# wenet-e2e/wesep

Measured on AMD Instinct MI355X. Metric: utterances/sec (4 s, 16 kHz, 2-spk) fwd+bwd, pBSRNN, higher is better.
Workload: dtype bf16x3+fp16x2+fp16x1 split products (+fp8 lo terms), fp32 accumulate; 1 GPU; pBSRNN FiLM multi-fuse, 6 repeats, feature_dim 128, fixed 256-d embeddings; fwd + SI-SDR + bwd + per-tensor clip + Adam-L2; bf16x3 (x-projections, projections, d(hcat), BN / mask GEMMs) + fp16x2 (recurrent products of all four recurrence kernels, d(xn)) + fp16x1 (LSTM weight gradients); 2-byte saved gates / d(gates); fp32 accumulate; BPTT kernels: W_hh as fp16 hi + block-scaled FP8 lo; the lo term; rows_per_gpu=32, global_rows=32, samples_per_row=64000, parallelism=dp1

## Files before the change

include/wesep_hip.h:

```cpp
#ifndef WESEP_HIP_H_
#define WESEP_HIP_H_

#ifdef __cplusplus
extern "C" {
#endif

#define WS_ABI_VERSION 20
#define WS_OK 0
#define WS_ERR_INVALID (-1)
#define WS_ERR_LAUNCH (-2)

int ws_abi_version(void);
const char* ws_last_error(void);

#define WS_PROF_LSTM_FWD 0
#define WS_PROF_LSTM_BWD 1
#define WS_PROF_GEMM_NT 2
#define WS_PROF_GEMM_TN 3
#define WS_PROF_NKINDS 4
int ws_prof_enable(int on);
int ws_prof_collect(int kind, double* total_ms, long long* launches);
int ws_debug_dirty_lds(float value, int nblocks, int spins, float* sink, void* stream);
int ws_debug_occupy(int nblocks, int usec, const unsigned* stop, float* sink, void* stream);

// ... 76 lines not shown

int ws_reduce_slabs(const float* slab, int nsplit, long long stride, long long count,
                    float* out, int w, long long ldo, void* stream);

int ws_transpose(const float* src, int rows, int cols, long long lds, float* dst, void* stream);

typedef struct ws_groups_geom {
  const int* band_w;
  const int* band_off;
  long long gs1, gs2, rs;
  int ngroups, gdiv, L, W;
  int nbands, pad_;
} ws_groups_geom;
int ws_group_stats(const float* x, const ws_groups_geom* geo, float eps, float* stats, void* stream);
int ws_group_stats_len(const float* x, const ws_groups_geom* geo, const int* glen, int glen_div, float eps, float* stats,
                       void* stream);

int ws_gn_bwd_reduce(const float* x, const float* dxn, const float* stats, const float* gamma,
                     const float* const* gamma_tab, const ws_groups_geom* geo, float* ab,
                     void* stream);
int ws_gn_bwd_apply(const float* x, const float* dxn, const float* stats, const float* ab,
                    const float* gamma, const float* const* gamma_tab, const float* res,
                    const ws_groups_geom* geo, float* dx, void* stream);
int ws_gn_param_grad(const float* x, const float* dxn, const float* stats,
                     const ws_groups_geom* geo, int nsplit, float* slab, void* stream);

int ws_gn_bwd_fused(const float* x, const float* dxn, const float* stats, const float* gamma,
                    const float* res, const ws_groups_geom* geo, int nwg, float* dx, float* pslab,
                    float* pout, unsigned* counter, void* stream);
int ws_gn_bwd_fused2(const float* x, const float* dxn, const float* dxn2, const float* stats, const float* gamma,
                     const float* res, const ws_groups_geom* geo, int nwg, float* dx, float* pslab,
                     float* pout, unsigned* counter, void* stream);
int ws_gn_bwd_apply_pg(const float* x, const float* dxn, const float* stats, const float* ab,
                       const float* gamma, const float* res, const ws_groups_geom* geo, float* dx,
                       float* pslab, float* pout, unsigned* counter, void* stream);

typedef struct ws_lstm_args {
  float* gates;
  float* cbuf;
  float* hcat;
  const float* dhcat;
  const float* wpack;
  long long sq_s1, sq_s2, step_rows;
  int nseq, sq_div, L, mode;
  const unsigned* run_if;
  const float* gates_in;
  float* dgates;
  int gfmt;
  int rfmt;
  const unsigned* amax;
  float* dxn;
  long long dxn_dir_stride;
  const float* wxpack;
} ws_lstm_args;
#define WS_GATES_F32 0
#define WS_GATES_H2 1
#define WS_GATES_H2S 2
#define WS_GATES_H2F 3
#define WS_DGATES_EXP 8
#define WS_LSTM_F32_MT1 1
#define WS_LSTM_F32_MT2 2
#define WS_LSTM_BF16X3 3
#define WS_LSTM_BF16X3_BLK 4
#define WS_LSTM_BF16X3_BLK16 5
#define WS_LSTM_H 256
#define WS_LSTM_PACK_FLOATS (2 * 4 * WS_LSTM_H * WS_LSTM_H)
int ws_lstm_pack(const float* whh_f, const float* whh_r, float* pack_fwd, float* pack_bwd,
                 int mode, void* stream);
int ws_lstm_pack_bwd_f8(const float* whh_f, const float* whh_r, float* pack_bwd, void* stream);
#define WS_LSTM_DX_PACK_FLOATS (16 * (48 * 1024 + 64) / 4)
int ws_lstm_pack_dx_f8(const float* wcat, float* pack, void* stream);
int ws_lstm_fwd(const ws_lstm_args* a, void* stream);
int ws_lstm_bwd(const ws_lstm_args* a, void* stream);
typedef struct ws_lstm_cluster_args {
  float* gates;
  float* cbuf;
  float* hcat;
  const float* dhcat;
  const float* whh_f;
  const float* whh_r;
  void* xchg;
  unsigned* flags;
  unsigned* status;
  int nseq, L;
  int dbg, gfmt;
  const float* gates_in;
} ws_lstm_cluster_args;
int ws_lstm_fwd_cluster(const ws_lstm_cluster_args* a, void* stream);
typedef struct ws_lstm_cluster2_args {
  float* gates;
  float* cbuf;
  float* hcat;
  const float* xn;
  const float* wcat;
  const float* bcat;
  const float* whh_f;
  const float* whh_r;
  void* xchg;
  unsigned* tword;
  unsigned* status;
  int nseq, L;
  int dbg, rfmt;
  float* dbg_buf;
} ws_lstm_cluster2_args;
int ws_lstm_fwd_cluster2(const ws_lstm_cluster2_args* a, void* stream);
int ws_lstm_bwd_cluster(const ws_lstm_cluster_args* a, void* stream);
typedef struct ws_lstm_pair_args {
  float* gates;
  const float* cbuf;
  const float* dhcat;
  const float* wpack;
  void* xchg;
  unsigned* flags;
  unsigned* status;
  float* dbg_buf;
  int nseq, L;
  int dbg, gfmt;
  float* dgates;
  const unsigned* amax;
  int rfmt, pad_;
} ws_lstm_pair_args;
int ws_lstm_pack_pair(const float* whh_f, const float* whh_r, float* pack, void* stream);
int ws_lstm_pack_pair_f16(const float* whh_f, const float* whh_r, float* pack, void* stream);
int ws_lstm_pack_pair_f8(const float* whh_f, const float* whh_r, float* pack, void* stream);
int ws_lstm_pack_pair_f8mx(const float* whh_f, const float* whh_r, float* pack, void* stream);
int ws_lstm_bwd_pair(const ws_lstm_pair_args* a, void* stream);
int ws_lstm_cat_ih(const float* wih_f, const float* wih_r, const float* bih_f, const float* bhh_f,
                   const float* bih_r, const float* bhh_r, int n_in, float* wcat, float* bcat,
                   void* stream);

typedef struct ws_seqmap {
  long long sq_s1, sq_s2, step_rows;
  int nseq, sq_div, L;
  int nvalid;
} ws_seqmap;

int ws_pack_w(const float* W, int N, int K, long long ldw, int trans, int order, float* out,
              void* stream);
int ws_pack_w_f16(const float* W, int N, int K, long long ldw, int trans, int order, float* out,
                  void* stream);
int ws_pack_w_f16f8(const float* W, int N, int K, long long ldw, int trans, float* out, void* stream);

typedef struct ws_gemm_p2b_args {
  const float* A;
  const float* Wpack;
  const float* bias;
  float* C;
  float* A_bl;
  const float* stats;
  const float* gamma;
  const float* beta;
  ws_seqmap sm;
  long long lda, st_m1, st_m2, st_base;
  int st_div1, st_div2, N, K;
  const unsigned* run_if;
  unsigned* amax;
  void* A_bl16;
} ws_gemm_p2b_args;
int ws_gemm_p2b(const ws_gemm_p2b_args* a, void* stream);
int ws_gemm_p2b_len(const ws_gemm_p2b_args* a, const int* steps, int steps_div, void* stream);

typedef struct ws_gemm_b2p_args {
  const float* A;
  const float* Wpack;
  const float* bias;
  const float* R;
  float* C;
  ws_seqmap sm;
  long long ldc;
  int N, K;
  int a_fmt, pad_;
  const unsigned* amax;
  void* a16_out;
} ws_gemm_b2p_args;
int ws_gemm_b2p(const ws_gemm_b2p_args* a, void* stream);

typedef struct ws_gemm_tnb_args {
  const float* G;
  const float* A0;
  const float* A1;
  float* slab;
  float* bslab;
  float* aslab;
  long long slab_stride, bslab_stride, aslab_stride;
  int g_width, g_off, g_cols;
  int a0_width, a0_off, a0_cols, a0_shift;
  int a1_width, a1_off, a1_cols, a1_shift;
  int nblk, L, nsplit, blocks_per_split;
  int g_fmt;
  const unsigned* amax;
  int a_fmt, pad_;
} ws_gemm_tnb_args;
int ws_gemm_tnb(const ws_gemm_tnb_args* a, void* stream);

typedef struct ws_bands {
  const int* band_of_bin;
  const int* band_f0;
  const int* band_bw;
  int nband, nbins;
} ws_bands;
int ws_stft_bandsplit(const float* wav, int R, int T, const ws_bands* b, float* xbs, void* stream);
int ws_stft_bandsplit_len(const float* wav, int R, int T, const int* lengths, const ws_bands* b, float* xbs, void* stream);
int ws_mask_istft_frames(const float* xbs, const float* mask3, int R, int Tf, const ws_bands* b,
                         float* frames, void* stream);
int ws_istft_ola(const float* frames, int R, int Tf, int T, float* wav, void* stream);
int ws_istft_ola_len(const float* frames, int R, int Tf, int T, const int* lengths, float* wav, void* stream);
int ws_mask_istft_bwd(const float* dwav, const float* xbs, const float* mask3, int R, int Tf,
                      int T, const ws_bands* b, float* dmask3, void* stream);

int ws_affine_fwd(const float* z, const float* a, const float* b, float a0, long long rows,
// ... 229 lines not shown
```

wesep_amd/_lib.py:

```python
import ctypes as C
import os

import numpy as np
import torch

_HERE = os.path.dirname(os.path.abspath(__file__))
LIB_PATH = os.environ.get("WESEP_HIP_LIB") or os.path.join(_HERE, "libwesep_hip.so")

WS_OK = 0
PROF_LSTM_FWD, PROF_LSTM_BWD, PROF_GEMM_NT, PROF_GEMM_TN = 0, 1, 2, 3
LSTM_H = 256
ABI_VERSION = 20
GATES_F32, GATES_H2, GATES_H2S, GATES_H2F = 0, 1, 2, 3
DGATES_EXP = 8


def dgates_scale(amax_bits: int) -> float:
    e = (int(amax_bits) >> 23) & 0xFF
    return 1.0 if e in (0, 255) else 2.0 ** (min(max(DGATES_EXP + 254 - e, 1), 253) - 127)


LSTM_F32_MT1, LSTM_F32_MT2, LSTM_BF16X3, LSTM_BF16X3_BLK, LSTM_BF16X3_BLK16 = 1, 2, 3, 4, 5
LSTM_PACK_FLOATS = 2 * 4 * LSTM_H * LSTM_H

# ... 13 lines not shown

class Conv3x3PackArgs(C.Structure):
    _fields_ = [("src", Conv3x3PackSrc * 5), ("out", _p), ("Cin", _i), ("Cout", _i), ("nsrc", _i), ("flip", _i)]


class Conv3x3Args(C.Structure):
    _fields_ = [(n, _p) for n in ("X", "W", "bias", "R", "Y")] + [(n, _ll) for n in ("ldx", "ldw", "ldy")] + \
               [(n, _i) for n in ("B", "H", "Wd", "Cin", "Cout", "pad_")]


class Conv3x3WgradArgs(C.Structure):
    _fields_ = [(n, _p) for n in ("G", "X", "slab", "bslab")] + [(n, _ll) for n in ("ldg", "ldx", "slab_stride", "bslab_stride")] + \
               [(n, _i) for n in ("B", "H", "Wd", "Wx", "sw", "Cin", "Nn", "nsplit", "tiles_per_split", "pad_")]


class HeadsArgs(C.Structure):
    _fields_ = [(n, _p) for n in ("x", "dy", "slope", "gamma", "beta", "y", "stats", "dx", "slab")] + \
               [(n, _ll) for n in ("ldx", "lddx")] + [(n, _i) for n in ("B", "T", "Tp", "Q", "nh", "ch", "nwg")] + \
               [("eps", C.c_float)]


class GemmNTArgs(C.Structure):
    _fields_ = [(n, _p) for n in ("A", "W", "bias", "C", "R", "T", "stats", "gamma", "beta", "groups")] + \
               [(n, _ll) for n in ("a_s1", "a_s2", "c_s1", "c_s2", "st_m1", "st_m2", "st_base")] + \
               [(n, _i) for n in ("a_div", "c_div", "st_div1", "st_div2", "M", "N", "K", "ldw",
                                  "act", "ngroups", "max_n", "vec")] + [("conv", ConvView)]


class GemmTNArgs(C.Structure):
    _fields_ = [(n, _p) for n in ("G", "A", "slab", "bslab", "stats", "gamma", "beta", "groups")] + \
               [(n, _ll) for n in ("g_s1", "g_s2", "a_s1", "a_s2", "st_m1", "st_m2", "st_base",
                                   "slab_stride", "bslab_stride", "out_off", "bout_off")] + \
               [(n, _i) for n in ("g_div", "a_div", "st_div1", "st_div2", "M", "Nn", "Kk",
                                  "rows_per_split", "nsplit", "shift_rows", "seq_div", "seq_len",
                                  "ngroups", "max_n", "max_k", "vec")] + [("conv", ConvView)]


class ConvWgradArgs(C.Structure):
    _fields_ = [(n, _p) for n in ("G", "X", "slab", "bslab")] + \
               [(n, _ll) for n in ("ldg", "slab_stride", "bslab_stride")] + \
               [(n, _i) for n in ("M", "Nn", "nsplit", "tiles_per_split")] + [("conv", ConvView)]


class GroupsGeom(C.Structure):
    _fields_ = [("band_w", _p), ("band_off", _p), ("gs1", _ll), ("gs2", _ll), ("rs", _ll),
                ("ngroups", _i), ("gdiv", _i), ("L", _i), ("W", _i), ("nbands", _i), ("pad_", _i)]


class LstmArgs(C.Structure):
    _fields_ = [(n, _p) for n in ("gates", "cbuf", "hcat", "dhcat", "wpack")] + \
               [(n, _ll) for n in ("sq_s1", "sq_s2", "step_rows")] + \
               [(n, _i) for n in ("nseq", "sq_div", "L", "mode")] + [("run_if", _p)] + \
               [("gates_in", _p), ("dgates", _p), ("gfmt", _i), ("rfmt", _i), ("amax", _p)] + \
               [("dxn", _p), ("dxn_dir_stride", _ll), ("wxpack", _p)]


class SeqMapC(C.Structure):
    _fields_ = [("sq_s1", _ll), ("sq_s2", _ll), ("step_rows", _ll), ("nseq", _i), ("sq_div", _i), ("L", _i), ("nvalid", _i)]


class GemmP2BArgs(C.Structure):
    _fields_ = [(n, _p) for n in ("A", "Wpack", "bias", "C", "A_bl", "stats", "gamma", "beta")] + \
               [("sm", SeqMapC)] + [(n, _ll) for n in ("lda", "st_m1", "st_m2", "st_base")] + \
               [(n, _i) for n in ("st_div1", "st_div2", "N", "K")] + [("run_if", _p), ("amax", _p), ("A_bl16", _p)]


class GemmB2PArgs(C.Structure):
    _fields_ = [(n, _p) for n in ("A", "Wpack", "bias", "R", "C")] + [("sm", SeqMapC), ("ldc", _ll), ("N", _i), ("K", _i),
                                                                         ("a_fmt", _i), ("pad_", _i), ("amax", _p), ("a16_out", _p)]


class GemmTNBArgs(C.Structure):
    _fields_ = [(n, _p) for n in ("G", "A0", "A1", "slab", "bslab", "aslab")] + \
               [(n, _ll) for n in ("slab_stride", "bslab_stride", "aslab_stride")] + \
               [(n, _i) for n in ("g_width", "g_off", "g_cols", "a0_width", "a0_off", "a0_cols", "a0_shift",
                                  "a1_width", "a1_off", "a1_cols", "a1_shift", "nblk", "L", "nsplit",
                                  "blocks_per_split", "g_fmt")] + [("amax", _p), ("a_fmt", _i), ("pad_", _i)]


class LstmClusterArgs(C.Structure):
    _fields_ = [(n, _p) for n in ("gates", "cbuf", "hcat", "dhcat", "whh_f", "whh_r", "xchg", "flags", "status")] + \
               [("nseq", _i), ("L", _i), ("dbg", _i), ("gfmt", _i), ("gates_in", _p)]


class LstmCluster2Args(C.Structure):
    _fields_ = [(n, _p) for n in ("gates", "cbuf", "hcat", "xn", "wcat", "bcat", "whh_f", "whh_r", "xchg", "tword", "status")] + \
               [("nseq", _i), ("L", _i), ("dbg", _i), ("rfmt", _i), ("dbg_buf", _p)]


class LstmPairArgs(C.Structure):
    _fields_ = [(n, _p) for n in ("gates", "cbuf", "dhcat", "wpack", "xchg", "flags", "status", "dbg_buf")] + \
               [("nseq", _i), ("L", _i), ("dbg", _i), ("gfmt", _i), ("dgates", _p), ("amax", _p), ("rfmt", _i), ("pad_", _i)]


class Bands(C.Structure):
    _fields_ = [("band_of_bin", _p), ("band_f0", _p), ("band_bw", _p), ("nband", _i), ("nbins", _i)]


GROUP_NT_DTYPE = np.dtype([("W", "<u8"), ("bias", "<u8"), ("gamma", "<u8"), ("beta", "<u8"),
                           ("a_off", "<i8"), ("c_off", "<i8"), ("st_base", "<i8"),
                           ("K", "<i4"), ("N", "<i4"), ("ldw", "<i4"), ("pad_", "<i4")])
GROUP_TN_DTYPE = np.dtype([("gamma", "<u8"), ("beta", "<u8"), ("g_off", "<i8"), ("a_off", "<i8"),
                           ("st_base", "<i8"), ("out_off", "<i8"), ("bout_off", "<i8"),
                           ("Nn", "<i4"), ("Kk", "<i4"), ("pad0_", "<i4"), ("pad1_", "<i4")])
TENSOR_REF_DTYPE = np.dtype([("param", "<u8"), ("grad", "<u8"), ("exp_avg", "<u8"),
                             ("exp_avg_sq", "<u8"), ("numel", "<i8")])
assert GROUP_NT_DTYPE.itemsize == 72 and GROUP_TN_DTYPE.itemsize == 72 and TENSOR_REF_DTYPE.itemsize == 40

class LstmFusedArgs(C.Structure):
    _fields_ = [("gates", _p), ("cbuf", _p), ("hcat", _p), ("xn", _p), ("wpack", _p), ("bias", _p),
                ("nseq", _i), ("L", _i), ("gfmt", _i), ("hfmt", _i)]


LSTM_FUSED_PACK_FLOATS = 2 * 8 * 24 * 4 * 2 * 64 * 4
LSTM_DX_PACK_FLOATS = 16 * (48 * 1024 + 64) // 4

_SIGS = {
    "ws_abi_version": (_i, []),
    "ws_last_error": (C.c_char_p, []),
    "ws_prof_enable": (_i, [_i]),
    "ws_prof_collect": (_i, [_i, C.POINTER(C.c_double), C.POINTER(_ll)]),
    "ws_debug_dirty_lds": (_i, [_f, _i, _i, _p, _p]),
    "ws_debug_occupy": (_i, [_i, _i, _p, _p, _p]),
    "ws_pack_w_f16": (_i, [_p, _i, _i, _ll, _i, _i, _p, _p]),
    "ws_pack_w_f16f8": (_i, [_p, _i, _i, _ll, _i, _p, _p]),
    "ws_gemm_nt": (_i, [C.POINTER(GemmNTArgs), _p]),
    "ws_gemm_tn": (_i, [C.POINTER(GemmTNArgs), _p]),
    "ws_reduce_slabs": (_i, [_p, _i, _ll, _ll, _p, _i, _ll, _p]),
    "ws_transpose": (_i, [_p, _i, _i, _ll, _p, _p]),
    "ws_group_stats": (_i, [_p, C.POINTER(GroupsGeom), _f, _p, _p]),
    "ws_group_stats_len": (_i, [_p, C.POINTER(GroupsGeom), _p, _i, _f, _p, _p]),
    "ws_gn_bwd_reduce": (_i, [_p, _p, _p, _p, _p, C.POINTER(GroupsGeom), _p, _p]),
    "ws_gn_bwd_apply": (_i, [_p, _p, _p, _p, _p, _p, _p, C.POINTER(GroupsGeom), _p, _p]),
    "ws_gn_param_grad": (_i, [_p, _p, _p, C.POINTER(GroupsGeom), _i, _p, _p]),
    "ws_gn_bwd_fused": (_i, [_p, _p, _p, _p, _p, C.POINTER(GroupsGeom), _i, _p, _p, _p, _p, _p]),
    "ws_gn_bwd_fused2": (_i, [_p, _p, _p, _p, _p, _p, C.POINTER(GroupsGeom), _i, _p, _p, _p, _p, _p]),
    "ws_gn_bwd_apply_pg": (_i, [_p, _p, _p, _p, _p, _p, C.POINTER(GroupsGeom), _p, _p, _p, _p, _p]),
    "ws_lstm_pack": (_i, [_p, _p, _p, _p, _i, _p]),
    "ws_lstm_fwd": (_i, [C.POINTER(LstmArgs), _p]),
    "ws_lstm_bwd": (_i, [C.POINTER(LstmArgs), _p]),
    "ws_lstm_fwd_cluster": (_i, [C.POINTER(LstmClusterArgs), _p]),
    "ws_lstm_bwd_cluster": (_i, [C.POINTER(LstmClusterArgs), _p]),
    "ws_lstm_fwd_cluster2": (_i, [C.POINTER(LstmCluster2Args), _p]),
    "ws_lstm_pack_pair": (_i, [_p, _p, _p, _p]),
    "ws_lstm_pack_pair_f16": (_i, [_p, _p, _p, _p]),
# ... 158 lines not shown
```

wesep_amd/blstm_core.py:

```python
import math
import os
from typing import NamedTuple

import numpy as np
import torch

from . import _lib as L
from . import dev

H = L.LSTM_H
G4 = 4 * H
N = 128


def _empty(dev_, *shape):
    return torch.empty(*shape, device=dev_, dtype=torch.float32)


def _reduce_new(slab, nsplit, stride, shape):
    out = _empty(slab.device, *shape)
    dev.reduce_slabs(slab, nsplit, stride, int(np.prod(shape)), out)
    return out


def _h2_probe() -> int:
    return int(os.environ.get("WESEP_H2_PROBE", "0"))


_PROBE_SAT = [0, 0.0]


def _probe_round(t, kind, packed=False):
    if kind == "f16":
        t.copy_(t.half().float())
    elif kind == "u16":
        v = t.view(-1, 2, 4, 64 * 128)
        v[:, :, 2].mul_(0.5).add_(0.5)
        v.copy_(torch.floor(v * 65535.0 + 0.5) / 65535.0)
        v[:, :, 2].mul_(2.0).sub_(1.0)
    elif packed and torch.cuda.is_available():
        t.view(torch.int32).bitwise_and_(-65536)
    else:
        t.copy_(t.bfloat16().float())


def tnb_a16() -> bool:
    return os.environ.get("WESEP_TNB_A16", "1") != "0"


def pair_rfmt(gfmt) -> int:
    rf = int(os.environ.get("WESEP_PAIR_RF", "3"))
    if rf not in (0, 1, 2, 3):
        raise ValueError(f"WESEP_PAIR_RF={rf}: 0, 1, 2 or 3")
    return rf if gfmt == L.GATES_H2F else 0


def dxn_fmt(g_fmt) -> int:
    return 3 if g_fmt == 2 and os.environ.get("WESEP_DXN_F8", "1") != "0" else g_fmt


def band_rfmt(gfmt, lmode) -> int:
    rf = int(os.environ.get("WESEP_BAND_RF", "3"))
    if rf not in (0, 2, 3):
        raise ValueError(f"WESEP_BAND_RF={rf}: 0, 2 or 3")
    if rf == 3 and os.environ.get("WESEP_BAND_DX", "0") == "1":
        rf = 2
    return rf if gfmt == L.GATES_H2F and lmode == L.LSTM_BF16X3_BLK else 0


def band_dx(brf, seq, geo) -> bool:
    return (brf == 2 and os.environ.get("WESEP_BAND_DX", "0") == "1" and not seq.nvalid and dev.gn_bwd_fused_ok(geo))


_SIDE_STREAMS = {}


def _side_stream(device):
    key = (device.type, device.index)
    if key not in _SIDE_STREAMS:
        pr = os.environ.get("WESEP_SIDE_PRIORITY")
        _SIDE_STREAMS[key] = torch.cuda.Stream(device=device, priority=int(pr)) if pr else torch.cuda.Stream(device=device)
    return _SIDE_STREAMS[key]
# ... 199 lines not shown
        self.cache.note(kind)
        return self.cache.get(self.sig, key, lambda: self._build(kind))

    def _build(self, kind):
        W, lmode, pair_rf = self, self.lmode, self.pair_rf
        wih_f, whh_f, bih_f, bhh_f, wih_r, whh_r, bih_r, bhh_r, proj_w = self.weights
        d = wih_f.device
        N = wih_f.shape[1]
        if kind == "cat":
            wcat, bcat = _empty(d, 2 * G4, N), _empty(d, 2 * G4)
            dev.lstm_cat_ih(wih_f.contiguous(), wih_r.contiguous(), bih_f, bhh_f, bih_r, bhh_r, N, wcat, bcat)
            return wcat, bcat
        if kind == "whh":
            return whh_f.contiguous(), whh_r.contiguous()
        if kind == "hh":
            pack_f, pack_b = _empty(d, L.LSTM_PACK_FLOATS), _empty(d, L.LSTM_PACK_FLOATS)
            dev.lstm_pack(*W("whh"), pack_f, pack_b, lmode)
            return pack_f, pack_b
        if kind == "hh8":
            pack = _empty(d, L.LSTM_PACK_FLOATS)
            dev.lstm_pack_bwd_f8(*W("whh"), pack)
            return pack
        if kind == "wx8":
            pack = _empty(d, L.LSTM_DX_PACK_FLOATS)
            dev.lstm_pack_dx_f8(W("cat")[0], pack)
            return pack
        if kind in ("hhp", "hhp16"):
            pack = _empty(d, L.LSTM_PACK_FLOATS)
            dev.lstm_pack_pair(*W("whh"), pack, f16=pair_rf if kind == "hhp16" else 0)
            return pack
        if kind in ("fused", "fused16", "fused8"):
            fpack = _empty(d, L.LSTM_FUSED_PACK_FLOATS)
            dev.lstm_pack_fused(wih_f.contiguous(), wih_r.contiguous(), *W("whh"), fpack,
                                hfmt={"fused": 0, "fused16": 1, "fused8": 5}[kind])
            return fpack
        if kind == "wih":
            out = _empty(d, 2 * G4 * N)
            dev.pack_w(W("cat")[0], 2 * G4, N, N, out, order=0)
            return out
        if kind in ("wihT", "wihT16", "wihT8"):
            out = _empty(d, N * 2 * G4)
            dev.pack_w(W("cat")[0], N, 2 * G4, N, out, trans=True, order=1, f16={"wihT": 0, "wihT16": 1, "wihT8": 2}[kind])
            return out
        if kind == "pw":
            return proj_w.contiguous()
        if kind == "proj":
            out = _empty(d, N * 2 * H)
            dev.pack_w(W("pw"), N, 2 * H, 2 * H, out, order=1)
            return out
        if kind == "projT":
            out = _empty(d, 2 * H * N)
            dev.pack_w(W("pw"), 2 * H, N, 2 * H, out, trans=True, order=0)
            return out
        raise KeyError(kind)


class BlstmPlan(NamedTuple):
    nb: int
    lmode: int
    cluster: bool
    fwd: str
    bptt: str
    grad: bool
    gfmt: int
    g_fmt: int
    a16: bool
    pair_rfmt: int
    band_rfmt: int
    band_dx: bool
    a_fmt: int


_WIHT_KIND = {0: "wihT", 1: "wihT", 2: "wihT16", 3: "wihT8"}


def make_plan(seq, device, grad, gn_geo=None, ragged=False) -> BlstmPlan:
    lmode = dev.lstm_blk_mode(seq.nseq)
    cluster = dev.lstm_cluster_ok(seq, device)
    bptt = _bptt_kind(seq, device, cluster)
    gfmt = L.GATES_F32 if bptt == "cluster" else dev.gates_fmt()
    h2 = gfmt != L.GATES_F32
    if ragged:
        fwd = "cluster" if cluster else "stream"
    elif dev.lstm_fuse_ok(seq.nseq, cluster):
        fwd = "fused"
    elif cluster:
        fwd = "cluster2" if h2 and dev.lstm_cluster2_on() else "cluster"
    else:
        fwd = "stream"
    g_fmt = {L.GATES_H2: 1, L.GATES_H2F: 2}.get(gfmt, 0)
    brf = band_rfmt(gfmt, lmode) if grad and bptt == "stream" else 0
    return BlstmPlan(
        nb=dev.bl_num_blocks(seq), lmode=lmode, cluster=cluster, fwd=fwd, bptt=bptt, grad=grad, gfmt=gfmt, g_fmt=g_fmt,
        a16=gfmt == L.GATES_H2F and grad and tnb_a16(), pair_rfmt=pair_rfmt(gfmt) if grad and bptt == "pair" else 0,
        band_rfmt=brf, band_dx=bool(brf) and gn_geo is not None and band_dx(brf, seq, gn_geo), a_fmt=dxn_fmt(g_fmt))


def consume_once(ctx, who):
    if ctx.consumed:
        raise L.WesepHipError(f"{who}: second backward through the same graph (retain_graph / multi-loss loops): "
                              "the blocked path consumes its saved gates in place; run the forward again")
    ctx.consumed = True


def blstm_forward(plan, W, x, seq, res, bias, norm=None, steps=None):
    d = x.device
    norm = norm or {}
    if steps is not None and (plan.fwd in ("fused", "cluster2") or plan.grad):
        raise L.WesepHipError(f"blstm_forward: per-sequence step counts with forward branch '{plan.fwd}', grad={plan.grad}: "
                              "only the branches over precomputed gates know them, and only the forward")
    lens = dict(steps=steps[0], steps_div=steps[1]) if steps is not None else {}
    nb, gfmt, lmode = plan.nb, plan.gfmt, plan.lmode
    h2 = gfmt != L.GATES_F32
    wcat, bcat = W("cat")
    whf, whr = W("whh")
    xn = _empty(d, nb, 32 * N)
    cbuf, hcat = _empty(d, nb, 32 * 2 * H), _empty(d, nb, 32 * 2 * H)
    gates = _empty(d, dev.blh_floats(nb, 2 * G4)) if h2 else _empty(d, nb, 32 * 2 * G4)
    xn16 = _empty(d, dev.blh_floats(nb, N)) if plan.a16 else None
    hcat16 = _empty(d, dev.blh_floats(nb, 2 * H)) if plan.a16 else None
    if plan.fwd == "fused":
        dev.gemm_p2b(A=x, lda=N, sm=seq, Wpack=None, N=0, C_out=None, A_bl=xn, A_bl16=xn16, **norm)
        hf = dev.lstm_fused_hfmt(gfmt)
        dev.lstm_fwd_fused(gates, cbuf, hcat, xn, W("fused8" if hf & 4 else "fused16" if hf else "fused"), bcat, seq, gfmt=gfmt,
                           hfmt=hf)
    elif plan.fwd == "cluster2":
        dev.gemm_p2b(A=x, lda=N, sm=seq, Wpack=None, N=0, C_out=None, A_bl=xn, A_bl16=xn16, **norm)
        tw = dev.lstm_fwd_cluster2(gates, cbuf, hcat, xn, wcat, bcat, whf, whr, seq, dbg=_cluster_dbg())
        pre = dev.fallback_scratch(d, nb * 32 * 2 * G4)
        dev.gemm_p2b(A=x, lda=N, sm=seq, Wpack=W("wih"), N=2 * G4, C_out=pre, bias=bcat, run_if=tw, **norm)
        dev.lstm_fwd(gates, cbuf, hcat, W("hh")[0], seq, lmode, run_if=tw, gfmt=gfmt, gates_in=pre)
        del pre
    else:
        pre = _empty(d, nb, 32 * 2 * G4) if h2 else gates
        xproj = dict(A=x, lda=N, sm=seq, Wpack=W("wih"), N=2 * G4, C_out=pre, bias=bcat, A_bl=xn, A_bl16=xn16, **norm, **lens)
        rec = dict(gfmt=gfmt, gates_in=pre) if h2 else {}
        dev.gemm_p2b(**xproj)
        if _h2_probe() & 768 and not torch.cuda.is_available():
            pre.copy_(pre.half().float() if _h2_probe() & 256 else pre.bfloat16().float())
        if plan.fwd == "cluster":
            tw = dev.lstm_fwd_cluster(gates, cbuf, hcat, whf, whr, seq, dbg=_cluster_dbg(), **rec)
            if not h2:
                dev.gemm_p2b(run_if=tw, **xproj)
            dev.lstm_fwd(gates, cbuf, hcat, W("hh")[0], seq, lmode, run_if=tw, **rec)
        else:
            dev.lstm_fwd(gates, cbuf, hcat, W("hh")[0], seq, lmode, **rec)
        del pre
    out = torch.empty_like(res)
    dev.gemm_b2p(A=hcat, K=2 * H, sm=seq, Wpack=W("proj"), C_out=out, ldc=N, bias=bias, R=res, a16_out=hcat16)
    if _h2_probe() and not h2:
        if _h2_probe() & 1:
            _probe_round(gates, "f16")
        if _h2_probe() & 8:
            _probe_round(gates, "u16")
        if _h2_probe() & 4:
            _probe_round(cbuf, "f16")
    if plan.grad:
        W("projT")
        if not plan.band_dx:
            W(_WIHT_KIND[plan.a_fmt])
        if plan.bptt == "pair":
            W("hhp16" if plan.pair_rfmt else "hhp")
        if (plan.bptt == "stream" and not plan.band_rfmt) or (plan.bptt == "pair" and h2):
            W("hh")
        if plan.bptt == "stream" and plan.band_rfmt:
            W("hh8")
            if plan.band_dx:
                W("wx8")
    return out, (gates, cbuf, hcat, xn16 if plan.a16 else xn, hcat16)


def blstm_bptt(plan, W, gates, cbuf, hcat, dout, seq, release):
    d = dout.device
    nb, gfmt = plan.nb, plan.gfmt
    dh, dout_bl = _empty(d, nb, 32 * 2 * H), _empty(d, nb, 32 * N)
    dxn2 = None
    amax = amax_word(d) if gfmt == L.GATES_H2F else None
    dev.gemm_p2b(A=dout, lda=N, sm=seq, Wpack=W("projT"), N=2 * H, C_out=dh, A_bl=dout_bl, amax=amax)
    if _h2_probe() & 16:
        _probe_round(dh, "bf16")
    ready = mark_wgrads_ready(d) if release else None
    if plan.bptt == "cluster":
        dg = gates
        dev.lstm_bwd_cluster(gates, cbuf, dh, *W("whh"), seq)
    elif gfmt == L.GATES_F32:
        dg = gates
        if plan.bptt == "pair":
            dev.lstm_bwd_pair(gates, cbuf, dh, W("hhp"), seq, dbg=_pair_dbg())
        else:
            dev.lstm_bwd(gates, cbuf, hcat, dh, W("hh")[1], seq, plan.lmode)
    elif plan.bptt == "pair":
        dg = _empty(d, nb, 32 * 2 * G4) if gfmt == L.GATES_H2S else _empty(d, dev.blh_floats(nb, 2 * G4))
        rf = plan.pair_rfmt
        tw = dev.lstm_bwd_pair(gates, cbuf, dh, W("hhp16" if rf else "hhp"), seq, gfmt=gfmt, dgates=dg, repairable=True,
                               dbg=_pair_dbg(), amax=amax, rfmt=rf, dbg_buf=_pair_stamp_buf(d, seq.L))
        dev.lstm_bwd(gates, cbuf, hcat, dh, W("hh")[1], seq, plan.lmode, gfmt=gfmt, dgates=dg, run_if=tw, amax=amax)
    else:
        dg = _empty(d, nb, 32 * 2 * G4) if gfmt == L.GATES_H2S else gates
        brf = plan.band_rfmt
        if plan.band_dx:
            dxn2 = _empty(d, 2, dout.numel() // N, N)
        dev.lstm_bwd(gates, cbuf, hcat, dh, W("hh8") if brf else W("hh")[1], seq, plan.lmode, gfmt=gfmt,
                     dgates=dg if gfmt == L.GATES_H2S else None, amax=amax, rfmt=brf, dxn=dxn2,
                     wxpack=W("wx8") if dxn2 is not None else None)
    if _h2_probe() & 2 and gfmt == L.GATES_F32:
        _probe_round(gates, "bf16", packed=True)
    if _h2_probe() & 32 and gfmt == L.GATES_F32 and not torch.cuda.is_available():
        amax = float(dh.abs().max())
        S = 2.0 ** (10 - math.floor(math.log2(amax))) if amax > 0 and math.isfinite(amax) else 1.0
        sc = gates * S
        _PROBE_SAT[0] += int((sc.abs() > 65504.0).sum())
        _PROBE_SAT[1] = max(_PROBE_SAT[1], float(sc.abs().max()) / 65504.0)
        gates.copy_(sc.clamp(-65504.0, 65504.0).half().float() / S)
    if ready is not None:
        flush_deferred_wgrads(d, ready)
    return dg, dout_bl, amax, dxn2


def weight_grads(gates, xn, hcat, dout_bl, seq, nb, g_fmt=0, amax=None, hcat16=None):
    d = gates.device
    a_fmt = 1 if hcat16 is not None else 0
    if _h2_probe() & 192 and not torch.cuda.is_available() and not a_fmt:
        rnd = (lambda t: t.half().float()) if _h2_probe() & 64 else (lambda t: t.bfloat16().float())
        xn, hcat = rnd(xn), rnd(hcat)
    if os.environ.get("WESEP_PROBE_SKIP_WGRAD") == "1":
        z_ = lambda *s_: torch.zeros(*s_, device=d)
        return [z_(G4, N), z_(G4, H), z_(G4), z_(G4), z_(G4, N), z_(G4, H), z_(G4), z_(G4), z_(N, 2 * H), z_(N)]
    if _h2_probe() & 1024 and not torch.cuda.is_available() and amax is not None:
        S = L.dgates_scale(int(amax.reshape(-1)[0]))
        hcat = hcat.half().float()
        dout_bl = (dout_bl * S).half().float() / S
    ns, bps = dev.tnb_splits(nb, (2 * H) // 128)
    slab, aslab = _empty(d, ns, 2 * H * N), _empty(d, ns, N)
    dev.gemm_tnb(G=hcat, g_width=2 * H, g_off=0, g_cols=2 * H, A0=dout_bl, a0_width=N, a0_off=0, a0_cols=N,
                 nblk=nb, L_=seq.L, slab=slab, nsplit=ns, blocks_per_split=bps, aslab=aslab)
    dproj_w = _reduce_new(slab, ns, 2 * H * N, (2 * H, N)).t().contiguous()
    dproj_b = _reduce_new(aslab, ns, N, (N,))
    ns, bps = dev.tnb_splits(nb, G4 // 128)
    slab, bslab = _empty(d, ns, G4 * (N + H)), _empty(d, ns, G4)
    dwih, dwhh, db = [], [], []
    for di in (0, 1):
        dev.gemm_tnb(G=gates, g_width=2 * G4, g_off=di * G4, g_cols=G4, A0=xn, a0_width=N, a0_off=0,
                     a0_cols=N, A1=hcat16 if a_fmt else hcat, a1_width=2 * H, a1_off=di * H, a1_cols=H,
                     a1_shift=(-1 if di == 0 else 1), nblk=nb, L_=seq.L, slab=slab, nsplit=ns,
                     blocks_per_split=bps, bslab=bslab, g_fmt=g_fmt, amax=amax, a_fmt=a_fmt)
        dw = _reduce_new(slab, ns, G4 * (N + H), (G4, N + H))
        dwih.append(dw[:, :N].contiguous())
        dwhh.append(dw[:, N:].contiguous())
        db.append(_reduce_new(bslab, ns, G4, (G4,)))
    return [dwih[0], dwhh[0], db[0], db[0].clone(), dwih[1], dwhh[1], db[1], db[1].clone(),
            dproj_w, dproj_b]


def blstm_weight_grads(plan, dg, xn, hcat, dout_bl, amax, hcat16, seq, box, order=tuple(range(10))):
    if box is None:
        wg = weight_grads(dg, xn, hcat, dout_bl, seq, plan.nb, plan.g_fmt, amax, hcat16)
        return [wg[i] for i in order]
# ... 19 lines not shown
```

wesep_amd/csrc/gemm_blk.hip:

```cpp
#include <stdlib.h>

#include <type_traits>

#include "common.h"

typedef __bf16 bf16x8 __attribute__((ext_vector_type(8)));
typedef unsigned int u32x4 __attribute__((ext_vector_type(4)));
typedef unsigned int u32x2 __attribute__((ext_vector_type(2)));
typedef float f32x2 __attribute__((ext_vector_type(2)));
typedef _Float16 f16x8 __attribute__((ext_vector_type(8)));
typedef _Float16 f16x2 __attribute__((ext_vector_type(2)));
typedef int i32x4 __attribute__((ext_vector_type(4)));
typedef int v8i __attribute__((ext_vector_type(8)));
typedef __fp16 h16x2 __attribute__((ext_vector_type(2)));

__device__ __forceinline__ f32x16 mfma32(bf16x8 a, bf16x8 b, f32x16 c) {
  return __builtin_amdgcn_mfma_f32_32x32x16_bf16(a, b, c, 0, 0, 0);
}

__device__ __forceinline__ void split8(const float* v, bf16x8& hi, bf16x8& lo) {
#pragma unroll
  for (int j = 0; j < 8; ++j) {
    hi[j] = (__bf16)v[j];
    lo[j] = (__bf16)(v[j] - (float)hi[j]);
// ... 108 lines not shown
__global__ __launch_bounds__(256) void pack_w16f8_kernel(const float* __restrict__ W, int K, long long ldw, int trans,
                                                         unsigned char* __restrict__ out) {
  const int st = blockIdx.x, nt = threadIdx.x >> 6, lane = threadIdx.x & 63, n = 32 * nt + (lane & 31);
  unsigned char* sb = out + (long long)st * 24576;
  float res[32];
  float mx = 0.f;
#pragma unroll
  for (int i = 0; i < 4; ++i) {
    f16x8 hi;
#pragma unroll
    for (int j = 0; j < 8; ++j) {
      const int k = 64 * st + 16 * i + 8 * (lane >> 5) + j;
      const float v = WS_PACK16_SCALE * (trans ? W[(long long)k * ldw + n] : W[(long long)n * ldw + k]);
      hi[j] = (_Float16)v;
      res[8 * i + j] = v - (float)hi[j];
      mx = fmaxf(mx, fabsf(res[8 * i + j]));
    }
    reinterpret_cast<f16x8*>(sb)[(i * 4 + nt) * 64 + lane] = hi;
  }
#pragma unroll
  for (int o = 32; o >= 1; o >>= 1) mx = fmaxf(mx, __shfl_xor(mx, o));
  int E = mx > 0.f ? ((__float_as_int(mx) >> 23) & 255) - 127 - 7 : 0;
  E = max(E, -126);
  const float inv = __int_as_float((127 - E) << 23);
  unsigned int* o8 = reinterpret_cast<unsigned int*>(sb + 16384 + nt * 2048 + lane * 16);
#pragma unroll
  for (int j = 0; j < 32; j += 4) {
    int c = 0;
    c = __builtin_amdgcn_cvt_pk_fp8_f32(res[j] * inv, res[j + 1] * inv, c, false);
    c = __builtin_amdgcn_cvt_pk_fp8_f32(res[j + 2] * inv, res[j + 3] * inv, c, true);
    o8[(j >> 4) * 256 + ((j & 15) >> 2)] = (unsigned int)c;
  }
  if (lane == 0) (out + (long long)(K / 64) * 24576)[st * 4 + nt] = (unsigned char)(127 + E);
}

extern "C" int ws_pack_w_f16f8(const float* W, int N, int K, long long ldw, int trans, float* out, void* stream) {
  WS_REQUIRE(W && out && N == 128 && K > 0 && K % 64 == 0, "ws_pack_w_f16f8: N = 128, K %% 64 (N=%d K=%d)", N, K);
  hipLaunchKernelGGL(pack_w16f8_kernel, dim3(K / 64), dim3(256), 0, (hipStream_t)stream, W, K, ldw, trans,
                     reinterpret_cast<unsigned char*>(out));
  return ws_check_launch("ws_pack_w_f16f8");
}

extern "C" int ws_pack_w(const float* W, int N, int K, long long ldw, int trans, int order, float* out,
                         void* stream) {
  WS_REQUIRE(W && out && N > 0 && K > 0 && N % 32 == 0 && K % 16 == 0, "ws_pack_w: N %% 32, K %% 16 (N=%d K=%d)",
             N, K);
  WS_REQUIRE(order == 0 || order == 1, "ws_pack_w: order");
  hipLaunchKernelGGL(pack_w_kernel, dim3((N * K / 8 + 255) / 256), dim3(256), 0, (hipStream_t)stream, W, N, K, ldw,
                     trans, order, reinterpret_cast<__bf16*>(out));
  return ws_check_launch("ws_pack_w");
}

#define P2B_K 128
template <bool LEN>
__global__ __launch_bounds__(512, 4) void gemm_p2b_kernel(const ws_gemm_p2b_args p, const int* __restrict__ steps,
                                                          int steps_div) {
  __shared__ __attribute__((aligned(16))) u32x4 wl[2][2048];
  if (p.run_if && *p.run_if == 0u) return;
  const int tid = threadIdx.x, lane = tid & 63, i = lane & 31, half = lane >> 5;
  const int w = __builtin_amdgcn_readfirstlane(tid >> 6);
  const int nblk = ((p.sm.nseq + 31) / 32) * p.sm.L;
  const int b = blockIdx.x * 8 + w;
  const bool active = b < nblk;
  const int bb = active ? b : nblk - 1;
  bool valid;
  const long long pos = seq_pos(p.sm, bb, i, valid);
  if (LEN) {
    const int tile = bb / p.sm.L, step = bb - tile * p.sm.L;
    const int nv = p.sm.nvalid > 0 ? p.sm.nvalid : p.sm.nseq;
    valid = valid && step < steps[min(tile * 32 + i, nv - 1) / steps_div];
  }

  bf16x8 xh[8], xl[8];
  {
    const float* arow = p.A + pos * p.lda;
    float mean = 0.f, rstd = 1.f;
    if (p.stats) {
      const long long s = (pos / p.st_div1) * p.st_m1 + (pos % p.st_div2) * p.st_m2 + p.st_base;
      mean = p.stats[2 * s];
      rstd = p.stats[2 * s + 1];
    }
    float* eb = p.A_bl ? p.A_bl + (long long)bb * (32 * P2B_K) + i * 4 : nullptr;
    unsigned short* eb16 = p.A_bl16 ? reinterpret_cast<unsigned short*>(p.A_bl16) + (long long)bb * (32 * P2B_K) + i * 4 : nullptr;
#pragma unroll
    for (int ks = 0; ks < 8; ++ks) {
      const int k0 = 16 * ks + 8 * half;
      f32x4 v0 = *reinterpret_cast<const f32x4*>(arow + k0);
      f32x4 v1 = *reinterpret_cast<const f32x4*>(arow + k0 + 4);
      if (p.stats) {
        const f32x4 g0 = *reinterpret_cast<const f32x4*>(p.gamma + k0), g1 = *reinterpret_cast<const f32x4*>(p.gamma + k0 + 4);
        const f32x4 b0 = *reinterpret_cast<const f32x4*>(p.beta + k0), b1 = *reinterpret_cast<const f32x4*>(p.beta + k0 + 4);
        v0 = (v0 - mean) * rstd * g0 + b0;
        v1 = (v1 - mean) * rstd * g1 + b1;
      }
      if (!valid) {
        v0 = f32x4{0.f, 0.f, 0.f, 0.f};
        v1 = v0;
      }
      const float v[8] = {v0[0], v0[1], v0[2], v0[3], v1[0], v1[1], v1[2], v1[3]};
      split8(v, xh[ks], xl[ks]);
      if (eb && active) {
        u32x4 c0, c1;
        pack8(xh[ks], xl[ks], c0, c1);
        *reinterpret_cast<u32x4*>(eb + (k0 / 4) * 128) = c0;
        *reinterpret_cast<u32x4*>(eb + (k0 / 4 + 1) * 128) = c1;
      }
      if (eb16 && active) {
        const f16x2 h0 = {(_Float16)v[0], (_Float16)v[1]}, h1 = {(_Float16)v[2], (_Float16)v[3]};
        const f16x2 h2 = {(_Float16)v[4], (_Float16)v[5]}, h3 = {(_Float16)v[6], (_Float16)v[7]};
        *reinterpret_cast<u32x2*>(eb16 + (k0 / 4) * 128) = u32x2{__builtin_bit_cast(unsigned, h0), __builtin_bit_cast(unsigned, h1)};
        *reinterpret_cast<u32x2*>(eb16 + (k0 / 4 + 1) * 128) = u32x2{__builtin_bit_cast(unsigned, h2), __builtin_bit_cast(unsigned, h3)};
      }
    }
  }

  const int nstage = p.N / 64;
  if (nstage == 0) return;
  const u32x4* wsrc = reinterpret_cast<const u32x4*>(p.Wpack);
  u32x4 wreg[4];
#pragma unroll
  for (int q = 0; q < 4; ++q) wreg[q] = wsrc[tid + 512 * q];
#pragma unroll
  for (int q = 0; q < 4; ++q) wl[0][tid + 512 * q] = wreg[q];
  __syncthreads();
  float* cblk = p.C + (long long)bb * 32 * p.N + i * 4;
  float cmax = 0.f;
  for (int st = 0; st < nstage; ++st) {
    const int cur = st & 1;
    if (st + 1 < nstage) {
#pragma unroll
      for (int q = 0; q < 4; ++q) wreg[q] = wsrc[(long long)(st + 1) * 2048 + tid + 512 * q];
    }
#pragma unroll
    for (int t2 = 0; t2 < 2; ++t2) {
      const u32x4* wt = &wl[cur][t2 * 1024 + lane];
      f32x16 acc;
#pragma unroll
      for (int ks = 0; ks < 8; ++ks) {
        const bf16x8 ah = __builtin_bit_cast(bf16x8, wt[(ks * 2) * 64]);
        const bf16x8 al = __builtin_bit_cast(bf16x8, wt[(ks * 2 + 1) * 64]);
        if (ks == 0) {
          const f32x16 zero = {0.f, 0.f, 0.f, 0.f, 0.f, 0.f, 0.f, 0.f, 0.f, 0.f, 0.f, 0.f, 0.f, 0.f, 0.f, 0.f};
          acc = mfma32(ah, xh[ks], zero);
        } else {
          acc = mfma32(ah, xh[ks], acc);
        }
        acc = mfma32(al, xh[ks], acc);
        acc = mfma32(ah, xl[ks], acc);
      }
      if (active) {
        const int n0 = st * 64 + t2 * 32;
#pragma unroll
        for (int j = 0; j < 4; ++j) {
          const int n = n0 + 8 * j + 4 * half;
          f32x4 v = {acc[4 * j], acc[4 * j + 1], acc[4 * j + 2], acc[4 * j + 3]};
          if (p.bias) v += *reinterpret_cast<const f32x4*>(p.bias + n);
          if (!valid) v = f32x4{0.f, 0.f, 0.f, 0.f};
          *reinterpret_cast<f32x4*>(cblk + (n / 4) * 128) = v;
          cmax = fmaxf(fmaxf(cmax, fmaxf(fabsf(v[0]), fabsf(v[1]))), fmaxf(fabsf(v[2]), fabsf(v[3])));
        }
      }
    }
    if (st + 1 < nstage) {
#pragma unroll
      for (int q = 0; q < 4; ++q) wl[cur ^ 1][tid + 512 * q] = wreg[q];
    }
    __syncthreads();
  }
  if (p.amax) {
#pragma unroll
    for (int o = 32; o > 0; o >>= 1) cmax = fmaxf(cmax, __shfl_xor(cmax, o, 64));
    if (lane == 0) atomicMax(p.amax, __float_as_uint(cmax));
  }
}

static int gemm_p2b_launch(const char* who, const ws_gemm_p2b_args* a, const int* steps, int steps_div, void* stream) {
  WS_REQUIRE(a && a->A && ((a->Wpack && a->C) || (a->N == 0 && (a->A_bl || a->A_bl16))), "%s: null pointer", who);
  WS_REQUIRE(a->K == P2B_K, "%s: K must be %d (got %d)", who, P2B_K, a->K);
  WS_REQUIRE(a->N >= 0 && a->N % 64 == 0, "%s: N %% 64 (N=%d)", who, a->N);
  WS_REQUIRE(a->lda >= a->K && a->lda % 4 == 0, "%s: lda", who);
  WS_REQUIRE(a->sm.nseq > 0 && a->sm.L > 0 && a->sm.sq_div > 0, "%s: bad sequence map", who);
  WS_REQUIRE(!a->stats || (a->gamma && a->beta && a->st_div1 > 0 && a->st_div2 > 0), "%s: norm args", who);
  const int nblk = ((a->sm.nseq + 31) / 32) * a->sm.L;
  hipStream_t s = (hipStream_t)stream;
  const bool timed = a->run_if == nullptr;
  if (timed) ws_prof_begin(WS_PROF_GEMM_NT, s);
  if (steps)
    hipLaunchKernelGGL((gemm_p2b_kernel<true>), dim3((nblk + 7) / 8), dim3(512), 0, s, *a, steps, steps_div);
  else
    hipLaunchKernelGGL((gemm_p2b_kernel<false>), dim3((nblk + 7) / 8), dim3(512), 0, s, *a, steps, steps_div);
  if (timed) ws_prof_end(WS_PROF_GEMM_NT, s);
  return ws_check_launch(who);
}

extern "C" int ws_gemm_p2b(const ws_gemm_p2b_args* a, void* stream) {
  return gemm_p2b_launch("ws_gemm_p2b", a, nullptr, 1, stream);
}

extern "C" int ws_gemm_p2b_len(const ws_gemm_p2b_args* a, const int* steps, int steps_div, void* stream) {
  WS_REQUIRE(steps && steps_div > 0, "ws_gemm_p2b_len: steps table / steps_div");
  return gemm_p2b_launch("ws_gemm_p2b_len", a, steps, steps_div, stream);
}

template <int A16>
__global__ __launch_bounds__(512, 4) void gemm_b2p_kernel(const ws_gemm_b2p_args p) {
  __shared__ __attribute__((aligned(16))) u32x4 wl[2][2048];
  __shared__ long long posl[8][32];
  const int tid = threadIdx.x, lane = tid & 63, i = lane & 31, half = lane >> 5;
  const int w = __builtin_amdgcn_readfirstlane(tid >> 6);
  const int nblk = ((p.sm.nseq + 31) / 32) * p.sm.L;
  const int b = blockIdx.x * 8 + w;
  const bool active = b < nblk;
  const int bb = active ? b : nblk - 1;
  {
    bool valid;
    const long long pos = seq_pos(p.sm, bb, i, valid);
    if (half == 0) posl[w][i] = valid ? pos : -1;
  }
  const int K = p.K, nstage = K / 64;
  typedef typename std::conditional<A16 != 0, u32x2, f32x4>::type acell;
  typedef typename std::conditional<A16 != 0, unsigned short, float>::type aelem;
  constexpr int SU = A16 == 3 ? 1536 : 2048, NQ = SU / 512;
  const int* wsc = reinterpret_cast<const int*>(reinterpret_cast<const unsigned char*>(p.Wpack) + (long long)nstage * 24576);
  int sc_n = A16 == 3 ? wsc[0] : 0;
  const float inv_s = A16 >= 2 ? ws_dgates_scale_inv(*p.amax) * (1.f / WS_PACK16_SCALE) : 1.f;
  const aelem* ab = reinterpret_cast<const aelem*>(p.A) + (long long)bb * 32 * K + i * 4 + 2 * half * 128;
  const __amdgpu_buffer_rsrc_t wsr = __builtin_amdgcn_make_buffer_rsrc(const_cast<float*>(p.Wpack), 0, (unsigned)nstage * SU * 16u,
                                                                        0x00020000);
  auto wstage = [&](int st, int buf) {
#pragma unroll
    for (int q = 0; q < NQ; ++q)
      __builtin_amdgcn_raw_ptr_buffer_load_lds(wsr, (__attribute__((address_space(3))) void*)&wl[buf][(w * NQ + q) * 64], 16, lane * 16,
                                               (st * SU + (w * NQ + q) * 64) * 16, 0, 0);
  };
  constexpr int HS = A16 == 0 ? 2 : 1, KH = 4 / HS;
  acell an[2 * KH];
  auto load_a = [&](int st, int hs) {
    const aelem* a2 = ab + ((long long)st * 16 + hs * KH * 4) * 128;
#pragma unroll
    for (int ks = 0; ks < KH; ++ks) {
      an[2 * ks] = *reinterpret_cast<const acell*>(a2 + (4 * ks) * 128);
      an[2 * ks + 1] = *reinterpret_cast<const acell*>(a2 + (4 * ks + 1) * 128);
    }
// ... 704 lines not shown
```

wesep_amd/csrc/lstm.hip:

```cpp
#include "common.h"

#define LH WS_LSTM_H
#define LG (4 * LH)
#define HL_LD 68
#define DG_LD 260

__device__ __forceinline__ f32x4 mfma16(float a, float b, f32x4 c) {
  return __builtin_amdgcn_mfma_f32_16x16x4f32(a, b, c, 0, 0, 0);
}

__device__ __forceinline__ float fast_sigmoid(float x) {
  return __builtin_amdgcn_rcpf(1.f + __expf(-x));
}
__device__ __forceinline__ float fast_tanh(float x) {
  const float ax = fabsf(x);
  const float e = __expf(-2.f * ax);
  const float t = (1.f - e) * __builtin_amdgcn_rcpf(1.f + e);
  return copysignf(t, x);
}

__global__ void lstm_pack_kernel(const float* __restrict__ whh_f, const float* __restrict__ whh_r,
                                 float* __restrict__ pf, float* __restrict__ pb) {
  const int total = 2 * LG * LH;
  for (int idx = blockIdx.x * blockDim.x + threadIdx.x; idx < total; idx += gridDim.x * blockDim.x) {
// ... 302 lines not shown
#pragma unroll
      for (int s = 0; s < 2; ++s)
#pragma unroll
        for (int r = 0; r < 4; ++r) dh[mt][s][r] = 0.f;
    const float* arow = dgl + (lq * 16 + l15) * DG_LD;
    f32x4 bcur[2], bnxt[2];
    bcur[0] = b00;
    bcur[1] = b01;
#pragma unroll 4
    for (int ks4 = 0; ks4 < 64; ++ks4) {
      if (ks4 + 1 < 64) {
        bnxt[0] = wp[((ks4 + 1) * 2 + 0) * 64];
        bnxt[1] = wp[((ks4 + 1) * 2 + 1) * 64];
      }
      f32x4 a[MT];
#pragma unroll
      for (int mt = 0; mt < MT; ++mt)
        a[mt] = *reinterpret_cast<const f32x4*>(arow + mt * (64 * DG_LD) + 4 * ks4);
#pragma unroll
      for (int q = 0; q < 4; ++q)
#pragma unroll
        for (int s = 0; s < 2; ++s)
#pragma unroll
          for (int mt = 0; mt < MT; ++mt) dh[mt][s] = mfma16(a[mt][q], bcur[s][q], dh[mt][s]);
      bcur[0] = bnxt[0];
      bcur[1] = bnxt[1];
    }
    __syncthreads();
  }
}

static int lstm_check(const ws_lstm_args* a, bool bwd, const char* who) {
  WS_REQUIRE(a && a->gates && a->cbuf && a->hcat && a->wpack, "%s: null pointer", who);
  WS_REQUIRE(!bwd || a->dhcat, "%s: null dhcat", who);
  WS_REQUIRE(a->nseq > 0 && a->L > 0 && a->sq_div > 0, "%s: bad nseq/L/sq_div", who);
  WS_REQUIRE((a->mode & 255) >= WS_LSTM_F32_MT1 && (a->mode & 255) <= WS_LSTM_BF16X3_BLK16, "%s: bad mode %d", who,
             a->mode);
  WS_REQUIRE(!a->run_if || (!bwd && (a->mode & 255) >= WS_LSTM_BF16X3) || (bwd && (a->mode & 255) >= WS_LSTM_BF16X3_BLK),
             "%s: run_if is honoured by the split-bf16 forward kernels and the blocked-layout BPTT kernels only", who);
  WS_REQUIRE(a->gfmt >= WS_GATES_F32 && a->gfmt <= WS_GATES_H2F, "%s: bad gfmt %d", who, a->gfmt);
  WS_REQUIRE(a->gfmt != WS_GATES_H2F || !bwd || a->amax, "%s: WS_GATES_H2F needs amax", who);
  WS_REQUIRE(a->gfmt == WS_GATES_F32 || (a->mode & 255) >= WS_LSTM_BF16X3_BLK,
             "%s: gfmt %d is a format of the blocked-layout modes", who, a->gfmt);
  WS_REQUIRE(a->gfmt == WS_GATES_F32 || bwd || a->gates_in, "%s: gfmt %d needs gates_in (the fp32 pre-activations)", who,
             a->gfmt);
  WS_REQUIRE(a->gfmt != WS_GATES_H2S || !bwd || a->dgates, "%s: WS_GATES_H2S needs dgates", who);
  WS_REQUIRE(a->gfmt == WS_GATES_F32 || ((a->mode >> 8) & 7) == 0, "%s: probe builds are WS_GATES_F32 only", who);
  WS_REQUIRE(a->rfmt == 0 || ((a->rfmt == 2 || a->rfmt == 3) && bwd && a->mode == WS_LSTM_BF16X3_BLK && a->gfmt == WS_GATES_H2F),
             "%s: rfmt %d (2 / 3 = fp16 recurrence on fp16 + FP8 weights, 3: the lo term on the FP8 MFMA: ws_lstm_bwd, "
             "WS_LSTM_BF16X3_BLK, WS_GATES_H2F only)", who, a->rfmt);
  WS_REQUIRE(!a->dxn || (bwd && a->rfmt == 2 && a->wxpack && a->dxn_dir_stride > 0 && a->dxn_dir_stride < (1ll << 29) && !a->run_if),
             "%s: dxn (d(xn) inside the BPTT, ABI v19) needs rfmt 2, wxpack (ws_lstm_pack_dx_f8), 0 < dxn_dir_stride < 2^29 floats "
             "(32-bit store offsets) and no run_if", who);
  return WS_OK;
}

extern "C" int ws_lstm_fwd(const ws_lstm_args* a, void* stream) {
  int rc = lstm_check(a, false, "ws_lstm_fwd");
  if (rc != WS_OK) return rc;
  hipStream_t s = (hipStream_t)stream;
  const int per = 16 * a->mode;
  dim3 grid((a->nseq + per - 1) / per, 2), block(512);
  const bool timed = a->run_if == nullptr;
  if (timed) ws_prof_begin(WS_PROF_LSTM_FWD, s);
  if ((a->mode & 255) == WS_LSTM_BF16X3_BLK16)
    ws_launch_lstm_fwd_s16(a, s);
  else if ((a->mode & 255) >= WS_LSTM_BF16X3)
    ws_launch_lstm_fwd_bf16(a, s);
  else if (a->mode == WS_LSTM_F32_MT1)
    hipLaunchKernelGGL((lstm_fwd_kernel<1>), grid, block, 0, s, *a);
  else
    hipLaunchKernelGGL((lstm_fwd_kernel<2>), grid, block, 0, s, *a);
  if (timed) ws_prof_end(WS_PROF_LSTM_FWD, s);
  return ws_check_launch("ws_lstm_fwd");
}

extern "C" int ws_lstm_bwd(const ws_lstm_args* a, void* stream) {
  int rc = lstm_check(a, true, "ws_lstm_bwd");
  if (rc != WS_OK) return rc;
  hipStream_t s = (hipStream_t)stream;
  const int per = 16 * a->mode;
  dim3 grid((a->nseq + per - 1) / per, 2), block(512);
  const bool timed = a->run_if == nullptr;
  if (timed) ws_prof_begin(WS_PROF_LSTM_BWD, s);
  if ((a->mode & 255) == WS_LSTM_BF16X3_BLK16)
    ws_launch_lstm_bwd_s16(a, s);
  else if ((a->mode & 255) >= WS_LSTM_BF16X3)
    ws_launch_lstm_bwd_bf16(a, s);
  else if (a->mode == WS_LSTM_F32_MT1)
    hipLaunchKernelGGL((lstm_bwd_kernel<1>), grid, block, 0, s, *a);
  else
    hipLaunchKernelGGL((lstm_bwd_kernel<2>), grid, block, 0, s, *a);
  if (timed) ws_prof_end(WS_PROF_LSTM_BWD, s);
  return ws_check_launch("ws_lstm_bwd");
}
```

wesep_amd/csrc/lstm_bf16.hip:

```cpp
#include <stdlib.h>

#include "lstm_bf16_common.h"

__global__ void lstm_pack_bf16_kernel(const float* __restrict__ whh_f, const float* __restrict__ whh_r,
                                      __bf16* __restrict__ pf, __bf16* __restrict__ pb) {
  const int total = 2 * LG * LH;
  for (int idx = blockIdx.x * blockDim.x + threadIdx.x; idx < total; idx += gridDim.x * blockDim.x) {
    {
      int r = idx;
      const int j = r & 7; r >>= 3;
      const int lane = r & 63; r >>= 6;
      const int g = r & 3; r >>= 2;
      const int ks = r & 15; r >>= 4;
      const int w = r & 7; r >>= 3;
      const int d = r;
      const float* W = d ? whh_r : whh_f;
      const int row = g * 256 + 32 * w + (lane & 31);
      const int k = 16 * ks + 8 * (lane >> 5) + j;
      const float v = W[row * LH + k];
      const __bf16 hi = (__bf16)v;
      const long long unit = ((((long long)(d * 8 + w) * 16 + ks) * 4 + g) * 2) * 64 + lane;
      pf[unit * 8 + j] = hi;
      pf[(unit + 64) * 8 + j] = (__bf16)(v - (float)hi);
    }
// ... 223 lines not shown
      for (int j = 0; j < 4; ++j)
#pragma unroll
        for (int r = 0; r < 4; ++r) acc[g][4 * j + r] += xg[g][j][r];
    if (!(DBG & 2)) {
#pragma unroll
      for (int j = 0; j < 4; ++j)
#pragma unroll
        for (int g = 0; g < 4; ++g) xg[g][j] = ld_gate(tn, g, j);
    }
    __builtin_amdgcn_sched_barrier(0);
#pragma unroll
    for (int j = 0; j < 4; ++j) {
      f32x4 pre[4];
#pragma unroll
      for (int g = 0; g < 4; ++g)
#pragma unroll
        for (int r = 0; r < 4; ++r) pre[g][r] = acc[g][4 * j + r];
      f32x4 vi, vf, vg, vo, vc, vh;
      const f32x4 cold = *reinterpret_cast<const f32x4*>(cme + 8 * j);
#pragma unroll
      for (int r = 0; r < 4; ++r) {
        const float ig = fsig(pre[0][r]);
        const float fg = fsig(pre[1][r]);
        const float gg = ftanh(pre[2][r]);
        const float og = fsig(pre[3][r]);
        const float cn = fg * cold[r] + ig * gg;
        vi[r] = ig;
        vf[r] = fg;
        vg[r] = gg;
        vo[r] = og;
        vc[r] = cn;
        vh[r] = og * ftanh(cn);
      }
      bf16x4 h_hi, h_lo;
      split4(vh, h_hi, h_lo);
      *reinterpret_cast<bf16x4*>(nhi + 8 * j) = h_hi;
      *reinterpret_cast<bf16x4*>(nlo + 8 * j) = h_lo;
      *reinterpret_cast<f32x4*>(cme + 8 * j) = vc;
      if (!(DBG & 1) || step == L - 1) {
        st_gate(vi, t, 0, j);
        st_gate(vf, t, 1, j);
        st_gate(vg, t, 2, j);
        st_gate(vo, t, 3, j);
        st_ch(vc, p.cbuf, t, j);
        if constexpr (BLK) st_ch(pack_hl4(h_hi, h_lo), p.hcat, t, j);
        else st_ch(vh, p.hcat, t, j);
      }
      __builtin_amdgcn_sched_barrier(0);
    }
    __syncthreads();
  }
}

template <bool BLK, int DBG, int GF = 0, int RF = 0, bool DX = false>
__global__ __launch_bounds__(512, 2) void lstm_bwd_bf16_kernel(const ws_lstm_args p) {
  static_assert(RF == 0 || (BLK && GF == WS_GATES_H2F), "the fp16 recurrence takes the scaled-fp16 d(gates) of WS_GATES_H2F");
  static_assert(!DX || RF == 2, "d(xn) in the BPTT rides on the fp16 d(gates) image of rfmt 2");
  __shared__ __attribute__((aligned(16))) __bf16 dgl[RF ? 1 : 2][SQ * DROW];
  __shared__ __attribute__((aligned(16))) f32x4 xred[DX ? 8 * 2 * 64 : 1];
  if (p.run_if && *p.run_if == 0u) return;
  const int d = blockIdx.y, bx = blockIdx.x;
  const int tid = threadIdx.x, lane = tid & 63, l31 = lane & 31, half = lane >> 5;
  const int w = __builtin_amdgcn_readfirstlane(tid >> 6);
  const int L = p.L;
  const int ss = min(bx * SQ + l31, p.nseq - 1);
  const long long rowbase =
      BLK ? 0 : (long long)(ss / p.sq_div) * p.sq_s1 + (long long)(ss % p.sq_div) * p.sq_s2;
  const int ubase = 32 * w + 4 * half;
  const int glane = ((d * 256 + 8 * w + half) * 32 + l31) * 16;
  const int clane = ((d * 64 + 8 * w + half) * 32 + l31) * 16;
  auto goff = [&](int t, int g, int j) -> long long {
    return ((rowbase + (long long)t * p.step_rows) * 2 + d) * LG + g * 256 + ubase + 8 * j;
  };
  auto coff = [&](int t, int j) -> long long {
    return (rowbase + (long long)t * p.step_rows) * (2 * LH) + d * LH + ubase + 8 * j;
  };
  float* gdst = GF == WS_GATES_H2S ? p.dgates : p.gates;
  auto grs = [&](int t) { return mkrsrc(gdst + (long long)(bx * L + t) * (SQ * 2 * LG), SQ * 2 * LG * 4); };
  auto hrs = [&](int t) { return mkrsrc(p.gates + (long long)(bx * L + t) * (SQ * LG), SQ * 2 * LG * 2); };
  constexpr bool G2 = GF == WS_GATES_H2 || GF == WS_GATES_H2F;
  float* hdst = (G2 && p.dgates) ? p.dgates : p.gates;
  auto ors = [&](int t) { return mkrsrc(hdst + (long long)(bx * L + t) * (SQ * LG), SQ * 2 * LG * 2); };
  const float dS = GF == WS_GATES_H2F ? ws_dgates_scale(*p.amax) : 1.f;
  auto crs = [&](const float* b, int t) { return mkrsrc(b + (long long)(bx * L + t) * (SQ * 2 * LH), SQ * 2 * LH * 4); };
  typedef typename gate_cell<GF>::type gcell;
  auto ld_gate = [&](int t, int g, int j) -> gcell {
    if constexpr (GF != 0) return bld8(hrs(t), glane >> 1, (g * 64 + 2 * j) * 256);
    else if constexpr (BLK) return bld(grs(t), glane, (g * 64 + 2 * j) * 512);
    else return *reinterpret_cast<const f32x4*>(p.gates + goff(t, g, j));
  };
  auto st_gate = [&](const f32x4& v, int t, int g, int j) {
    if constexpr (BLK) bst(v, grs(t), glane, (g * 64 + 2 * j) * 512);
    else *reinterpret_cast<f32x4*>(p.gates + goff(t, g, j)) = v;
  };
  auto ld_ch = [&](const float* b, int t, int j) -> f32x4 {
    if constexpr (BLK) return bld(crs(b, t), clane, 2 * j * 512);
    else return *reinterpret_cast<const f32x4*>(b + coff(t, j));
  };

  const int kpar = DX ? (w >> 2) : 0;
  const __amdgpu_buffer_rsrc_t wrs = __builtin_amdgcn_make_buffer_rsrc(
      const_cast<float*>(p.wpack) + (long long)(d * 8 + w) * (64 * 2 * 64 * 4), 0, 64 * 2 * 1024, 0x00020000);
  const int wlane = lane * 16;
  bf16x8 wr[2][RF ? 4 : 8];
  u32x2 wq[2][RF ? 4 : 1];
  float wS[RF ? 8 : 1];
  int wE[RF == 3 ? 8 : 1];
  auto wfill = [&](int s, int chunk, int zo) {
    if constexpr (RF != 0) {
#pragma unroll
      for (int q = 0; q < 4; ++q) {
        const int fq = q ^ kpar;
        wr[s][q] = wload(wrs, wlane, zo + chunk * 6144 + fq * 1024);
        wq[s][q] = __builtin_bit_cast(u32x2, __builtin_amdgcn_raw_buffer_load_b64(wrs, lane * 8, zo + chunk * 6144 + 4096 + fq * 512, 0));
      }
    } else {
#pragma unroll
      for (int f = 0; f < 8; ++f) wr[s][f] = wload(wrs, wlane + (f & 3) * 1024, zo + chunk * 8192 + (f >> 2) * 4096);
    }
  };
  typedef _Float16 f16x8 __attribute__((ext_vector_type(8)));
  typedef _Float16 f16x2 __attribute__((ext_vector_type(2)));
  const __amdgpu_buffer_rsrc_t xrs = __builtin_amdgcn_make_buffer_rsrc(
      const_cast<char*>(reinterpret_cast<const char*>(p.wxpack)) + (DX ? (long long)(d * 8 + w) * WS_DX_REGION : 0), 0,
      DX ? WS_DX_REGION : 0, 0x00020000);
  bf16x8 xr[2][DX ? 2 : 1];
  u32x2 xq[2][DX ? 2 : 1];
  float xS[DX ? 8 : 1];
  f32x16 dxa;
  auto xfill = [&](int s, int chunk, int zo) {
    if constexpr (DX) {
#pragma unroll
      for (int q = 0; q < 2; ++q) {
        xr[s][q] = wload(xrs, wlane + q * 1024, zo + chunk * 3072);
        xq[s][q] = __builtin_bit_cast(u32x2, __builtin_amdgcn_raw_buffer_load_b64(xrs, lane * 8 + q * 512, zo + chunk * 3072 + 2048, 0));
      }
    }
  };
  if constexpr (RF != 0) {
    const float* st = p.wpack + (long long)(d * 8 + w) * (64 * 2 * 64 * 4) + 96 * 256;
#pragma unroll
    for (int g8 = 0; g8 < 8; ++g8) wS[g8] = __builtin_bit_cast(float, __builtin_amdgcn_readfirstlane(__builtin_bit_cast(int, st[g8])));
    if constexpr (RF == 3) {
#pragma unroll
      for (int g8 = 0; g8 < 8; ++g8) wE[g8] = (__builtin_bit_cast(int, wS[g8]) >> 23) & 255;
    }
  }
  if constexpr (DX) {
    const float* st = reinterpret_cast<const float*>(reinterpret_cast<const char*>(p.wxpack) + (long long)(d * 8 + w) * WS_DX_REGION + 48 * 1024);
#pragma unroll
    for (int g8 = 0; g8 < 8; ++g8) xS[g8] = __builtin_bit_cast(float, __builtin_amdgcn_readfirstlane(__builtin_bit_cast(int, st[g8])));
  }
  unsigned xoff = 0u;
  if constexpr (DX) {
    const int sq = bx * SQ + l31;
    const long long row = (long long)(sq / p.sq_div) * p.sq_s1 + (long long)(sq % p.sq_div) * p.sq_s2;
    xoff = sq < p.nseq ? (unsigned)(row * 512 + (32 * (w & 3) + 16 * kpar + 4 * half) * 4) : 0x80000000u;
  }
  const __amdgpu_buffer_rsrc_t xors = __builtin_amdgcn_make_buffer_rsrc(
      DX ? p.dxn + (long long)d * p.dxn_dir_stride : nullptr, 0, DX ? (unsigned)(p.dxn_dir_stride * 4) : 0u, 0x00020000);
  gcell n_i[4], n_f[4], n_g[4], n_o[4];
  f32x4 n_dh[4], n_cp[4], c_cur[4], dc[4];
  f32x16 dhr;
  const f32x4 zero4v = {0.f, 0.f, 0.f, 0.f};
#pragma unroll
  for (int j = 0; j < 4; ++j) dc[j] = zero4v;
#pragma unroll
  for (int i = 0; i < 16; ++i) dhr[i] = 0.f;

  auto load_step = [&](int t, int j) {
    n_i[j] = ld_gate(t, 0, j);
    n_f[j] = ld_gate(t, 1, j);
    n_g[j] = ld_gate(t, 2, j);
    n_o[j] = ld_gate(t, 3, j);
    n_dh[j] = ld_ch(p.dhcat, t, j);
    const int tp = d == 0 ? max(t - 1, 0) : min(t + 1, L - 1);
    n_cp[j] = ld_ch(p.cbuf, tp, j);
  };
  {
    const int t0 = d == 0 ? L - 1 : 0;
#pragma unroll
    for (int j = 0; j < 4; ++j) {
      load_step(t0, j);
      c_cur[j] = ld_ch(p.cbuf, t0, j);
    }
  }
  __builtin_amdgcn_sched_barrier(0);
  wfill(0, 0, 0);
  xfill(0, 0, 0);
  wfill(1, 1, 0);
  xfill(1, 1, 0);
  __builtin_amdgcn_sched_barrier(0);

  for (int step = 0; step < L; ++step) {
    const int t = d == 0 ? L - 1 - step : step;
    const int sn = min(step + 1, L - 1);
    const int tn = d == 0 ? L - 1 - sn : sn;
    const bool has_prev = d == 0 ? (t > 0) : (t < L - 1);
    int zo = 0;
    asm volatile("" : "+s"(zo));
    __bf16* dhi = &dgl[0][l31 * DROW + ubase];
    __bf16* dlo = &dgl[RF ? 0 : 1][l31 * DROW + ubase];
#pragma unroll
    for (int j = 0; j < 4; ++j) {
      f32x4 pi, pf, pg, po;
      const f32x4 vi = gate_val<false>(n_i[j]), vf = gate_val<false>(n_f[j]), vg = gate_val<true>(n_g[j]),
                  vo = gate_val<false>(n_o[j]);
#pragma unroll
      for (int r = 0; r < 4; ++r) {
        const float ig = vi[r], fg = vf[r], gg = vg[r], og = vo[r];
        const float dhv = dh_in<GF>(n_dh[j][r], dhr[4 * j + r], dS);
        const float tc = ftanh(c_cur[j][r]);
        const float dov = dhv * tc;
        const float dcv = dc[j][r] + dhv * og * (1.f - tc * tc);
        dc[j][r] = dcv * fg;
        pi[r] = dcv * gg * ig * (1.f - ig);
        pf[r] = dcv * (has_prev ? n_cp[j][r] : 0.f) * fg * (1.f - fg);
        pg[r] = dcv * ig * (1.f - gg * gg);
        po[r] = dov * og * (1.f - og);
      }
      c_cur[j] = n_cp[j];
      const bool st = !(DBG & 1) || step == L - 1;
      auto emit = [&](const f32x4& v, int g) {
        if constexpr (RF != 0) {
          const u32x2 code = enc_f16x4(v);
          *reinterpret_cast<u32x2*>(dhi + 256 * g + 8 * j) = code;
          if (st) bst8(code, ors(t), glane >> 1, (g * 64 + 2 * j) * 256);
          return;
        }
        bf16x4 hi, lo;
        split4(v, hi, lo);
        *reinterpret_cast<bf16x4*>(dhi + 256 * g + 8 * j) = hi;
        *reinterpret_cast<bf16x4*>(dlo + 256 * g + 8 * j) = lo;
        if (st) {
          if constexpr (G2) bst8(enc_dgates<GF>(v, hi), ors(t), glane >> 1, (g * 64 + 2 * j) * 256);
          else if constexpr (BLK) st_gate(pack_hl4(hi, lo), t, g, j);
          else st_gate(v, t, g, j);
        }
      };
      emit(pi, 0);
      emit(pf, 1);
      emit(pg, 2);
      emit(po, 3);
      if (!(DBG & 2)) load_step(tn, j);
      __builtin_amdgcn_sched_barrier(0);
    }
    __syncthreads();

    const __bf16* bhi = &dgl[0][l31 * DROW + 8 * half];
    const __bf16* blo = &dgl[RF ? 0 : 1][l31 * DROW + 8 * half];
    const __bf16* bhx[2] = {bhi + 16 * kpar, bhi - 16 * kpar};
    f32x16 acc0;
    f32x16 acc1;
    v8i b8;
#pragma unroll
    for (int ch = 0; ch < 16; ++ch) {
      const int s = ch & 1;
#pragma unroll
      for (int q = 0; q < 4; ++q) {
        const int ks = 4 * ch + q;
        const bf16x8 bh = *reinterpret_cast<const bf16x8*>((DX ? bhx[q & 1] : bhi) + 16 * ks);
        if constexpr (RF == 3) {
          typedef _Float16 f16x2 __attribute__((ext_vector_type(2)));
          typedef short s16x2 __attribute__((ext_vector_type(2)));
// ... 70 lines not shown
      const bool hi_rows = kpar != 0;
#pragma unroll
      for (int i = 0; i < 2; ++i) {
        f32x4 send;
#pragma unroll
        for (int r = 0; r < 4; ++r) {
          const float lo_v = dxa[4 * i + r], hi_v = dxa[8 + 4 * i + r];
          send[r] = hi_rows ? lo_v : hi_v;
          keep[i][r] = hi_rows ? hi_v : lo_v;
        }
        xred[(w * 2 + i) * 64 + lane] = send;
      }
    }
    __syncthreads();
    if constexpr (DX) {
      const float us = (1.f / 256.f) / dS;
      const unsigned trow = (unsigned)t * (unsigned)p.step_rows * 512u;
#pragma unroll
      for (int i = 0; i < 2; ++i) {
        const f32x4 o = xred[((w ^ 4) * 2 + i) * 64 + lane];
        __builtin_amdgcn_raw_buffer_store_b128(__builtin_bit_cast(u32x4, (keep[i] + o) * us), xors, xoff + trow + 32 * i, 0, 0);
      }
    }
  }
}

#define WS_DBG_DISPATCH(KERNEL)                                                          \
  if ((a->mode & 255) == WS_LSTM_BF16X3_BLK && a->gfmt == WS_GATES_H2) {                 \
    hipLaunchKernelGGL((KERNEL<true, 0, WS_GATES_H2>), grid, block, 0, s, *a);           \
  } else if ((a->mode & 255) == WS_LSTM_BF16X3_BLK && a->gfmt == WS_GATES_H2S) {         \
    hipLaunchKernelGGL((KERNEL<true, 0, WS_GATES_H2S>), grid, block, 0, s, *a);          \
  } else if ((a->mode & 255) == WS_LSTM_BF16X3_BLK && a->gfmt == WS_GATES_H2F) {         \
    hipLaunchKernelGGL((KERNEL<true, 0, WS_GATES_H2F>), grid, block, 0, s, *a);          \
  } else if ((a->mode & 255) == WS_LSTM_BF16X3_BLK) {                                    \
    switch ((a->mode >> 8) & 7) {                                                        \
      case 0: hipLaunchKernelGGL((KERNEL<true, 0>), grid, block, 0, s, *a); break;       \
      case 1: hipLaunchKernelGGL((KERNEL<true, 1>), grid, block, 0, s, *a); break;       \
      case 2: hipLaunchKernelGGL((KERNEL<true, 2>), grid, block, 0, s, *a); break;       \
      case 4: hipLaunchKernelGGL((KERNEL<true, 4>), grid, block, 0, s, *a); break;       \
      default: hipLaunchKernelGGL((KERNEL<true, 7>), grid, block, 0, s, *a); break;      \
    }                                                                                    \
  } else {                                                                               \
    hipLaunchKernelGGL((KERNEL<false, 0>), grid, block, 0, s, *a);                       \
  }

int ws_launch_lstm_fwd_bf16(const ws_lstm_args* a, hipStream_t s) {
  dim3 grid((a->nseq + SQ - 1) / SQ, 2), block(512);
  WS_DBG_DISPATCH(lstm_fwd_bf16_kernel)
  return 0;
}

int ws_launch_lstm_bwd_bf16(const ws_lstm_args* a, hipStream_t s) {
  dim3 grid((a->nseq + SQ - 1) / SQ, 2), block(512);
  if (a->rfmt == 2 && a->dxn) {
    hipLaunchKernelGGL((lstm_bwd_bf16_kernel<true, 0, WS_GATES_H2F, 2, true>), grid, block, 0, s, *a);
    return 0;
  }
  if (a->rfmt == 2) {
    hipLaunchKernelGGL((lstm_bwd_bf16_kernel<true, 0, WS_GATES_H2F, 2>), grid, block, 0, s, *a);
    return 0;
  }
  if (a->rfmt == 3) {
    hipLaunchKernelGGL((lstm_bwd_bf16_kernel<true, 0, WS_GATES_H2F, 3>), grid, block, 0, s, *a);
    return 0;
  }
  WS_DBG_DISPATCH(lstm_bwd_bf16_kernel)
  return 0;
}
```

wesep_amd/csrc/lstm_bf16_common.h:

```cpp
#pragma once
#include "common.h"

typedef __bf16 bf16x8 __attribute__((ext_vector_type(8)));
typedef __bf16 bf16x4 __attribute__((ext_vector_type(4)));

#define LH WS_LSTM_H
#define LG (4 * LH)
#define SQ 32
#define HROW 264
#define DROW 1032

typedef unsigned int u32x4 __attribute__((ext_vector_type(4)));

__device__ __forceinline__ bf16x8 wload(__amdgpu_buffer_rsrc_t rsrc, int voff, int soff) {
  return __builtin_bit_cast(bf16x8, __builtin_amdgcn_raw_buffer_load_b128(rsrc, voff, soff, 0));
}

__device__ __forceinline__ __amdgpu_buffer_rsrc_t mkrsrc(const float* base, unsigned bytes) {
  return __builtin_amdgcn_make_buffer_rsrc(const_cast<float*>(base), 0, bytes, 0x00020000);
}
#ifndef WS_STREAM_AUX
#define WS_STREAM_AUX 2
#endif
__device__ __forceinline__ f32x4 bld(__amdgpu_buffer_rsrc_t r, int voff, int soff) {
// ... 56 lines not shown
  l.y = __builtin_amdgcn_perm(u[3], u[2], WS_SEL_LO16);
  hi = __builtin_bit_cast(bf16x4, h);
  lo = __builtin_bit_cast(bf16x4, l);
}


typedef unsigned int u32x2 __attribute__((ext_vector_type(2)));
#define WS_U16_SIG 65535.f
#define WS_U16_TANH 32767.5f

__device__ __forceinline__ u32x2 bld8(__amdgpu_buffer_rsrc_t r, int voff, int soff) {
  return __builtin_bit_cast(u32x2, __builtin_amdgcn_raw_buffer_load_b64(r, voff, soff, WS_STREAM_AUX));
}
__device__ __forceinline__ void bst8(const u32x2& v, __amdgpu_buffer_rsrc_t r, int voff, int soff) {
  __builtin_amdgcn_raw_buffer_store_b64(v, r, voff + soff, 0, WS_STREAM_AUX);
}
template <bool TANH>
__device__ __forceinline__ u32x2 enc_u16x4(const f32x4& v) {
  const float s = TANH ? WS_U16_TANH : WS_U16_SIG, o = TANH ? WS_U16_TANH + 0.5f : 0.5f;
  unsigned u[4];
#pragma unroll
  for (int j = 0; j < 4; ++j) u[j] = (unsigned)__builtin_fmaf(v[j], s, o);
  return u32x2{u[0] | (u[1] << 16), u[2] | (u[3] << 16)};
}
template <bool TANH>
__device__ __forceinline__ f32x4 dec_u16x4(const u32x2& c) {
  const float s = TANH ? 1.f / WS_U16_TANH : 1.f / WS_U16_SIG, o = TANH ? -1.f : 0.f;
  f32x4 v;
  v[0] = __builtin_fmaf((float)(c[0] & 0xffffu), s, o);
  v[1] = __builtin_fmaf((float)(c[0] >> 16), s, o);
  v[2] = __builtin_fmaf((float)(c[1] & 0xffffu), s, o);
  v[3] = __builtin_fmaf((float)(c[1] >> 16), s, o);
  return v;
}
__device__ __forceinline__ u32x2 bf16x4_bits(const bf16x4& v) { return __builtin_bit_cast(u32x2, v); }
typedef _Float16 f16x4 __attribute__((ext_vector_type(4)));
__device__ __forceinline__ u32x2 enc_f16x4(const f32x4& vs) {
  f16x4 h;
#pragma unroll
  for (int j = 0; j < 4; ++j) h[j] = (_Float16)vs[j];
  return __builtin_bit_cast(u32x2, h);
}
template <int GF>
__device__ __forceinline__ u32x2 enc_dgates(const f32x4& v, const bf16x4& hi) {
  if constexpr (GF == WS_GATES_H2F) return enc_f16x4(v);
  else return bf16x4_bits(hi);
}
template <int GF>
__device__ __forceinline__ float dh_in(float dh, float rec, float S) {
  if constexpr (GF == WS_GATES_H2F) return __builtin_fmaf(dh, S, rec);
  else return dh + rec;
}

template <int GF> struct gate_cell { typedef f32x4 type; };
template <> struct gate_cell<WS_GATES_H2> { typedef u32x2 type; };
template <> struct gate_cell<WS_GATES_H2S> { typedef u32x2 type; };
template <> struct gate_cell<WS_GATES_H2F> { typedef u32x2 type; };
template <bool TANH> __device__ __forceinline__ f32x4 gate_val(const f32x4& c) { return c; }
template <bool TANH> __device__ __forceinline__ f32x4 gate_val(const u32x2& c) { return dec_u16x4<TANH>(c); }
```

wesep_amd/csrc/lstm_bf16_s16.hip:

```cpp
#include "lstm_bf16_common.h"

#define S16 16

__device__ __forceinline__ f32x4 mfma16(bf16x8 a, bf16x8 b, f32x4 c) {
  return __builtin_amdgcn_mfma_f32_16x16x32_bf16(a, b, c, 0, 0, 0);
}

__global__ void lstm_pack_s16_kernel(const float* __restrict__ whh_f, const float* __restrict__ whh_r,
                                     __bf16* __restrict__ pf, __bf16* __restrict__ pb) {
  const int total = 2 * LG * LH;
  for (int idx = blockIdx.x * blockDim.x + threadIdx.x; idx < total; idx += gridDim.x * blockDim.x) {
    {
      int r = idx;
      const int j = r & 7; r >>= 3;
      const int lane = r & 63; r >>= 6;
      const int tile = r & 7; r >>= 3;
      const int ks = r & 7; r >>= 3;
      const int w = r & 7; r >>= 3;
      const int d = r;
      const float* W = d ? whh_r : whh_f;
      const int row = (tile >> 1) * 256 + 32 * w + 16 * (tile & 1) + (lane & 15);
      const int k = 32 * ks + 8 * (lane >> 4) + j;
      const float v = W[row * LH + k];
      const __bf16 hi = (__bf16)v;
// ... 121 lines not shown

    const int sn = min(step + 1, L - 1);
    const int tn = d == 0 ? sn : L - 1 - sn;
#pragma unroll
    for (int g = 0; g < 4; ++g)
#pragma unroll
      for (int tu = 0; tu < 2; ++tu) acc[g][tu] += xg[g][tu];
#pragma unroll
    for (int tu = 0; tu < 2; ++tu)
#pragma unroll
      for (int g = 0; g < 4; ++g) xg[g][tu] = ld_gate(tn, g, tu);
    __builtin_amdgcn_sched_barrier(0);
    __bf16* nhi = &hl[cur ^ 1][0][n * HROW + ubase];
    __bf16* nlo = &hl[cur ^ 1][1][n * HROW + ubase];
#pragma unroll
    for (int tu = 0; tu < 2; ++tu) {
      f32x4 vi, vf, vg, vo, vc, vh;
      const f32x4 cold = *reinterpret_cast<const f32x4*>(cme + 16 * tu);
#pragma unroll
      for (int r = 0; r < 4; ++r) {
        const float ig = fsig(acc[0][tu][r]);
        const float fg = fsig(acc[1][tu][r]);
        const float gg = ftanh(acc[2][tu][r]);
        const float og = fsig(acc[3][tu][r]);
        const float cn = fg * cold[r] + ig * gg;
        vi[r] = ig;
        vf[r] = fg;
        vg[r] = gg;
        vo[r] = og;
        vc[r] = cn;
        vh[r] = og * ftanh(cn);
      }
      bf16x4 h_hi, h_lo;
      split4(vh, h_hi, h_lo);
      *reinterpret_cast<bf16x4*>(nhi + 16 * tu) = h_hi;
      *reinterpret_cast<bf16x4*>(nlo + 16 * tu) = h_lo;
      *reinterpret_cast<f32x4*>(cme + 16 * tu) = vc;
      st_gate(vi, t, 0, tu);
      st_gate(vf, t, 1, tu);
      st_gate(vg, t, 2, tu);
      st_gate(vo, t, 3, tu);
      st_ch(vc, p.cbuf, t, tu);
      st_ch(pack_hl4(h_hi, h_lo), p.hcat, t, tu);
      __builtin_amdgcn_sched_barrier(0);
    }
    __syncthreads();
  }
}


#ifndef S16_DBG
#define S16_DBG 0
#endif
template <int GF>
__global__ __launch_bounds__(512, 2) void lstm_bwd_s16_kernel(const ws_lstm_args p) {
  __shared__ __attribute__((aligned(16))) __bf16 dgl[2][S16 * DROW];
  if (p.run_if && *p.run_if == 0u) return;
  const int d = blockIdx.y;
  const int tile = blockIdx.x >> 1, hb = blockIdx.x & 1;
  const int tid = threadIdx.x, lane = tid & 63, n = lane & 15, mq = lane >> 4;
  const int w = __builtin_amdgcn_readfirstlane(tid >> 6);
  const int L = p.L;
  const int glane = ((d * 256 + 8 * w + mq) * 32 + 16 * hb + n) * 16;
  const int clane = ((d * 64 + 8 * w + mq) * 32 + 16 * hb + n) * 16;
  float* gdst = GF == WS_GATES_H2S ? p.dgates : p.gates;
  auto grs = [&](int t) { return mkrsrc(gdst + (long long)(tile * L + t) * (SQ * 2 * LG), SQ * 2 * LG * 4); };
  auto hrs = [&](int t) { return mkrsrc(p.gates + (long long)(tile * L + t) * (SQ * LG), SQ * 2 * LG * 2); };
  constexpr bool G2 = GF == WS_GATES_H2 || GF == WS_GATES_H2F;
  float* hdst = (G2 && p.dgates) ? p.dgates : p.gates;
  auto ors = [&](int t) { return mkrsrc(hdst + (long long)(tile * L + t) * (SQ * LG), SQ * 2 * LG * 2); };
  const float dS = GF == WS_GATES_H2F ? ws_dgates_scale(*p.amax) : 1.f;
  auto crs = [&](const float* b, int t) { return mkrsrc(b + (long long)(tile * L + t) * (SQ * 2 * LH), SQ * 2 * LH * 4); };
  typedef typename gate_cell<GF>::type gcell;
  auto ld_gate = [&](int t, int g, int tu) -> gcell {
    if constexpr (GF != 0) return bld8(hrs(t), glane >> 1, (g * 64 + 4 * tu) * 256);
    else return bld(grs(t), glane, (g * 64 + 4 * tu) * 512);
  };
  auto st_gate = [&](const f32x4& v, int t, int g, int tu) { bst(v, grs(t), glane, (g * 64 + 4 * tu) * 512); };
  auto ld_ch = [&](const float* b, int t, int tu) -> f32x4 { return bld(crs(b, t), clane, 4 * tu * 512); };
  const int ubase = 32 * w + 4 * mq;

  const __amdgpu_buffer_rsrc_t wrs = __builtin_amdgcn_make_buffer_rsrc(
      const_cast<float*>(p.wpack) + (long long)(d * 8 + w) * (32 * 4 * 64 * 4), 0, 32 * 4 * 1024, 0x00020000);
  const int wlane = lane * 16;
  bf16x8 wr[2][16];
#pragma unroll
  for (int s = 0; s < 2; ++s)
#pragma unroll
    for (int f = 0; f < 16; ++f) wr[s][f] = wload(wrs, wlane + (f & 3) * 1024, s * 16384 + (f >> 2) * 4096);

  gcell n_i[2], n_f[2], n_g[2], n_o[2];
  f32x4 n_dh[2], n_cp[2], c_cur[2], dc[2], dhr[2];
  const f32x4 zero4v = {0.f, 0.f, 0.f, 0.f};
#pragma unroll
  for (int tu = 0; tu < 2; ++tu) dc[tu] = dhr[tu] = zero4v;
  auto load_step = [&](int t, int tu) {
    n_i[tu] = ld_gate(t, 0, tu);
    n_f[tu] = ld_gate(t, 1, tu);
    n_g[tu] = ld_gate(t, 2, tu);
    n_o[tu] = ld_gate(t, 3, tu);
    n_dh[tu] = ld_ch(p.dhcat, t, tu);
    const int tp = d == 0 ? max(t - 1, 0) : min(t + 1, L - 1);
    n_cp[tu] = ld_ch(p.cbuf, tp, tu);
  };
  {
    const int t0 = d == 0 ? L - 1 : 0;
#pragma unroll
    for (int tu = 0; tu < 2; ++tu) {
      load_step(t0, tu);
      c_cur[tu] = ld_ch(p.cbuf, t0, tu);
    }
  }

  for (int step = 0; step < L; ++step) {
    const int t = d == 0 ? L - 1 - step : step;
    const int sn = min(step + 1, L - 1);
    const int tn = d == 0 ? L - 1 - sn : sn;
    const bool has_prev = d == 0 ? (t > 0) : (t < L - 1);
    int zo = 0;
    asm volatile("" : "+s"(zo));
    __bf16* dhi = &dgl[0][n * DROW + ubase];
    __bf16* dlo = &dgl[1][n * DROW + ubase];
#pragma unroll
    for (int tu = 0; tu < 2; ++tu) {
      f32x4 pi, pf, pg, po;
      const f32x4 vi = gate_val<false>(n_i[tu]), vf = gate_val<false>(n_f[tu]), vg = gate_val<true>(n_g[tu]),
                  vo = gate_val<false>(n_o[tu]);
#pragma unroll
      for (int r = 0; r < 4; ++r) {
        const float ig = vi[r], fg = vf[r], gg = vg[r], og = vo[r];
        const float dhv = dh_in<GF>(n_dh[tu][r], dhr[tu][r], dS);
        const float tc = ftanh(c_cur[tu][r]);
        const float dov = dhv * tc;
        const float dcv = dc[tu][r] + dhv * og * (1.f - tc * tc);
        dc[tu][r] = dcv * fg;
        pi[r] = dcv * gg * ig * (1.f - ig);
        pf[r] = dcv * (has_prev ? n_cp[tu][r] : 0.f) * fg * (1.f - fg);
        pg[r] = dcv * ig * (1.f - gg * gg);
        po[r] = dov * og * (1.f - og);
      }
      c_cur[tu] = n_cp[tu];
      auto emit = [&](const f32x4& v, int g) {
        bf16x4 hi, lo;
        split4(v, hi, lo);
        *reinterpret_cast<bf16x4*>(dhi + 256 * g + 16 * tu) = hi;
        *reinterpret_cast<bf16x4*>(dlo + 256 * g + 16 * tu) = lo;
        if constexpr (G2) bst8(enc_dgates<GF>(v, hi), ors(t), glane >> 1, (g * 64 + 4 * tu) * 256);
        else if (!(S16_DBG & 2)) st_gate(pack_hl4(hi, lo), t, g, tu);
      };
      emit(pi, 0);
      emit(pf, 1);
      emit(pg, 2);
      emit(po, 3);
      if (!(S16_DBG & 1)) load_step(tn, tu);
      __builtin_amdgcn_sched_barrier(0);
    }
    __syncthreads();

    const __bf16* bhi = &dgl[0][n * DROW + 8 * mq];
    const __bf16* blo = &dgl[1][n * DROW + 8 * mq];
    f32x4 acc[2];
#pragma unroll
    for (int ch = 0; ch < 8; ++ch) {
      const int s = ch & 1;
#pragma unroll
      for (int q = 0; q < 4; ++q) {
        const int ks = 4 * ch + q;
        const bf16x8 bh = *reinterpret_cast<const bf16x8*>(bhi + 32 * ks);
        const bf16x8 bl = *reinterpret_cast<const bf16x8*>(blo + 32 * ks);
#pragma unroll
        for (int tu = 0; tu < 2; ++tu) {
          const int f = (q * 2 + tu) * 2;
          if (ks == 0)
            acc[tu] = mfma16(wr[s][f], bh, zero4v);
          else
            acc[tu] = mfma16(wr[s][f], bh, acc[tu]);
        }
#pragma unroll
        for (int tu = 0; tu < 2; ++tu) acc[tu] = mfma16(wr[s][(q * 2 + tu) * 2 + 1], bh, acc[tu]);
#pragma unroll
        for (int tu = 0; tu < 2; ++tu) acc[tu] = mfma16(wr[s][(q * 2 + tu) * 2], bl, acc[tu]);
      }
      const int cn = (ch + 2) & 7;
      if (!(S16_DBG & 4)) {
#pragma unroll
      for (int f = 0; f < 16; ++f)
        wr[s][f] = wload(wrs, wlane + (f & 3) * 1024, zo + cn * 16384 + (f >> 2) * 4096);
      }
      __builtin_amdgcn_sched_barrier(0);
    }
    dhr[0] = acc[0];
    dhr[1] = acc[1];
    __syncthreads();
  }
}

int ws_launch_lstm_fwd_s16(const ws_lstm_args* a, hipStream_t s) {
  dim3 grid(2 * ((a->nseq + SQ - 1) / SQ), 2), block(512);
  if (a->gfmt) hipLaunchKernelGGL(lstm_fwd_s16_kernel<WS_GATES_H2>, grid, block, 0, s, *a);
  else hipLaunchKernelGGL(lstm_fwd_s16_kernel<0>, grid, block, 0, s, *a);
  return 0;
}

int ws_launch_lstm_bwd_s16(const ws_lstm_args* a, hipStream_t s) {
  dim3 grid(2 * ((a->nseq + SQ - 1) / SQ), 2), block(512);
  if (a->gfmt == WS_GATES_H2) hipLaunchKernelGGL(lstm_bwd_s16_kernel<WS_GATES_H2>, grid, block, 0, s, *a);
  else if (a->gfmt == WS_GATES_H2S) hipLaunchKernelGGL(lstm_bwd_s16_kernel<WS_GATES_H2S>, grid, block, 0, s, *a);
  else if (a->gfmt == WS_GATES_H2F) hipLaunchKernelGGL(lstm_bwd_s16_kernel<WS_GATES_H2F>, grid, block, 0, s, *a);
  else hipLaunchKernelGGL(lstm_bwd_s16_kernel<0>, grid, block, 0, s, *a);
  return 0;
}
```

wesep_amd/csrc/lstm_pair.hip:

```cpp
#include "lstm_bf16_common.h"

typedef __attribute__((address_space(1))) unsigned gu32;
#define SC1 16
#define PR_ROW 520
#define PR_SPIN_LIMIT (1u << 22)
#define PR_XSLOT 16384

__global__ void lstm_pack_pair_kernel(const float* __restrict__ whh_f, const float* __restrict__ whh_r,
                                      __bf16* __restrict__ out) {
  const int total = 2 * LG * LH;
  for (int idx = blockIdx.x * blockDim.x + threadIdx.x; idx < total; idx += gridDim.x * blockDim.x) {
    int r = idx;
    const int j = r & 7; r >>= 3;
    const int lane = r & 63; r >>= 6;
    const int ks = r & 31; r >>= 5;
    const int w = r & 7; r >>= 3;
    const int hs = r & 1; r >>= 1;
    const int d = r;
    const float* W = d ? whh_r : whh_f;
    const int mt = w < 4 ? 4 * (1 - hs) + w : 4 * hs + (w - 4);
    const int u = 32 * mt + (lane & 31);
    const int kl = 16 * ks + 8 * (lane >> 5) + j;
    const int row = (kl >> 7) * LH + 128 * hs + (kl & 127);
    const float v = W[row * LH + u];
// ... 113 lines not shown
}

extern "C" int ws_lstm_pack_pair_f8mx(const float* whh_f, const float* whh_r, float* pack, void* stream) {
  WS_REQUIRE(whh_f && whh_r && pack, "ws_lstm_pack_pair_f8mx: null pointer");
  hipLaunchKernelGGL(lstm_pack_pair_f8mx_kernel, dim3(32), dim3(512), 0, (hipStream_t)stream, whh_f, whh_r,
                     reinterpret_cast<char*>(pack));
  return ws_check_launch("ws_lstm_pack_pair_f8mx");
}

extern "C" int ws_lstm_pack_pair_f8(const float* whh_f, const float* whh_r, float* pack, void* stream) {
  WS_REQUIRE(whh_f && whh_r && pack, "ws_lstm_pack_pair_f8: null pointer");
  hipLaunchKernelGGL(lstm_pack_pair_f8_kernel, dim3(32), dim3(512), 0, (hipStream_t)stream, whh_f, whh_r,
                     reinterpret_cast<char*>(pack));
  return ws_check_launch("ws_lstm_pack_pair_f8");
}

extern "C" int ws_lstm_pack_pair_f16(const float* whh_f, const float* whh_r, float* pack, void* stream) {
  WS_REQUIRE(whh_f && whh_r && pack, "ws_lstm_pack_pair_f16: null pointer");
  hipLaunchKernelGGL(lstm_pack_pair_f16_kernel, dim3(512), dim3(256), 0, (hipStream_t)stream, whh_f, whh_r,
                     reinterpret_cast<_Float16*>(pack));
  return ws_check_launch("ws_lstm_pack_pair_f16");
}

extern "C" int ws_lstm_pack_pair(const float* whh_f, const float* whh_r, float* pack, void* stream) {
  WS_REQUIRE(whh_f && whh_r && pack, "ws_lstm_pack_pair: null pointer");
  hipLaunchKernelGGL(lstm_pack_pair_kernel, dim3(512), dim3(256), 0, (hipStream_t)stream, whh_f, whh_r,
                     reinterpret_cast<__bf16*>(pack));
  return ws_check_launch("ws_lstm_pack_pair");
}

__device__ __noinline__ void pair_timed_out(unsigned* tword, unsigned* status) {
  __hip_atomic_store((gu32*)tword, 1u, __ATOMIC_RELAXED, __HIP_MEMORY_SCOPE_AGENT);
  if (status) __hip_atomic_store((gu32*)status, 1u, __ATOMIC_RELAXED, __HIP_MEMORY_SCOPE_AGENT);
}

#define PAIR_RING 4
template <int RF> struct pair_ldsk { static constexpr int value = RF ? 12 : 8; };

typedef _Float16 f16x8 __attribute__((ext_vector_type(8)));
template <int RF>
__device__ __forceinline__ f32x16 pair_mfma(const bf16x8& a, const bf16x8& b, const f32x16& c) {
  if constexpr (RF != 0)
    return __builtin_amdgcn_mfma_f32_32x32x16_f16(__builtin_bit_cast(f16x8, a), __builtin_bit_cast(f16x8, b), c, 0, 0, 0);
  else
    return mfma32(a, b, c);
}

#define TS(k)                                                                                                      \
  if constexpr (V & 2048) {                                                                                        \
    if (pr == 0 && hs == 0 && wx == 0 && lane == 0 && p.dbg_buf)                                                   \
      reinterpret_cast<unsigned long long*>(p.dbg_buf)[(step * 2 + role) * 8 + (k)] = __builtin_readcyclecounter(); \
  }

template <int V, int GF = 0, int RF = 0>
__global__ __launch_bounds__(512, 2) void lstm_bwd_pair_kernel(const ws_lstm_pair_args p) {
  static_assert(RF == 0 || GF == WS_GATES_H2F, "the fp16 recurrence takes the scaled-fp16 d(gates) of WS_GATES_H2F");
  constexpr int PAIR_LDSK = pair_ldsk<RF>::value;
  __shared__ __attribute__((aligned(16))) __bf16 bimg[RF ? 1 : 2][SQ * PR_ROW];
  constexpr int LDSK8 = 27;
  constexpr int LDSB = 6;
  constexpr bool RES = RF >= 2;
  __shared__ __attribute__((aligned(16))) bf16x8 whl[RF == 3 ? 8 * LDSB * 128 : RF == 2 ? 4 * LDSK8 * 64 : 8 * PAIR_LDSK * 64];
  __shared__ __attribute__((aligned(16))) f32x4 rec[2][512];
  const int ntile = (p.nseq + SQ - 1) / SQ, npair = 2 * ntile;
  const int pr = ((int)blockIdx.x >> 4) * 8 + ((int)blockIdx.x & 7), hs = ((int)blockIdx.x >> 3) & 1;
  if (pr >= npair) return;
  long long wall_in = 0;
  if constexpr (V & 2048) wall_in = wall_clock64();
  const int d = pr & 1, tile = pr >> 1;
  const int tid = threadIdx.x, lane = tid & 63, n = lane & 31, half = lane >> 5;
  const int w = __builtin_amdgcn_readfirstlane(tid >> 6);
  const bool xrole = w < 4;
  const int wx = w & 3, role = w >> 2;
  const int L = p.L;

  const int q0 = 8 * wx + 4 * role + half;
  const int gvo = ((d * 256 + 32 * hs + q0) * 32 + n) * 16;
  const int cvo = ((d * 64 + 32 * hs + q0) * 32 + n) * 16;
  float* gdst = GF == WS_GATES_H2S ? p.dgates : p.gates;
  auto grs = [&](int t) { return mkrsrc(gdst + (long long)(tile * L + t) * (SQ * 2 * LG), SQ * 2 * LG * 4); };
  auto hrs = [&](int t) { return mkrsrc(p.gates + (long long)(tile * L + t) * (SQ * LG), SQ * 2 * LG * 2); };
  constexpr bool G2 = GF == WS_GATES_H2 || GF == WS_GATES_H2F;
  float* hdst = (G2 && p.dgates) ? p.dgates : p.gates;
  auto ors = [&](int t) { return mkrsrc(hdst + (long long)(tile * L + t) * (SQ * LG), SQ * 2 * LG * 2); };
  const float dS = GF == WS_GATES_H2F ? ws_dgates_scale(*p.amax) : 1.f;
  auto crs = [&](const float* b, int t) { return mkrsrc(b + (long long)(tile * L + t) * (SQ * 2 * LH), SQ * 2 * LH * 4); };
  typedef typename gate_cell<GF>::type gcell;
  auto ld_gate = [&](int t, int g, int e) -> gcell {
    if constexpr (GF != 0) return bld8(hrs(t), gvo >> 1, (g * 64 + 2 * e) * 256);
    else return bld(grs(t), gvo, (g * 64 + 2 * e) * 512);
  };
  const __amdgpu_buffer_rsrc_t xrs = __builtin_amdgcn_make_buffer_rsrc(
      reinterpret_cast<char*>(p.xchg) + (long long)pr * (4 * PR_XSLOT), 0, 4 * PR_XSLOT, 0x00020000);
  gu32* flags = (gu32*)(p.flags) + pr * 8;
  const int xc0 = ((8 * wx + half) * 32 + n) * 16;

  const char* wbase = reinterpret_cast<const char*>(p.wpack) + (long long)((d * 2 + hs) * 8 + w) * (2 * 32 * 1024);
  bf16x8 wh[32];
#pragma unroll
  for (int ks = 0; ks < 32; ++ks) wh[ks] = *reinterpret_cast<const bf16x8*>(wbase + ks * 1024 + lane * 16);
  bf16x8* wlds = &whl[w * PAIR_LDSK * 64 + lane];
  u32x2* wlds8 = reinterpret_cast<u32x2*>(whl) + w * LDSK8 * 64 + lane;
  u32x2 wq[RF == 2 ? 32 - LDSK8 : 1];
  v8i wq8[RF == 3 ? 8 - LDSB : 1];
  bf16x8* wlds3 = &whl[w * LDSB * 128 + lane];
  int sA = 127;
  float wS = 1.f;
  if constexpr (RF == 3) {
#pragma unroll
    for (int kb = 0; kb < 8; ++kb) {
      const i32x4 p0 = *reinterpret_cast<const i32x4*>(wbase + 32 * 1024 + kb * 2048 + lane * 16);
      const i32x4 p1 = *reinterpret_cast<const i32x4*>(wbase + 32 * 1024 + kb * 2048 + 1024 + lane * 16);
      if (kb < LDSB) {
        wlds3[(2 * kb) * 64] = __builtin_bit_cast(bf16x8, p0);
        wlds3[(2 * kb + 1) * 64] = __builtin_bit_cast(bf16x8, p1);
      } else {
        wq8[kb >= LDSB ? kb - LDSB : 0] = __builtin_shufflevector(p0, p1, 0, 1, 2, 3, 4, 5, 6, 7);
      }
    }
    sA = __builtin_amdgcn_readfirstlane(*reinterpret_cast<const int*>(wbase + 48 * 1024 + 4));
  } else if constexpr (RF == 2) {
#pragma unroll
    for (int ks = 0; ks < LDSK8; ++ks)
      wlds8[ks * 64] = *reinterpret_cast<const u32x2*>(wbase + 32 * 1024 + ks * 512 + lane * 8);
#pragma unroll
    for (int ks = 0; ks < 32 - LDSK8; ++ks)
      wq[ks] = *reinterpret_cast<const u32x2*>(wbase + 32 * 1024 + (LDSK8 + ks) * 512 + lane * 8);
    wS = __builtin_bit_cast(float, __builtin_amdgcn_readfirstlane(*reinterpret_cast<const int*>(wbase + 48 * 1024)));
  } else {
#pragma unroll
    for (int ks = 0; ks < PAIR_LDSK; ++ks)
      wlds[ks * 64] = *reinterpret_cast<const bf16x8*>(wbase + 32 * 1024 + ks * 1024 + lane * 16);
  }
  const __amdgpu_buffer_rsrc_t wrs =
      __builtin_amdgcn_make_buffer_rsrc(const_cast<char*>(wbase) + 32 * 1024, 0, 32 * 1024, 0x00020000);
  const int wlane = lane * 16;
  constexpr int NCH = 32 / PAIR_RING, CH0 = PAIR_LDSK / PAIR_RING;

  rec[0][tid] = rec[1][tid] = f32x4{0.f, 0.f, 0.f, 0.f};
  const f32x4* oth = &rec[role][(wx * 2) * 64 + lane];
  f32x4* mineo = &rec[role ^ 1][(wx * 2) * 64 + lane];

  gcell n_i[2], n_f[2], n_g[2], n_o[2];
  f32x4 n_dh[2], n_cp[2], c_cur[2], dc[2], mine[2];
  const f32x4 zero4v = {0.f, 0.f, 0.f, 0.f};
  auto load_step = [&](int t, int e) {
    n_i[e] = ld_gate(t, 0, e);
    n_f[e] = ld_gate(t, 1, e);
    n_g[e] = ld_gate(t, 2, e);
    n_o[e] = ld_gate(t, 3, e);
    n_dh[e] = bld(crs(p.dhcat, t), cvo, 2 * e * 512);
    const int tp = d == 0 ? max(t - 1, 0) : min(t + 1, L - 1);
    n_cp[e] = bld(crs(p.cbuf, tp), cvo, 2 * e * 512);
  };
  unsigned sink = 0u;
  auto touch = [&](__amdgpu_buffer_rsrc_t r, int voff, int soff) {
    asm volatile("buffer_load_dword %0, %1, %2, %3 offen" : "+v"(sink) : "v"(voff), "s"(r), "s"(soff));
  };
  auto touch_step = [&](int t) {
    const int tp = d == 0 ? max(t - 1, 0) : min(t + 1, L - 1);
#pragma unroll
    for (int e = 0; e < 2; ++e) {
#pragma unroll
      for (int g = 0; g < 4; ++g) touch(hrs(t), gvo >> 1, (g * 64 + 2 * e) * 256);
      touch(crs(p.dhcat, t), cvo, 2 * e * 512);
      touch(crs(p.cbuf, tp), cvo, 2 * e * 512);
    }
  };
  {
    const int t0 = d == 0 ? L - 1 : 0;
#pragma unroll
    for (int e = 0; e < 2; ++e) {
      load_step(t0, e);
      c_cur[e] = bld(crs(p.cbuf, t0), cvo, 2 * e * 512);
      dc[e] = mine[e] = zero4v;
    }
  }
  int dead = 0;
  __syncthreads();
  if constexpr (V & 2048) {
    if (threadIdx.x == 0 && p.dbg_buf) {
      long long* wt = reinterpret_cast<long long*>(p.dbg_buf) + (long long)L * 16 + (pr * 2 + hs) * 4;
      wt[0] = wall_in;
      wt[1] = wall_clock64();
    }
  }

  for (int step = 0; step < L; ++step) {
    const int t = d == 0 ? L - 1 - step : step;
    const int sn = min(step + 1, L - 1);
    const int tn = d == 0 ? L - 1 - sn : sn;
    const bool has_prev = d == 0 ? (t > 0) : (t < L - 1);
    const int par = step & 1;
    int zo = 0;
    asm volatile("" : "+s"(zo));
    f32x4 pk[2][4];
    TS(0);
#pragma unroll
    for (int e = 0; e < 2; ++e) {
      const int q = q0 + 2 * e;
      f32x4 dhr = mine[e] + oth[e * 64];
      if constexpr (RF != 0) dhr *= (1.f / 256.f);
      f32x4 pi, pf, pg, po;
      const f32x4 vi = gate_val<false>(n_i[e]), vf = gate_val<false>(n_f[e]), vg = gate_val<true>(n_g[e]),
                  vo = gate_val<false>(n_o[e]);
#pragma unroll
      for (int r = 0; r < 4; ++r) {
        const float ig = vi[r], fg = vf[r], gg = vg[r], og = vo[r];
        const float dhv = dh_in<GF>(n_dh[e][r], dhr[r], dS);
        const float tc = ftanh(c_cur[e][r]);
        const float dov = dhv * tc;
        const float dcv = dc[e][r] + dhv * og * (1.f - tc * tc);
        dc[e][r] = dcv * fg;
        pi[r] = dcv * gg * ig * (1.f - ig);
        pf[r] = dcv * (has_prev ? n_cp[e][r] : 0.f) * fg * (1.f - fg);
        pg[r] = dcv * ig * (1.f - gg * gg);
        po[r] = dov * og * (1.f - og);
      }
      c_cur[e] = n_cp[e];
      auto emit = [&](const f32x4& v, int g) {
        if constexpr (RF != 0) {
          const u32x2 code = enc_f16x4(v);
          *reinterpret_cast<u32x2*>(&bimg[0][n * PR_ROW + g * 128 + 4 * q]) = code;
          bst8(code, ors(t), gvo >> 1, (g * 64 + 2 * e) * 256);
          return;
        }
        bf16x4 hi, lo;
        split4(v, hi, lo);
        *reinterpret_cast<bf16x4*>(&bimg[0][n * PR_ROW + g * 128 + 4 * q]) = hi;
        *reinterpret_cast<bf16x4*>(&bimg[RF ? 0 : 1][n * PR_ROW + g * 128 + 4 * q]) = lo;
        if constexpr (G2) {
          bst8(enc_dgates<GF>(v, hi), ors(t), gvo >> 1, (g * 64 + 2 * e) * 256);
        } else {
          pk[e][g] = pack_hl4(hi, lo);
          bst(pk[e][g], grs(t), gvo, (g * 64 + 2 * e) * 512);
        }
      };
      emit(pi, 0);
      emit(pf, 1);
      emit(pg, 2);
      emit(po, 3);
    }
    if constexpr (RES) asm volatile("" : "+v"(sink));
    TS(1);
    __syncthreads();
    TS(2);

    if constexpr (RES) touch_step(tn);
    if (xrole) __builtin_amdgcn_s_setprio(1);
    bf16x8 wl[2][PAIR_RING];
    if constexpr (!RES) {
#pragma unroll
      for (int s = 0; s < 2; ++s)
#pragma unroll
        for (int f = 0; f < PAIR_RING; ++f)
          wl[s][f] = wload(wrs, wlane + f * 1024, zo + (CH0 + s) * (PAIR_RING * 1024));
    }
    const __bf16* bhi = &bimg[0][n * PR_ROW + 8 * half];
    const __bf16* blo = &bimg[RF ? 0 : 1][n * PR_ROW + 8 * half];
    f32x16 acc0, acc1;
#pragma unroll
    for (int r = 0; r < 16; ++r) acc0[r] = acc1[r] = 0.f;
// ... 139 lines not shown
          __builtin_amdgcn_s_sleep(1);
        }
      }
      TS(6);
      if (p.dbg & 64) __builtin_amdgcn_fence(__ATOMIC_ACQUIRE, "agent");
#pragma unroll
      for (int q4 = 0; q4 < 4; ++q4)
        pv[q4] = (p.dbg & 2) ? u32x4{0u, 0u, 0u, 0u}
                             : __builtin_amdgcn_raw_buffer_load_b128(xrs, xc0, (par * 2 + hs) * PR_XSLOT + q4 * 1024, SC1);
      }
      if (dead) {
#pragma unroll
        for (int q4 = 0; q4 < 4; ++q4) pv[q4] = u32x4{0x7fc00000u, 0x7fc00000u, 0x7fc00000u, 0x7fc00000u};
      }
      if (p.dbg_buf && !(V & 2048)) {
        float* db = p.dbg_buf + ((((long long)pr * L + step) * 2 + hs) * 2) * 4096;
#pragma unroll
        for (int q4 = 0; q4 < 4; ++q4) {
          *reinterpret_cast<f32x4*>(db + (xc0 >> 2) + q4 * 256) = sum[q4];
          *reinterpret_cast<u32x4*>(db + 4096 + (xc0 >> 2) + q4 * 256) = pv[q4];
        }
      }
      mine[0] = __builtin_bit_cast(f32x4, pv[0]);
      mine[1] = __builtin_bit_cast(f32x4, pv[1]);
      if constexpr (V & 2048) {
        asm volatile("s_waitcnt vmcnt(12)" ::: "memory");
        TS(7);
      }
      mineo[0] = __builtin_bit_cast(f32x4, pv[2]);
      mineo[64] = __builtin_bit_cast(f32x4, pv[3]);
    } else {
      mineo[0] = sum[0];
      mineo[64] = sum[1];
      mine[0] = sum[2];
      mine[1] = sum[3];
      TS(4);
      load_step(tn, 0);
      load_step(tn, 1);
    }
    __syncthreads();
  }
  if constexpr (V & 2048) {
    if (threadIdx.x == 0 && p.dbg_buf)
      reinterpret_cast<long long*>(p.dbg_buf)[(long long)L * 16 + (pr * 2 + hs) * 4 + 2] = wall_clock64();
  }
}

extern "C" int ws_lstm_bwd_pair(const ws_lstm_pair_args* a, void* stream) {
  WS_REQUIRE(a && a->gates && a->cbuf && a->dhcat && a->wpack && a->xchg && a->flags, "ws_lstm_bwd_pair: null pointer");
  WS_REQUIRE(a->nseq > 0 && a->L > 0, "ws_lstm_bwd_pair: nseq and L must be positive");
  WS_REQUIRE(a->gfmt >= WS_GATES_F32 && a->gfmt <= WS_GATES_H2F && (a->gfmt != WS_GATES_H2S || a->dgates) &&
                 (a->gfmt != WS_GATES_H2F || a->amax),
             "ws_lstm_bwd_pair: gfmt %d (WS_GATES_H2S needs dgates, WS_GATES_H2F needs amax)", a->gfmt);
  WS_REQUIRE(a->rfmt == 0 || (a->rfmt >= 1 && a->rfmt <= 3 && a->gfmt == WS_GATES_H2F),
             "ws_lstm_bwd_pair: rfmt %d (1 / 2 / 3 = fp16 recurrence, fp16 + fp16 / fp16 + fp8 weights / + the lo term on the FP8 "
             "MFMA: WS_GATES_H2F only)", a->rfmt);
  const int npair = 2 * ((a->nseq + SQ - 1) / SQ);
  static int cus = 0;
  if (!cus && hipDeviceGetAttribute(&cus, hipDeviceAttributeMultiprocessorCount, 0) != hipSuccess) cus = 0;
  WS_REQUIRE(2 * npair <= cus, "ws_lstm_bwd_pair: %d workgroups must be co-resident but the device has %d CUs", 2 * npair,
             cus);
  const int grid = 16 * ((npair + 7) / 8);
  hipStream_t s = (hipStream_t)stream;
  hipError_t e = hipMemsetAsync(a->flags, 0, ((size_t)npair * 8 + 8) * sizeof(unsigned), s);
  WS_REQUIRE(e == hipSuccess, "ws_lstm_bwd_pair: hipMemsetAsync failed");
  if (a->rfmt != 0) {
    e = hipMemsetAsync(a->xchg, 0x01, (size_t)npair * 4 * PR_XSLOT, s);
    WS_REQUIRE(e == hipSuccess, "ws_lstm_bwd_pair: hipMemsetAsync failed");
  }
  ws_prof_begin(WS_PROF_LSTM_BWD, s);
  if (a->rfmt == 3) {
    WS_REQUIRE(!(a->dbg & 2048), "ws_lstm_bwd_pair: cycle stamps (dbg 2048) exist for rfmt 0 .. 2");
    if (a->dbg & 8) hipLaunchKernelGGL((lstm_bwd_pair_kernel<8, WS_GATES_H2F, 3>), dim3(grid), dim3(512), 0, s, *a);
    else hipLaunchKernelGGL((lstm_bwd_pair_kernel<0, WS_GATES_H2F, 3>), dim3(grid), dim3(512), 0, s, *a);
    ws_prof_end(WS_PROF_LSTM_BWD, s);
    return ws_check_launch("ws_lstm_bwd_pair");
  }
  if (a->rfmt == 2) {
    if (a->dbg & 8) hipLaunchKernelGGL((lstm_bwd_pair_kernel<8, WS_GATES_H2F, 2>), dim3(grid), dim3(512), 0, s, *a);
    else if (a->dbg & 2048) hipLaunchKernelGGL((lstm_bwd_pair_kernel<2048, WS_GATES_H2F, 2>), dim3(grid), dim3(512), 0, s, *a);
    else hipLaunchKernelGGL((lstm_bwd_pair_kernel<0, WS_GATES_H2F, 2>), dim3(grid), dim3(512), 0, s, *a);
    ws_prof_end(WS_PROF_LSTM_BWD, s);
    return ws_check_launch("ws_lstm_bwd_pair");
  }
  if (a->rfmt == 1) {
    if (a->dbg & 8) hipLaunchKernelGGL((lstm_bwd_pair_kernel<8, WS_GATES_H2F, 1>), dim3(grid), dim3(512), 0, s, *a);
    else if (a->dbg & 2048) hipLaunchKernelGGL((lstm_bwd_pair_kernel<2048, WS_GATES_H2F, 1>), dim3(grid), dim3(512), 0, s, *a);
    else hipLaunchKernelGGL((lstm_bwd_pair_kernel<0, WS_GATES_H2F, 1>), dim3(grid), dim3(512), 0, s, *a);
    ws_prof_end(WS_PROF_LSTM_BWD, s);
    return ws_check_launch("ws_lstm_bwd_pair");
  }
  switch ((a->dbg & (8 | 2048)) + a->gfmt) {
    case 0: hipLaunchKernelGGL((lstm_bwd_pair_kernel<0, 0>), dim3(grid), dim3(512), 0, s, *a); break;
    case 1: hipLaunchKernelGGL((lstm_bwd_pair_kernel<0, WS_GATES_H2>), dim3(grid), dim3(512), 0, s, *a); break;
    case 2: hipLaunchKernelGGL((lstm_bwd_pair_kernel<0, WS_GATES_H2S>), dim3(grid), dim3(512), 0, s, *a); break;
    case 3: hipLaunchKernelGGL((lstm_bwd_pair_kernel<0, WS_GATES_H2F>), dim3(grid), dim3(512), 0, s, *a); break;
    case 8: hipLaunchKernelGGL((lstm_bwd_pair_kernel<8, 0>), dim3(grid), dim3(512), 0, s, *a); break;
    case 9: hipLaunchKernelGGL((lstm_bwd_pair_kernel<8, WS_GATES_H2>), dim3(grid), dim3(512), 0, s, *a); break;
    case 10: hipLaunchKernelGGL((lstm_bwd_pair_kernel<8, WS_GATES_H2S>), dim3(grid), dim3(512), 0, s, *a); break;
    case 11: hipLaunchKernelGGL((lstm_bwd_pair_kernel<8, WS_GATES_H2F>), dim3(grid), dim3(512), 0, s, *a); break;
    case 2048: hipLaunchKernelGGL((lstm_bwd_pair_kernel<2048, 0>), dim3(grid), dim3(512), 0, s, *a); break;
    case 2048 + 3: hipLaunchKernelGGL((lstm_bwd_pair_kernel<2048, WS_GATES_H2F>), dim3(grid), dim3(512), 0, s, *a); break;
    default: WS_REQUIRE(false, "ws_lstm_bwd_pair: dbg bits 8 and 2048 are exclusive; cycle stamps: WS_GATES_F32 / H2F only");
  }
  ws_prof_end(WS_PROF_LSTM_BWD, s);
  return ws_check_launch("ws_lstm_bwd_pair");
}
```

wesep_amd/dev.py:

```python
import ctypes as C
import os
from typing import NamedTuple, Optional

import numpy as np
import torch

from . import _lib as L

BIG = 1 << 30


def gemm_mode() -> str:
    return os.environ.get("WESEP_GEMM", "bf16x3")


def _mode_bit(mode):
    return 4 if (mode or gemm_mode()) == "bf16x3" else 0
GN_EPS = float(np.finfo(np.float32).eps)


class Rows(NamedTuple):
    div: int
    s1: int
    s2: int


def flat(ld: int) -> Rows:
    return Rows(BIG, 0, ld)


class StatMap(NamedTuple):
    div1: int
    m1: int
    div2: int
    m2: int
    base: int = 0


def _chk(t: Optional[torch.Tensor], name: str, dtype=torch.float32):
    if t is None:
        return
    if not t.is_cuda or t.dtype != dtype or not t.is_contiguous():
        raise L.WesepHipError(f"{name}: expected a contiguous {dtype} CUDA tensor, got "
                              f"{t.dtype} {t.device} contiguous={t.is_contiguous()}")


def _p(t: Optional[torch.Tensor], off: int = 0):
    if t is None:
        return None
    return C.c_void_p(t.data_ptr() + 4 * off)


ALG = None
# ... 244 lines not shown
    L.check(L.lib().ws_gn_param_grad(_p(x), _p(dxn), _p(stats), C.byref(g), nsplit, _p(slab),
                                     L.stream_ptr()), "ws_gn_param_grad")


class SeqMap(NamedTuple):
    nseq: int
    div: int
    s1: int
    s2: int
    step_rows: int
    L: int
    nvalid: int = 0


def lstm_mode(nseq: int) -> int:
    if os.environ.get("WESEP_LSTM", "bf16x3") == "bf16x3":
        return L.LSTM_BF16X3
    return L.LSTM_F32_MT2 if nseq >= 8192 else L.LSTM_F32_MT1


def lstm_blk_mode(nseq: int) -> int:
    env = os.environ.get("WESEP_LSTM_SEQS")
    if env:
        return L.LSTM_BF16X3_BLK16 if env == "16" else L.LSTM_BF16X3_BLK
    return L.LSTM_BF16X3_BLK16 if 2 * (-(-nseq // 32)) <= 128 else L.LSTM_BF16X3_BLK


def lstm_pack(whh_f, whh_r, pack_fwd, pack_bwd, mode=L.LSTM_BF16X3):
    for n, t in (("whh_f", whh_f), ("whh_r", whh_r), ("pack_fwd", pack_fwd), ("pack_bwd", pack_bwd)):
        _chk(t, n)
    L.check(L.lib().ws_lstm_pack(_p(whh_f), _p(whh_r), _p(pack_fwd), _p(pack_bwd), mode,
                                 L.stream_ptr()), "ws_lstm_pack")


def lstm_pack_bwd_f8(whh_f, whh_r, pack_bwd):
    for n, t in (("whh_f", whh_f), ("whh_r", whh_r), ("pack_bwd", pack_bwd)):
        _chk(t, n)
    L.check(L.lib().ws_lstm_pack_bwd_f8(_p(whh_f), _p(whh_r), _p(pack_bwd), L.stream_ptr()), "ws_lstm_pack_bwd_f8")


def lstm_pack_dx_f8(wcat, pack):
    for n, t in (("wcat", wcat), ("pack", pack)):
        _chk(t, n)
    L.check(L.lib().ws_lstm_pack_dx_f8(_p(wcat), _p(pack), L.stream_ptr()), "ws_lstm_pack_dx_f8")


def lstm_cat_ih(wih_f, wih_r, bih_f, bhh_f, bih_r, bhh_r, n_in, wcat, bcat):
    for t in (wih_f, wih_r, bih_f, bhh_f, bih_r, bhh_r, wcat, bcat):
        _chk(t, "lstm_cat_ih arg")
    L.check(L.lib().ws_lstm_cat_ih(_p(wih_f), _p(wih_r), _p(bih_f), _p(bhh_f), _p(bih_r), _p(bhh_r),
                                   n_in, _p(wcat), _p(bcat), L.stream_ptr()), "ws_lstm_cat_ih")


def _bptt_bytes(gfmt: int) -> int:
    return {L.GATES_F32: 40, L.GATES_H2: 24, L.GATES_H2S: 32, L.GATES_H2F: 24}[gfmt]


def gates_fmt() -> int:
    return {"h2": L.GATES_H2F, "h2b": L.GATES_H2, "h2s": L.GATES_H2S, "f32": L.GATES_F32}[os.environ.get("WESEP_GATES", "h2")]


def blh_floats(nblocks: int, C_: int) -> int:
    return nblocks * 32 * C_ // 2


def _lstm_args(gates, cbuf, hcat, wpack, sm: SeqMap, mode, dhcat=None, run_if=None, gfmt=0, gates_in=None, dgates=None,
               amax=None, rfmt=0, dxn=None, wxpack=None):
    for n, t in (("gates", gates), ("cbuf", cbuf), ("hcat", hcat), ("wpack", wpack), ("dhcat", dhcat),
                 ("gates_in", gates_in), ("dgates", dgates), ("dxn", dxn), ("wxpack", wxpack)):
        _chk(t, n)
    a = L.LstmArgs()
    a.gates, a.cbuf, a.hcat, a.dhcat, a.wpack = _p(gates), _p(cbuf), _p(hcat), _p(dhcat), _p(wpack)
    a.sq_s1, a.sq_s2, a.step_rows = sm.s1, sm.s2, sm.step_rows
    a.nseq, a.sq_div, a.L, a.mode = sm.nseq, sm.div, sm.L, mode
    a.run_if = C.c_void_p(run_if.data_ptr()) if run_if is not None else None
    a.gates_in, a.dgates, a.gfmt, a.rfmt = _p(gates_in), _p(dgates), gfmt, rfmt
    a.amax = C.c_void_p(amax.data_ptr()) if amax is not None else None
    if dxn is not None:
        if dxn.dim() != 3 or dxn.shape[0] != 2 or dxn.shape[2] != 128 or getattr(sm, "nvalid", 0):
            raise L.WesepHipError(f"lstm_bwd: dxn must be [2, P, 128] on a sequence map without padding sequences, got {tuple(dxn.shape)}")
        a.dxn, a.dxn_dir_stride, a.wxpack = _p(dxn), dxn.shape[1] * 128, _p(wxpack)
    return a


def lstm_fwd(gates, cbuf, hcat, wpack, sm: SeqMap, mode=L.LSTM_BF16X3, run_if=None, gfmt=0, gates_in=None):
    a = _lstm_args(gates, cbuf, hcat, wpack, sm, mode, run_if=run_if, gfmt=gfmt, gates_in=gates_in)
    if run_if is None:
        u = ALG_LSTM_UNITS or L.LSTM_H
        _alg("lstm_fwd", sm.nseq * sm.L * 2 * u * (16 + (2 if gfmt else 4) * 4 + 8), 2 * sm.nseq * sm.L * 2 * 4 * u * u)
    L.check(L.lib().ws_lstm_fwd(C.byref(a), L.stream_ptr()), "ws_lstm_fwd")


def lstm_bwd(gates, cbuf, hcat, dhcat, wpack, sm: SeqMap, mode=L.LSTM_BF16X3, gfmt=0, dgates=None, run_if=None, amax=None,
             rfmt=0, dxn=None, wxpack=None):
    a = _lstm_args(gates, cbuf, hcat, wpack, sm, mode, dhcat, gfmt=gfmt, dgates=dgates, run_if=run_if, amax=amax, rfmt=rfmt,
                   dxn=dxn, wxpack=wxpack)
    if run_if is None:
        _alg("lstm_bwd", _bptt_bytes(gfmt) * sm.nseq * sm.L * 2 * (ALG_LSTM_UNITS or L.LSTM_H),
             2 * sm.nseq * sm.L * 2 * 4 * (ALG_LSTM_UNITS or L.LSTM_H) ** 2)
    L.check(L.lib().ws_lstm_bwd(C.byref(a), L.stream_ptr()), "ws_lstm_bwd")


_CU_COUNT = {}


def cu_count(device) -> int:
    key = (device.type, device.index)
    if key not in _CU_COUNT:
        _CU_COUNT[key] = torch.cuda.get_device_properties(device).multi_processor_count
    return _CU_COUNT[key]


def lstm_cluster_ok(sm: SeqMap, device) -> bool:
    if os.environ.get("WESEP_LSTM_CLUSTER", "1") == "0":
        return False
    return sm.nseq % 64 == 0 and (sm.nseq // 32) * 8 <= cu_count(device) and sm.L >= 64


class _ClusterScratch:

    def __init__(self, device):
        self.device = device
        self.xchg = None
        self.flags = None
        self.status = torch.zeros(2, device=device, dtype=torch.int32)
        self.host = torch.zeros(2, dtype=torch.int32)
        if device.type == "cuda" and torch.cuda.is_available():
            self.host = self.host.pin_memory()
        self.event = None
        self.fallbacks = 0

    def get(self, xchg_floats: int, nflags: int):
        if self.xchg is None or self.xchg.numel() < xchg_floats:
            self.xchg = torch.empty(xchg_floats, device=self.device, dtype=torch.float32)
        if self.flags is None or self.flags.numel() < nflags:
            self.flags = torch.empty(nflags, device=self.device, dtype=torch.int32)
        return self.xchg, self.flags


_CLUSTER_SCRATCH = {}


def _cluster_scratch(device) -> _ClusterScratch:
    key = (device.type, device.index, L.stream_ptr().value)
    if key not in _CLUSTER_SCRATCH:
        _CLUSTER_SCRATCH[key] = _ClusterScratch(device)
    return _CLUSTER_SCRATCH[key]


# ... 106 lines not shown

def lstm_fwd_cluster2(gates, cbuf, hcat, xn, wcat, bcat, whh_f, whh_r, sm: SeqMap, status=None, dbg=0, dbg_buf=None, rfmt=None):
    for n, t in (("gates", gates), ("cbuf", cbuf), ("hcat", hcat), ("xn", xn), ("wcat", wcat), ("bcat", bcat),
                 ("whh_f", whh_f), ("whh_r", whh_r)):
        _chk(t, n)
    ncl = sm.nseq // 32
    sc = _cluster_scratch(gates.device)
    xchg, flags = sc.get(ncl * 2 * 8 * 4096 // 4, ncl * 8 + 8)
    a = L.LstmCluster2Args()
    a.gates, a.cbuf, a.hcat, a.xn, a.wcat, a.bcat = _p(gates), _p(cbuf), _p(hcat), _p(xn), _p(wcat), _p(bcat)
    a.whh_f, a.whh_r = _p(whh_f), _p(whh_r)
    tw = flags[ncl * 8:ncl * 8 + 1]
    a.xchg, a.tword = C.c_void_p(xchg.data_ptr()), C.c_void_p(tw.data_ptr())
    a.status = C.c_void_p((status if status is not None else sc.status).data_ptr())
    a.nseq, a.L, a.dbg = sm.nseq, sm.L, dbg
    a.rfmt = cluster2_rfmt() if rfmt is None else rfmt
    a.dbg_buf = C.c_void_p(dbg_buf.data_ptr()) if dbg_buf is not None else None
    u = ALG_LSTM_UNITS or L.LSTM_H
    _alg("lstm_fwd", sm.nseq * sm.L * (2 * u * 16 + 4 * 128), 2 * sm.nseq * sm.L * 2 * 4 * u * (u + 128))
    L.check(L.lib().ws_lstm_fwd_cluster2(C.byref(a), L.stream_ptr()), "ws_lstm_fwd_cluster2")
    return tw


def lstm_bwd_cluster(gates, cbuf, dhcat, whh_f, whh_r, sm: SeqMap, status=None, dbg=0):
    for n, t in (("gates", gates), ("cbuf", cbuf), ("dhcat", dhcat), ("whh_f", whh_f), ("whh_r", whh_r)):
        _chk(t, n)
    ncl = sm.nseq // 32
    sc = _cluster_scratch(gates.device)
    xchg, flags = sc.get(ncl * 2 * 64 * 8192 // 4, ncl * 8 + 8)
    a = L.LstmClusterArgs()
    a.gates, a.cbuf, a.dhcat, a.whh_f, a.whh_r = _p(gates), _p(cbuf), _p(dhcat), _p(whh_f), _p(whh_r)
    a.xchg, a.flags = C.c_void_p(xchg.data_ptr()), C.c_void_p(flags.data_ptr())
    a.status = C.c_void_p(status.data_ptr() if status is not None else sc.status.data_ptr() + 4)
    a.nseq, a.L, a.dbg = sm.nseq, sm.L, dbg
    L.check(L.lib().ws_lstm_bwd_cluster(C.byref(a), L.stream_ptr()), "ws_lstm_bwd_cluster")
    return flags[ncl * 8:ncl * 8 + 1]


def lstm_pair_ok(sm: SeqMap, device) -> bool:
    if os.environ.get("WESEP_LSTM_PAIR_BWD", "1") == "0":
        return False
    return 4 * (-(-sm.nseq // 32)) <= cu_count(device) // 2 and sm.L >= 64


def lstm_pack_pair(whh_f, whh_r, pack, f16=False):
    for n, t in (("whh_f", whh_f), ("whh_r", whh_r), ("pack", pack)):
        _chk(t, n)
    fn = (L.lib().ws_lstm_pack_pair, L.lib().ws_lstm_pack_pair_f16, L.lib().ws_lstm_pack_pair_f8,
          L.lib().ws_lstm_pack_pair_f8mx)[int(f16)]
    L.check(fn(_p(whh_f), _p(whh_r), _p(pack), L.stream_ptr()), "ws_lstm_pack_pair")


def lstm_bwd_pair(gates, cbuf, dhcat, wpack, sm: SeqMap, status=None, dbg=0, dbg_buf=None, gfmt=0, dgates=None,
                  repairable=False, amax=None, rfmt=0):
    for n, t in (("gates", gates), ("cbuf", cbuf), ("dhcat", dhcat), ("wpack", wpack), ("dgates", dgates)):
        _chk(t, n)
    npair = 2 * (-(-sm.nseq // 32))
    sc = _cluster_scratch(gates.device)
    xchg, flags = sc.get(npair * 65536 // 4, npair * 8 + 8)
    a = L.LstmPairArgs()
    a.gates, a.cbuf, a.dhcat, a.wpack = _p(gates), _p(cbuf), _p(dhcat), _p(wpack)
    a.xchg, a.flags = C.c_void_p(xchg.data_ptr()), C.c_void_p(flags.data_ptr())
    a.status = C.c_void_p(status.data_ptr() if status is not None else sc.status.data_ptr() + (0 if repairable else 4))
    a.nseq, a.L, a.dbg = sm.nseq, sm.L, dbg
    a.dbg_buf = C.c_void_p(dbg_buf.data_ptr()) if dbg_buf is not None else None
    a.gfmt, a.dgates = gfmt, _p(dgates)
    a.amax = C.c_void_p(amax.data_ptr()) if amax is not None else None
    a.rfmt = rfmt
    _alg("lstm_bwd", _bptt_bytes(gfmt) * sm.nseq * sm.L * 2 * (ALG_LSTM_UNITS or L.LSTM_H),
             2 * sm.nseq * sm.L * 2 * 4 * (ALG_LSTM_UNITS or L.LSTM_H) ** 2)
    L.check(L.lib().ws_lstm_bwd_pair(C.byref(a), L.stream_ptr()), "ws_lstm_bwd_pair")
    return flags[npair * 8:npair * 8 + 1]


class BandTables:

    def __init__(self, band_width, device):
        bw = np.asarray(band_width, dtype=np.int32)
        f0 = np.concatenate([[0], np.cumsum(bw)[:-1]]).astype(np.int32)
        self.nband = len(bw)
        self.nbins = int(bw.sum())
        self.bw_host, self.f0_host = bw, f0
        bob = np.repeat(np.arange(self.nband, dtype=np.int32), bw)
        to = lambda a: torch.from_numpy(np.ascontiguousarray(a)).to(device)
        self.band_of_bin, self.f0, self.bw = to(bob), to(f0), to(bw)
        self.bw2, self.off2 = to(2 * bw), to(2 * f0)

    def c(self):
        b = L.Bands()
        b.band_of_bin = C.c_void_p(self.band_of_bin.data_ptr())
        b.band_f0 = C.c_void_p(self.f0.data_ptr())
        b.band_bw = C.c_void_p(self.bw.data_ptr())
        b.nband, b.nbins = self.nband, self.nbins
        return b


def stft_bandsplit(wav, bands: BandTables, xbs, lengths=None):
    _chk(wav, "wav")
    _chk(xbs, "xbs")
    R, T = wav.shape
    b = bands.c()
    if lengths is not None:
        _chk_lens(lengths, R, "ws_stft_bandsplit_len")
        L.check(L.lib().ws_stft_bandsplit_len(_p(wav), R, T, _tab(lengths), C.byref(b), _p(xbs), L.stream_ptr()),
                "ws_stft_bandsplit_len")
        return
    L.check(L.lib().ws_stft_bandsplit(_p(wav), R, T, C.byref(b), _p(xbs), L.stream_ptr()),
            "ws_stft_bandsplit")


def mask_istft_frames(xbs, mask3, R, Tf, bands: BandTables, frames):
    for n, t in (("xbs", xbs), ("mask3", mask3), ("frames", frames)):
        _chk(t, n)
    b = bands.c()
    L.check(L.lib().ws_mask_istft_frames(_p(xbs), _p(mask3), R, Tf, C.byref(b), _p(frames),
                                         L.stream_ptr()), "ws_mask_istft_frames")


def istft_ola(frames, R, Tf, T, wav, lengths=None):
    _chk(frames, "frames")
    _chk(wav, "wav")
# ... 138 lines not shown
    out = torch.zeros(P, Cq * 4, device=xb.device, dtype=xb.dtype)
    out[pos[valid]] = rows[valid]
    return out


def blh_bf16_pack(xb: torch.Tensor) -> torch.Tensor:
    return xb.to(torch.bfloat16).contiguous().view(torch.float32)


def blh_f16_pack(xb: torch.Tensor) -> torch.Tensor:
    return xb.to(torch.float16).contiguous().view(torch.float32)


def blh_f16_unpack(buf: torch.Tensor, nblk: int, C_: int) -> torch.Tensor:
    return buf.reshape(-1)[: nblk * 32 * C_ // 2].view(torch.float16).view(nblk, C_ // 4, 32, 4).float()


def blh_bf16_unpack(buf: torch.Tensor, nblk: int, C_: int) -> torch.Tensor:
    return buf.reshape(-1)[: nblk * 32 * C_ // 2].view(torch.bfloat16).view(nblk, C_ // 4, 32, 4).float()


def blh_gates_unpack(buf: torch.Tensor, nblk: int) -> torch.Tensor:
    Cq = 2 * 4 * L.LSTM_H // 4
    code = (buf.reshape(-1)[: nblk * 32 * Cq * 2].view(torch.int16).to(torch.int32) & 0xFFFF).view(nblk, Cq, 32, 4).double()
    s_sig = float(torch.tensor(1.0 / 65535.0, dtype=torch.float32))
    s_tanh = float(torch.tensor(1.0 / 32767.5, dtype=torch.float32))
    is_g = ((torch.arange(Cq, device=buf.device) >> 6) & 3 == 2).view(1, Cq, 1, 1)
    return torch.where(is_g, code * s_tanh - 1.0, code * s_sig).float()


def _smc(sm: SeqMap):
    c = L.SeqMapC()
    c.sq_s1, c.sq_s2, c.step_rows, c.nseq, c.sq_div, c.L = sm.s1, sm.s2, sm.step_rows, sm.nseq, sm.div, sm.L
    c.nvalid = sm.nvalid
    return c


def pack_w(W, N: int, K: int, ldw: int, out, trans=False, order=0, w_off=0, f16=False):
    _chk(W, "W")
    _chk(out, "out")
    if out.numel() < N * K:
        raise L.WesepHipError("pack_w: output too small")
    if int(f16) == 2:
        if order != 1:
            raise L.WesepHipError("pack_w: the fp16 + FP8 pack exists in the b2p order only")
        L.check(L.lib().ws_pack_w_f16f8(_p(W, w_off), N, K, ldw, int(trans), _p(out), L.stream_ptr()), "ws_pack_w_f16f8")
        return
    fn = L.lib().ws_pack_w_f16 if f16 else L.lib().ws_pack_w
    L.check(fn(_p(W, w_off), N, K, ldw, int(trans), order, _p(out), L.stream_ptr()), "ws_pack_w_f16" if f16 else "ws_pack_w")


def gemm_p2b(*, A, lda: int, sm: SeqMap, Wpack, N: int, C_out, K=128, bias=None, A_bl=None, stats=None,
             gamma=None, beta=None, stat_map: Optional[StatMap] = None, run_if=None, amax=None, A_bl16=None, steps=None,
             steps_div=1):
    for n, t in (("A", A), ("Wpack", Wpack), ("bias", bias), ("C", C_out), ("A_bl", A_bl), ("stats", stats),
                 ("gamma", gamma), ("beta", beta), ("A_bl16", A_bl16)):
        _chk(t, n)
    a = L.GemmP2BArgs()
    a.A, a.Wpack, a.bias, a.C, a.A_bl = _p(A), _p(Wpack), _p(bias), _p(C_out), _p(A_bl)
    a.stats, a.gamma, a.beta = _p(stats), _p(gamma), _p(beta)
    a.sm = _smc(sm)
    st = stat_map or StatMap(1, 0, 1, 0, 0)
    a.st_div1, a.st_m1, a.st_div2, a.st_m2, a.st_base = st
    a.lda, a.N, a.K = lda, N, K
    a.run_if = C.c_void_p(run_if.data_ptr()) if run_if is not None else None
    a.amax = C.c_void_p(amax.data_ptr()) if amax is not None else None
    a.A_bl16 = _p(A_bl16)
    if ALG is not None and run_if is None:
        rows = (getattr(sm, "nvalid", 0) or sm.nseq) * sm.L
        _alg("gemm_nt", rows * (4 * K + 4 * N + (4 * K if A_bl is not None else 0) + (2 * K if A_bl16 is not None else 0)) + 4 * N * K,
             2 * rows * N * K)
    if steps is not None:
        _chk_lens(steps, -(-(getattr(sm, "nvalid", 0) or sm.nseq) // steps_div), "ws_gemm_p2b_len")
        L.check(L.lib().ws_gemm_p2b_len(C.byref(a), _tab(steps), steps_div, L.stream_ptr()), "ws_gemm_p2b_len")
        return
    L.check(L.lib().ws_gemm_p2b(C.byref(a), L.stream_ptr()), "ws_gemm_p2b")


def gemm_b2p(*, A, K: int, sm: SeqMap, Wpack, C_out, ldc: int, N=128, bias=None, R=None, a_fmt=0, amax=None, a16_out=None):
    for n, t in (("A", A), ("Wpack", Wpack), ("bias", bias), ("C", C_out), ("R", R), ("a16_out", a16_out)):
        _chk(t, n)
    if a16_out is not None and a_fmt != 0:
        raise L.WesepHipError("gemm_b2p: a16_out goes with a_fmt = 0 (split-pair A)")
    a = L.GemmB2PArgs()
    a.A, a.Wpack, a.bias, a.R, a.C = _p(A), _p(Wpack), _p(bias), _p(R), _p(C_out)
    a.sm = _smc(sm)
    a.ldc, a.N, a.K, a.a_fmt = ldc, N, K, a_fmt
    a.amax = C.c_void_p(amax.data_ptr()) if amax is not None else None
    a.a16_out = _p(a16_out)
    if ALG is not None:
        rows = (getattr(sm, "nvalid", 0) or sm.nseq) * sm.L
        _alg("gemm_nt", rows * ((2 if a_fmt else 4) * K + 4 * N * (1 + (R is not None)) + (2 * K if a16_out is not None else 0))
             + 4 * N * K, 2 * rows * N * K)
    L.check(L.lib().ws_gemm_b2p(C.byref(a), L.stream_ptr()), "ws_gemm_b2p")


def tnb_splits(nblk: int, gtiles: int):
    cap = int(os.environ.get("WESEP_TNB_MAXSPLIT", "64"))
    nsplit = max(1, min(cap, int(os.environ.get("WESEP_TNB_WGS", "256")) // gtiles, nblk))
    if nsplit >= 8:
        nsplit -= nsplit % 8
    bps = -(-nblk // nsplit)
    return nsplit, bps


def gemm_tnb(*, G, g_width: int, g_off: int, g_cols: int, A0, a0_width: int, a0_off: int, a0_cols: int,
             nblk: int, L_: int, slab, nsplit: int, blocks_per_split: int, a0_shift=0, A1=None, a1_width=0,
             a1_off=0, a1_cols=0, a1_shift=0, bslab=None, aslab=None, g_fmt=0, amax=None, a_fmt=0):
    for n, t in (("G", G), ("A0", A0), ("A1", A1), ("slab", slab), ("bslab", bslab), ("aslab", aslab)):
        _chk(t, n)
    a = L.GemmTNBArgs()
    a.G, a.A0, a.A1, a.slab, a.bslab, a.aslab = _p(G), _p(A0), _p(A1), _p(slab), _p(bslab), _p(aslab)
    a.slab_stride = g_cols * (a0_cols + a1_cols)
    a.bslab_stride = g_cols
    a.aslab_stride = a0_cols + a1_cols
    a.g_width, a.g_off, a.g_cols = g_width, g_off, g_cols
    a.a0_width, a.a0_off, a.a0_cols, a.a0_shift = a0_width, a0_off, a0_cols, a0_shift
    a.a1_width, a.a1_off, a.a1_cols, a.a1_shift = a1_width, a1_off, a1_cols, a1_shift
    a.nblk, a.L, a.nsplit, a.blocks_per_split, a.g_fmt, a.a_fmt = nblk, L_, nsplit, blocks_per_split, g_fmt, a_fmt
    a.amax = C.c_void_p(amax.data_ptr()) if amax is not None else None
    if ALG is not None:
        rows, acols = nblk * 32, a0_cols + a1_cols
        _alg("gemm_tn", rows * ((2 if g_fmt else 4) * g_cols + (2 if a_fmt else 4) * acols) + 4 * nsplit * g_cols * acols,
# ... 724 lines not shown
```

Baseline: 345.6 utterances/s.

## Store d(hcat) as block-scaled fp16 from projection GEMM into BPTT kernels

The projection-transpose GEMM can now emit d(hcat) directly as fp16 scaled per 32-row block, with the scale derived from the row amax of dout and the L1 norm of the projection weight. The BPTT kernels (stream and pair) read this fp16 image plus a per-block scale instead of an fp32 buffer. The aim is to halve the d(hcat) write and read traffic in the backward recurrence. In exchange it adds an amax reduction to the GEMM, extra template variants, and a bounded-precision risk in the gradients. It is enabled by default through an environment flag.

Result: no change. 349.1 utterances/s (median of 6 runs) (+1.0%).

```diff
diff --git a/include/wesep_hip.h b/include/wesep_hip.h
--- a/include/wesep_hip.h
+++ b/include/wesep_hip.h
@@ -152,6 +152,7 @@
   float* dxn;
   long long dxn_dir_stride;
   const float* wxpack;
+  const float* dh_scale;
 } ws_lstm_args;
 #define WS_GATES_F32 0
 #define WS_GATES_H2 1
@@ -219,6 +220,7 @@
   float* dgates;
   const unsigned* amax;
   int rfmt, pad_;
+  const float* dh_scale;
 } ws_lstm_pair_args;
 int ws_lstm_pack_pair(const float* whh_f, const float* whh_r, float* pack, void* stream);
 int ws_lstm_pack_pair_f16(const float* whh_f, const float* whh_r, float* pack, void* stream);
@@ -256,6 +258,9 @@
   const unsigned* run_if;
   unsigned* amax;
   void* A_bl16;
+  void* C16;
+  float* c_scale;
+  const float* w_l1;
 } ws_gemm_p2b_args;
 int ws_gemm_p2b(const ws_gemm_p2b_args* a, void* stream);
 int ws_gemm_p2b_len(const ws_gemm_p2b_args* a, const int* steps, int steps_div, void* stream);
diff --git a/wesep_amd/_lib.py b/wesep_amd/_lib.py
--- a/wesep_amd/_lib.py
+++ b/wesep_amd/_lib.py
@@ -89,7 +89,8 @@
                [(n, _ll) for n in ("sq_s1", "sq_s2", "step_rows")] + \
                [(n, _i) for n in ("nseq", "sq_div", "L", "mode")] + [("run_if", _p)] + \
                [("gates_in", _p), ("dgates", _p), ("gfmt", _i), ("rfmt", _i), ("amax", _p)] + \
-               [("dxn", _p), ("dxn_dir_stride", _ll), ("wxpack", _p)]
+               [("dxn", _p), ("dxn_dir_stride", _ll), ("wxpack", _p)] + \
+               [("dh_scale", _p)]
 
 
 class SeqMapC(C.Structure):
@@ -99,7 +100,8 @@
 class GemmP2BArgs(C.Structure):
     _fields_ = [(n, _p) for n in ("A", "Wpack", "bias", "C", "A_bl", "stats", "gamma", "beta")] + \
                [("sm", SeqMapC)] + [(n, _ll) for n in ("lda", "st_m1", "st_m2", "st_base")] + \
-               [(n, _i) for n in ("st_div1", "st_div2", "N", "K")] + [("run_if", _p), ("amax", _p), ("A_bl16", _p)]
+               [(n, _i) for n in ("st_div1", "st_div2", "N", "K")] + [("run_if", _p), ("amax", _p), ("A_bl16", _p)] + \
+               [("C16", _p), ("c_scale", _p), ("w_l1", _p)]
 
 
 class GemmB2PArgs(C.Structure):
@@ -127,7 +129,8 @@
 
 class LstmPairArgs(C.Structure):
     _fields_ = [(n, _p) for n in ("gates", "cbuf", "dhcat", "wpack", "xchg", "flags", "status", "dbg_buf")] + \
-               [("nseq", _i), ("L", _i), ("dbg", _i), ("gfmt", _i), ("dgates", _p), ("amax", _p), ("rfmt", _i), ("pad_", _i)]
+               [("nseq", _i), ("L", _i), ("dbg", _i), ("gfmt", _i), ("dgates", _p), ("amax", _p), ("rfmt", _i), ("pad_", _i),
+                ("dh_scale", _p)]
 
 
 class Bands(C.Structure):
diff --git a/wesep_amd/blstm_core.py b/wesep_amd/blstm_core.py
--- a/wesep_amd/blstm_core.py
+++ b/wesep_amd/blstm_core.py
@@ -28,6 +28,19 @@
 
 
 _PROBE_SAT = [0, 0.0]
+
+
+def dh16_block_scale(a_max, w_l1):
+    be = ((a_max.float() * w_l1).view(torch.int32) >> 23) & 0xFF
+    ok = (be >= 15) & (be != 255)
+    return torch.where(ok, (268 - be) << 23, torch.full_like(be, 127 << 23)).view(torch.float32)
+
+
+def _probe_round_dh16(dh, dout, sm, w_l1):
+    pos, valid = dev.bl_positions(sm, dout.device)
+    a = dout.reshape(-1, dout.shape[-1])[pos.reshape(-1)].abs().amax(dim=1) * valid.reshape(-1).to(dout.dtype)
+    s = dh16_block_scale(a.view(-1, 32).amax(dim=1), float(w_l1)).view(-1, 1)
+    dh.copy_((dh * s).half().float() / s)
 
 
 def _probe_round(t, kind, packed=False):
@@ -333,6 +346,8 @@
             out = _empty(d, 2 * H * N)
             dev.pack_w(W("pw"), 2 * H, N, 2 * H, out, trans=True, order=0)
             return out
+        if kind == "projT_l1":
+            return W("pw").abs().sum(dim=0).amax().reshape(1)
         raise KeyError(kind)
 
 
@@ -350,12 +365,13 @@
     band_rfmt: int
     band_dx: bool
     a_fmt: int
+    dh16: bool = False
 
 
 _WIHT_KIND = {0: "wihT", 1: "wihT", 2: "wihT16", 3: "wihT8"}
 
 
-def make_plan(seq, device, grad, gn_geo=None, ragged=False) -> BlstmPlan:
+def make_plan(seq, device, grad, gn_geo=None, ragged=False, dh16=True) -> BlstmPlan:
     lmode = dev.lstm_blk_mode(seq.nseq)
     cluster = dev.lstm_cluster_ok(seq, device)
     bptt = _bptt_kind(seq, device, cluster)
@@ -371,10 +387,13 @@
         fwd = "stream"
     g_fmt = {L.GATES_H2: 1, L.GATES_H2F: 2}.get(gfmt, 0)
     brf = band_rfmt(gfmt, lmode) if grad and bptt == "stream" else 0
+    bdx = bool(brf) and gn_geo is not None and band_dx(brf, seq, gn_geo)
+    d16 = (dh16 and grad and gfmt == L.GATES_H2F and bptt in ("pair", "stream") and not bdx and dev.dh16_on()
+           and not _pair_stamp_on() and dev.dh16_accepted())
     return BlstmPlan(
         nb=dev.bl_num_blocks(seq), lmode=lmode, cluster=cluster, fwd=fwd, bptt=bptt, grad=grad, gfmt=gfmt, g_fmt=g_fmt,
         a16=gfmt == L.GATES_H2F and grad and tnb_a16(), pair_rfmt=pair_rfmt(gfmt) if grad and bptt == "pair" else 0,
-        band_rfmt=brf, band_dx=bool(brf) and gn_geo is not None and band_dx(brf, seq, gn_geo), a_fmt=dxn_fmt(g_fmt))
+        band_rfmt=brf, band_dx=bdx, a_fmt=dxn_fmt(g_fmt), dh16=d16)
 
 
 def consume_once(ctx, who):
@@ -438,6 +457,8 @@
             _probe_round(cbuf, "f16")
     if plan.grad:
         W("projT")
+        if plan.dh16:
+            W("projT_l1")
         if not plan.band_dx:
             W(_WIHT_KIND[plan.a_fmt])
         if plan.bptt == "pair":
@@ -454,12 +475,18 @@
 def blstm_bptt(plan, W, gates, cbuf, hcat, dout, seq, release):
     d = dout.device
     nb, gfmt = plan.nb, plan.gfmt
-    dh, dout_bl = _empty(d, nb, 32 * 2 * H), _empty(d, nb, 32 * N)
+    dout_bl = _empty(d, nb, 32 * N)
     dxn2 = None
     amax = amax_word(d) if gfmt == L.GATES_H2F else None
-    dev.gemm_p2b(A=dout, lda=N, sm=seq, Wpack=W("projT"), N=2 * H, C_out=dh, A_bl=dout_bl, amax=amax)
-    if _h2_probe() & 16:
-        _probe_round(dh, "bf16")
+    if plan.dh16:
+        dh, dhs = _empty(d, dev.blh_floats(nb, 2 * H)), dict(dh_scale=_empty(d, nb))
+        dev.gemm_p2b(A=dout, lda=N, sm=seq, Wpack=W("projT"), N=2 * H, C_out=None, A_bl=dout_bl, amax=amax, C16=dh,
+                     c_scale=dhs["dh_scale"], w_l1=W("projT_l1"))
+    else:
+        dh, dhs = _empty(d, nb, 32 * 2 * H), {}
+        dev.gemm_p2b(A=dout, lda=N, sm=seq, Wpack=W("projT"), N=2 * H, C_out=dh, A_bl=dout_bl, amax=amax)
+        if _h2_probe() & 16:
+            _probe_round_dh16(dh, dout, seq, W("projT_l1"))
     ready = mark_wgrads_ready(d) if release else None
     if plan.bptt == "cluster":
         dg = gates
@@ -474,8 +501,8 @@
         dg = _empty(d, nb, 32 * 2 * G4) if gfmt == L.GATES_H2S else _empty(d, dev.blh_floats(nb, 2 * G4))
         rf = plan.pair_rfmt
         tw = dev.lstm_bwd_pair(gates, cbuf, dh, W("hhp16" if rf else "hhp"), seq, gfmt=gfmt, dgates=dg, repairable=True,
-                               dbg=_pair_dbg(), amax=amax, rfmt=rf, dbg_buf=_pair_stamp_buf(d, seq.L))
-        dev.lstm_bwd(gates, cbuf, hcat, dh, W("hh")[1], seq, plan.lmode, gfmt=gfmt, dgates=dg, run_if=tw, amax=amax)
+                               dbg=_pair_dbg(), amax=amax, rfmt=rf, dbg_buf=_pair_stamp_buf(d, seq.L), **dhs)
+        dev.lstm_bwd(gates, cbuf, hcat, dh, W("hh")[1], seq, plan.lmode, gfmt=gfmt, dgates=dg, run_if=tw, amax=amax, **dhs)
     else:
         dg = _empty(d, nb, 32 * 2 * G4) if gfmt == L.GATES_H2S else gates
         brf = plan.band_rfmt
@@ -483,7 +510,7 @@
             dxn2 = _empty(d, 2, dout.numel() // N, N)
         dev.lstm_bwd(gates, cbuf, hcat, dh, W("hh8") if brf else W("hh")[1], seq, plan.lmode, gfmt=gfmt,
                      dgates=dg if gfmt == L.GATES_H2S else None, amax=amax, rfmt=brf, dxn=dxn2,
-                     wxpack=W("wx8") if dxn2 is not None else None)
+                     wxpack=W("wx8") if dxn2 is not None else None, **dhs)
     if _h2_probe() & 2 and gfmt == L.GATES_F32:
         _probe_round(gates, "bf16", packed=True)
     if _h2_probe() & 32 and gfmt == L.GATES_F32 and not torch.cuda.is_available():
diff --git a/wesep_amd/csrc/gemm_blk.hip b/wesep_amd/csrc/gemm_blk.hip
--- a/wesep_amd/csrc/gemm_blk.hip
+++ b/wesep_amd/csrc/gemm_blk.hip
@@ -184,7 +184,14 @@
 }
 
 #define P2B_K 128
-template <bool LEN>
+__device__ __forceinline__ float p2b_block_scale(float bound, float& inv) {
+  const int be = (int)((__float_as_uint(bound) >> 23) & 0xffu);
+  inv = 1.f;
+  if (be < 15 || be == 255) return 1.f;
+  inv = __uint_as_float((unsigned)(be - 14) << 23);
+  return __uint_as_float((unsigned)(268 - be) << 23);
+}
+template <bool LEN, int H16>
 __global__ __launch_bounds__(512, 4) void gemm_p2b_kernel(const ws_gemm_p2b_args p, const int* __restrict__ steps,
                                                           int steps_div) {
   __shared__ __attribute__((aligned(16))) u32x4 wl[2][2048];
@@ -204,6 +211,7 @@
   }
 
   bf16x8 xh[8], xl[8];
+  float amx = 0.f;
   {
     const float* arow = p.A + pos * p.lda;
     float mean = 0.f, rstd = 1.f;
@@ -231,6 +239,11 @@
       }
       const float v[8] = {v0[0], v0[1], v0[2], v0[3], v1[0], v1[1], v1[2], v1[3]};
       split8(v, xh[ks], xl[ks]);
+      if constexpr (H16) {
+        amx = fmaxf(fmaxf(amx, fmaxf(fmaxf(fabsf(v[0]), fabsf(v[1])), fmaxf(fabsf(v[2]), fabsf(v[3])))),
+                    fmaxf(fmaxf(fabsf(v[4]), fabsf(v[5])), fmaxf(fabsf(v[6]), fabsf(v[7]))));
+        asm volatile("" : "+v"(amx));
+      }
       if (eb && active) {
         u32x4 c0, c1;
         pack8(xh[ks], xl[ks], c0, c1);
@@ -255,8 +268,18 @@
 #pragma unroll
   for (int q = 0; q < 4; ++q) wl[0][tid + 512 * q] = wreg[q];
   __syncthreads();
-  float* cblk = p.C + (long long)bb * 32 * p.N + i * 4;
-  float cmax = 0.f;
+  float* cblk = p.C ? p.C + (long long)bb * 32 * p.N + i * 4 : nullptr;
+  unsigned cmax = 0u;
+  float sb = 1.f;
+  unsigned short* c16blk = nullptr;
+  if constexpr (H16) {
+#pragma unroll
+    for (int o = 32; o > 0; o >>= 1) amx = fmaxf(amx, __shfl_xor(amx, o, 64));
+    float inv;
+    sb = p2b_block_scale(amx * *p.w_l1, inv);
+    if (active && lane == 0) p.c_scale[bb] = inv;
+    c16blk = reinterpret_cast<unsigned short*>(p.C16) + (long long)bb * 32 * p.N + i * 4;
+  }
   for (int st = 0; st < nstage; ++st) {
     const int cur = st & 1;
     if (st + 1 < nstage) {
@@ -288,8 +311,13 @@
           f32x4 v = {acc[4 * j], acc[4 * j + 1], acc[4 * j + 2], acc[4 * j + 3]};
           if (p.bias) v += *reinterpret_cast<const f32x4*>(p.bias + n);
           if (!valid) v = f32x4{0.f, 0.f, 0.f, 0.f};
-          *reinterpret_cast<f32x4*>(cblk + (n / 4) * 128) = v;
-          cmax = fmaxf(fmaxf(cmax, fmaxf(fabsf(v[0]), fabsf(v[1]))), fmaxf(fabsf(v[2]), fabsf(v[3])));
+          if constexpr (H16 != 1) *reinterpret_cast<f32x4*>(cblk + (n / 4) * 128) = v;
+          if constexpr (H16) {
+            const f16x2 h0 = {(_Float16)(v[0] * sb), (_Float16)(v[1] * sb)}, h1 = {(_Float16)(v[2] * sb), (_Float16)(v[3] * sb)};
+            *reinterpret_cast<u32x2*>(c16blk + (n / 4) * 128) = u32x2{__builtin_bit_cast(unsigned, h0), __builtin_bit_cast(unsigned, h1)};
+          }
+#pragma unroll
+          for (int r = 0; r < 4; ++r) cmax = max(cmax, min(__float_as_uint(fabsf(v[r])), 0x7f800000u));
         }
       }
     }
@@ -301,13 +329,15 @@
   }
   if (p.amax) {
 #pragma unroll
-    for (int o = 32; o > 0; o >>= 1) cmax = fmaxf(cmax, __shfl_xor(cmax, o, 64));
-    if (lane == 0) atomicMax(p.amax, __float_as_uint(cmax));
+    for (int o = 32; o > 0; o >>= 1) cmax = max(cmax, (unsigned)__shfl_xor((int)cmax, o, 64));
+    if (lane == 0) atomicMax(p.amax, cmax);
   }
 }
 
 static int gemm_p2b_launch(const char* who, const ws_gemm_p2b_args* a, const int* steps, int steps_div, void* stream) {
-  WS_REQUIRE(a && a->A && ((a->Wpack && a->C) || (a->N == 0 && (a->A_bl || a->A_bl16))), "%s: null pointer", who);
+  WS_REQUIRE(a && a->A && ((a->Wpack && (a->C || a->C16)) || (a->N == 0 && (a->A_bl || a->A_bl16))), "%s: null pointer", who);
+  WS_REQUIRE(!a->C16 || (a->N > 0 && a->c_scale && a->w_l1 && !a->bias),
+             "%s: C16 (block-scaled fp16 output) needs N > 0, c_scale, w_l1 and no bias", who);
   WS_REQUIRE(a->K == P2B_K, "%s: K must be %d (got %d)", who, P2B_K, a->K);
   WS_REQUIRE(a->N >= 0 && a->N % 64 == 0, "%s: N %% 64 (N=%d)", who, a->N);
   WS_REQUIRE(a->lda >= a->K && a->lda % 4 == 0, "%s: lda", who);
@@ -317,10 +347,20 @@
   hipStream_t s = (hipStream_t)stream;
   const bool timed = a->run_if == nullptr;
   if (timed) ws_prof_begin(WS_PROF_GEMM_NT, s);
-  if (steps)
-    hipLaunchKernelGGL((gemm_p2b_kernel<true>), dim3((nblk + 7) / 8), dim3(512), 0, s, *a, steps, steps_div);
+  const dim3 grid((nblk + 7) / 8);
+  const int h16 = a->C16 ? (a->C ? 2 : 1) : 0;
+  if (steps && h16 == 2)
+    hipLaunchKernelGGL((gemm_p2b_kernel<true, 2>), grid, dim3(512), 0, s, *a, steps, steps_div);
+  else if (steps && h16)
+    hipLaunchKernelGGL((gemm_p2b_kernel<true, 1>), grid, dim3(512), 0, s, *a, steps, steps_div);
+  else if (steps)
+    hipLaunchKernelGGL((gemm_p2b_kernel<true, 0>), grid, dim3(512), 0, s, *a, steps, steps_div);
+  else if (h16 == 2)
+    hipLaunchKernelGGL((gemm_p2b_kernel<false, 2>), grid, dim3(512), 0, s, *a, steps, steps_div);
+  else if (h16)
+    hipLaunchKernelGGL((gemm_p2b_kernel<false, 1>), grid, dim3(512), 0, s, *a, steps, steps_div);
   else
-    hipLaunchKernelGGL((gemm_p2b_kernel<false>), dim3((nblk + 7) / 8), dim3(512), 0, s, *a, steps, steps_div);
+    hipLaunchKernelGGL((gemm_p2b_kernel<false, 0>), grid, dim3(512), 0, s, *a, steps, steps_div);
   if (timed) ws_prof_end(WS_PROF_GEMM_NT, s);
   return ws_check_launch(who);
 }
diff --git a/wesep_amd/csrc/lstm.hip b/wesep_amd/csrc/lstm.hip
--- a/wesep_amd/csrc/lstm.hip
+++ b/wesep_amd/csrc/lstm.hip
@@ -378,6 +378,8 @@
   WS_REQUIRE(!a->dxn || (bwd && a->rfmt == 2 && a->wxpack && a->dxn_dir_stride > 0 && a->dxn_dir_stride < (1ll << 29) && !a->run_if),
              "%s: dxn (d(xn) inside the BPTT, ABI v19) needs rfmt 2, wxpack (ws_lstm_pack_dx_f8), 0 < dxn_dir_stride < 2^29 floats "
              "(32-bit store offsets) and no run_if", who);
+  WS_REQUIRE(!a->dh_scale || (bwd && (a->mode == WS_LSTM_BF16X3_BLK || a->mode == WS_LSTM_BF16X3_BLK16) && a->gfmt == WS_GATES_H2F && !a->dxn),
+             "%s: dh_scale (block-scaled fp16 d(hcat)) needs ws_lstm_bwd, a blocked-layout mode, WS_GATES_H2F and no dxn", who);
   return WS_OK;
 }
 
diff --git a/wesep_amd/csrc/lstm_bf16.hip b/wesep_amd/csrc/lstm_bf16.hip
--- a/wesep_amd/csrc/lstm_bf16.hip
+++ b/wesep_amd/csrc/lstm_bf16.hip
@@ -299,9 +299,10 @@
   }
 }
 
-template <bool BLK, int DBG, int GF = 0, int RF = 0, bool DX = false>
+template <bool BLK, int DBG, int GF = 0, int RF = 0, bool DX = false, bool DH16 = false>
 __global__ __launch_bounds__(512, 2) void lstm_bwd_bf16_kernel(const ws_lstm_args p) {
   static_assert(RF == 0 || (BLK && GF == WS_GATES_H2F), "the fp16 recurrence takes the scaled-fp16 d(gates) of WS_GATES_H2F");
+  static_assert(!DH16 || (BLK && GF == WS_GATES_H2F && !DX), "block-scaled fp16 d(hcat): blocked layout, WS_GATES_H2F, no d(xn)");
   static_assert(!DX || RF == 2, "d(xn) in the BPTT rides on the fp16 d(gates) image of rfmt 2");
   __shared__ __attribute__((aligned(16))) __bf16 dgl[RF ? 1 : 2][SQ * DROW];
   __shared__ __attribute__((aligned(16))) f32x4 xred[DX ? 8 * 2 * 64 : 1];
@@ -344,6 +345,11 @@
     if constexpr (BLK) return bld(crs(b, t), clane, 2 * j * 512);
     else return *reinterpret_cast<const f32x4*>(b + coff(t, j));
   };
+  typedef typename dh_cell<DH16>::type dhcell;
+  auto ld_dh = [&](int t, int j) -> dhcell {
+    if constexpr (DH16) return bld8(mkrsrc(p.dhcat + (long long)(bx * L + t) * (SQ * LH), SQ * 2 * LH * 2), clane >> 1, 2 * j * 256);
+    else return ld_ch(p.dhcat, t, j);
+  };
 
   const int kpar = DX ? (w >> 2) : 0;
   const __amdgpu_buffer_rsrc_t wrs = __builtin_amdgcn_make_buffer_rsrc(
@@ -407,7 +413,9 @@
   const __amdgpu_buffer_rsrc_t xors = __builtin_amdgcn_make_buffer_rsrc(
       DX ? p.dxn + (long long)d * p.dxn_dir_stride : nullptr, 0, DX ? (unsigned)(p.dxn_dir_stride * 4) : 0u, 0x00020000);
   gcell n_i[4], n_f[4], n_g[4], n_o[4];
-  f32x4 n_dh[4], n_cp[4], c_cur[4], dc[4];
+  dhcell n_dh[4];
+  float n_ds = 1.f;
+  f32x4 n_cp[4], c_cur[4], dc[4];
   f32x16 dhr;
   const f32x4 zero4v = {0.f, 0.f, 0.f, 0.f};
 #pragma unroll
@@ -420,7 +428,10 @@
     n_f[j] = ld_gate(t, 1, j);
     n_g[j] = ld_gate(t, 2, j);
     n_o[j] = ld_gate(t, 3, j);
-    n_dh[j] = ld_ch(p.dhcat, t, j);
+    n_dh[j] = ld_dh(t, j);
+    if constexpr (DH16) {
+      if (j == 0) n_ds = p.dh_scale[bx * L + t];
+    }
     const int tp = d == 0 ? max(t - 1, 0) : min(t + 1, L - 1);
     n_cp[j] = ld_ch(p.cbuf, tp, j);
   };
@@ -448,6 +459,7 @@
     asm volatile("" : "+s"(zo));
     __bf16* dhi = &dgl[0][l31 * DROW + ubase];
     __bf16* dlo = &dgl[RF ? 0 : 1][l31 * DROW + ubase];
+    const float dSb = DH16 ? dS * dh_uniform(n_ds) : dS;
 #pragma unroll
     for (int j = 0; j < 4; ++j) {
       f32x4 pi, pf, pg, po;
@@ -456,7 +468,7 @@
 #pragma unroll
       for (int r = 0; r < 4; ++r) {
         const float ig = vi[r], fg = vf[r], gg = vg[r], og = vo[r];
-        const float dhv = dh_in<GF>(n_dh[j][r], dhr[4 * j + r], dS);
+        const float dhv = dh_in<GF>(dh_elem(n_dh[j], r), dhr[4 * j + r], dSb);
         const float tc = ftanh(c_cur[j][r]);
         const float dov = dhv * tc;
         const float dcv = dc[j][r] + dhv * og * (1.f - tc * tc);
@@ -633,6 +645,12 @@
 
 int ws_launch_lstm_bwd_bf16(const ws_lstm_args* a, hipStream_t s) {
   dim3 grid((a->nseq + SQ - 1) / SQ, 2), block(512);
+  if (a->dh_scale) {
+    if (a->rfmt == 3) hipLaunchKernelGGL((lstm_bwd_bf16_kernel<true, 0, WS_GATES_H2F, 3, false, true>), grid, block, 0, s, *a);
+    else if (a->rfmt == 2) hipLaunchKernelGGL((lstm_bwd_bf16_kernel<true, 0, WS_GATES_H2F, 2, false, true>), grid, block, 0, s, *a);
+    else hipLaunchKernelGGL((lstm_bwd_bf16_kernel<true, 0, WS_GATES_H2F, 0, false, true>), grid, block, 0, s, *a);
+    return 0;
+  }
   if (a->rfmt == 2 && a->dxn) {
     hipLaunchKernelGGL((lstm_bwd_bf16_kernel<true, 0, WS_GATES_H2F, 2, true>), grid, block, 0, s, *a);
     return 0;
diff --git a/wesep_amd/csrc/lstm_bf16_common.h b/wesep_amd/csrc/lstm_bf16_common.h
--- a/wesep_amd/csrc/lstm_bf16_common.h
+++ b/wesep_amd/csrc/lstm_bf16_common.h
@@ -132,6 +132,14 @@
   else return dh + rec;
 }
 
+template <bool DH16> struct dh_cell { typedef f32x4 type; };
+template <> struct dh_cell<true> { typedef u32x2 type; };
+__device__ __forceinline__ float dh_elem(const f32x4& c, int r) { return c[r]; }
+__device__ __forceinline__ float dh_elem(const u32x2& c, int r) { return (float)__builtin_bit_cast(f16x4, c)[r]; }
+__device__ __forceinline__ float dh_uniform(float raw) {
+  return __builtin_bit_cast(float, __builtin_amdgcn_readfirstlane(__builtin_bit_cast(int, raw)));
+}
+
 template <int GF> struct gate_cell { typedef f32x4 type; };
 template <> struct gate_cell<WS_GATES_H2> { typedef u32x2 type; };
 template <> struct gate_cell<WS_GATES_H2S> { typedef u32x2 type; };
diff --git a/wesep_amd/csrc/lstm_bf16_s16.hip b/wesep_amd/csrc/lstm_bf16_s16.hip
--- a/wesep_amd/csrc/lstm_bf16_s16.hip
+++ b/wesep_amd/csrc/lstm_bf16_s16.hip
@@ -197,8 +197,9 @@
 #ifndef S16_DBG
 #define S16_DBG 0
 #endif
-template <int GF>
+template <int GF, bool DH16 = false>
 __global__ __launch_bounds__(512, 2) void lstm_bwd_s16_kernel(const ws_lstm_args p) {
+  static_assert(!DH16 || GF == WS_GATES_H2F, "block-scaled fp16 d(hcat): WS_GATES_H2F only");
   __shared__ __attribute__((aligned(16))) __bf16 dgl[2][S16 * DROW];
   if (p.run_if && *p.run_if == 0u) return;
   const int d = blockIdx.y;
@@ -223,6 +224,11 @@
   };
   auto st_gate = [&](const f32x4& v, int t, int g, int tu) { bst(v, grs(t), glane, (g * 64 + 4 * tu) * 512); };
   auto ld_ch = [&](const float* b, int t, int tu) -> f32x4 { return bld(crs(b, t), clane, 4 * tu * 512); };
+  typedef typename dh_cell<DH16>::type dhcell;
+  auto ld_dh = [&](int t, int tu) -> dhcell {
+    if constexpr (DH16) return bld8(mkrsrc(p.dhcat + (long long)(tile * L + t) * (SQ * LH), SQ * 2 * LH * 2), clane >> 1, 4 * tu * 256);
+    else return ld_ch(p.dhcat, t, tu);
+  };
   const int ubase = 32 * w + 4 * mq;
 
   const __amdgpu_buffer_rsrc_t wrs = __builtin_amdgcn_make_buffer_rsrc(
@@ -235,7 +241,9 @@
     for (int f = 0; f < 16; ++f) wr[s][f] = wload(wrs, wlane + (f & 3) * 1024, s * 16384 + (f >> 2) * 4096);
 
   gcell n_i[2], n_f[2], n_g[2], n_o[2];
-  f32x4 n_dh[2], n_cp[2], c_cur[2], dc[2], dhr[2];
+  dhcell n_dh[2];
+  float n_ds = 1.f;
+  f32x4 n_cp[2], c_cur[2], dc[2], dhr[2];
   const f32x4 zero4v = {0.f, 0.f, 0.f, 0.f};
 #pragma unroll
   for (int tu = 0; tu < 2; ++tu) dc[tu] = dhr[tu] = zero4v;
@@ -244,7 +252,10 @@
     n_f[tu] = ld_gate(t, 1, tu);
     n_g[tu] = ld_gate(t, 2, tu);
     n_o[tu] = ld_gate(t, 3, tu);
-    n_dh[tu] = ld_ch(p.dhcat, t, tu);
+    n_dh[tu] = ld_dh(t, tu);
+    if constexpr (DH16) {
+      if (tu == 0) n_ds = p.dh_scale[tile * L + t];
+    }
     const int tp = d == 0 ? max(t - 1, 0) : min(t + 1, L - 1);
     n_cp[tu] = ld_ch(p.cbuf, tp, tu);
   };
@@ -266,6 +277,7 @@
     asm volatile("" : "+s"(zo));
     __bf16* dhi = &dgl[0][n * DROW + ubase];
     __bf16* dlo = &dgl[1][n * DROW + ubase];
+    const float dSb = DH16 ? dS * dh_uniform(n_ds) : dS;
 #pragma unroll
     for (int tu = 0; tu < 2; ++tu) {
       f32x4 pi, pf, pg, po;
@@ -274,7 +286,7 @@
 #pragma unroll
       for (int r = 0; r < 4; ++r) {
         const float ig = vi[r], fg = vf[r], gg = vg[r], og = vo[r];
-        const float dhv = dh_in<GF>(n_dh[tu][r], dhr[tu][r], dS);
+        const float dhv = dh_in<GF>(dh_elem(n_dh[tu], r), dhr[tu][r], dSb);
         const float tc = ftanh(c_cur[tu][r]);
         const float dov = dhv * tc;
         const float dcv = dc[tu][r] + dhv * og * (1.f - tc * tc);
@@ -351,6 +363,7 @@
   dim3 grid(2 * ((a->nseq + SQ - 1) / SQ), 2), block(512);
   if (a->gfmt == WS_GATES_H2) hipLaunchKernelGGL(lstm_bwd_s16_kernel<WS_GATES_H2>, grid, block, 0, s, *a);
   else if (a->gfmt == WS_GATES_H2S) hipLaunchKernelGGL(lstm_bwd_s16_kernel<WS_GATES_H2S>, grid, block, 0, s, *a);
+  else if (a->gfmt == WS_GATES_H2F && a->dh_scale) hipLaunchKernelGGL((lstm_bwd_s16_kernel<WS_GATES_H2F, true>), grid, block, 0, s, *a);
   else if (a->gfmt == WS_GATES_H2F) hipLaunchKernelGGL(lstm_bwd_s16_kernel<WS_GATES_H2F>, grid, block, 0, s, *a);
   else hipLaunchKernelGGL(lstm_bwd_s16_kernel<0>, grid, block, 0, s, *a);
   return 0;
diff --git a/wesep_amd/csrc/lstm_pair.hip b/wesep_amd/csrc/lstm_pair.hip
--- a/wesep_amd/csrc/lstm_pair.hip
+++ b/wesep_amd/csrc/lstm_pair.hip
@@ -189,9 +189,10 @@
       reinterpret_cast<unsigned long long*>(p.dbg_buf)[(step * 2 + role) * 8 + (k)] = __builtin_readcyclecounter(); \
   }
 
-template <int V, int GF = 0, int RF = 0>
+template <int V, int GF = 0, int RF = 0, bool DH16 = false>
 __global__ __launch_bounds__(512, 2) void lstm_bwd_pair_kernel(const ws_lstm_pair_args p) {
   static_assert(RF == 0 || GF == WS_GATES_H2F, "the fp16 recurrence takes the scaled-fp16 d(gates) of WS_GATES_H2F");
+  static_assert(!DH16 || GF == WS_GATES_H2F, "block-scaled fp16 d(hcat): WS_GATES_H2F only");
   constexpr int PAIR_LDSK = pair_ldsk<RF>::value;
   __shared__ __attribute__((aligned(16))) __bf16 bimg[RF ? 1 : 2][SQ * PR_ROW];
   constexpr int LDSK8 = 27;
@@ -222,10 +223,16 @@
   auto ors = [&](int t) { return mkrsrc(hdst + (long long)(tile * L + t) * (SQ * LG), SQ * 2 * LG * 2); };
   const float dS = GF == WS_GATES_H2F ? ws_dgates_scale(*p.amax) : 1.f;
   auto crs = [&](const float* b, int t) { return mkrsrc(b + (long long)(tile * L + t) * (SQ * 2 * LH), SQ * 2 * LH * 4); };
+  auto drs = [&](int t) { return mkrsrc(p.dhcat + (long long)(tile * L + t) * (SQ * LH), SQ * 2 * LH * 2); };
   typedef typename gate_cell<GF>::type gcell;
+  typedef typename dh_cell<DH16>::type dhcell;
   auto ld_gate = [&](int t, int g, int e) -> gcell {
     if constexpr (GF != 0) return bld8(hrs(t), gvo >> 1, (g * 64 + 2 * e) * 256);
     else return bld(grs(t), gvo, (g * 64 + 2 * e) * 512);
+  };
+  auto ld_dh = [&](int t, int e) -> dhcell {
+    if constexpr (DH16) return bld8(drs(t), cvo >> 1, 2 * e * 256);
+    else return bld(crs(p.dhcat, t), cvo, 2 * e * 512);
   };
   const __amdgpu_buffer_rsrc_t xrs = __builtin_amdgcn_make_buffer_rsrc(
       reinterpret_cast<char*>(p.xchg) + (long long)pr * (4 * PR_XSLOT), 0, 4 * PR_XSLOT, 0x00020000);
@@ -279,14 +286,19 @@
   f32x4* mineo = &rec[role ^ 1][(wx * 2) * 64 + lane];
 
   gcell n_i[2], n_f[2], n_g[2], n_o[2];
-  f32x4 n_dh[2], n_cp[2], c_cur[2], dc[2], mine[2];
+  dhcell n_dh[2];
+  float n_ds = 1.f;
+  f32x4 n_cp[2], c_cur[2], dc[2], mine[2];
   const f32x4 zero4v = {0.f, 0.f, 0.f, 0.f};
   auto load_step = [&](int t, int e) {
     n_i[e] = ld_gate(t, 0, e);
     n_f[e] = ld_gate(t, 1, e);
     n_g[e] = ld_gate(t, 2, e);
     n_o[e] = ld_gate(t, 3, e);
-    n_dh[e] = bld(crs(p.dhcat, t), cvo, 2 * e * 512);
+    n_dh[e] = ld_dh(t, e);
+    if constexpr (DH16) {
+      if (e == 0) n_ds = p.dh_scale[tile * L + t];
+    }
     const int tp = d == 0 ? max(t - 1, 0) : min(t + 1, L - 1);
     n_cp[e] = bld(crs(p.cbuf, tp), cvo, 2 * e * 512);
   };
@@ -300,7 +312,8 @@
     for (int e = 0; e < 2; ++e) {
 #pragma unroll
       for (int g = 0; g < 4; ++g) touch(hrs(t), gvo >> 1, (g * 64 + 2 * e) * 256);
-      touch(crs(p.dhcat, t), cvo, 2 * e * 512);
+      if constexpr (DH16) touch(drs(t), cvo >> 1, 2 * e * 256);
+      else touch(crs(p.dhcat, t), cvo, 2 * e * 512);
       touch(crs(p.cbuf, tp), cvo, 2 * e * 512);
     }
   };
@@ -332,6 +345,7 @@
     int zo = 0;
     asm volatile("" : "+s"(zo));
     f32x4 pk[2][4];
+    const float dSb = DH16 ? dS * dh_uniform(n_ds) : dS;
     TS(0);
 #pragma unroll
     for (int e = 0; e < 2; ++e) {
@@ -344,7 +358,7 @@
 #pragma unroll
       for (int r = 0; r < 4; ++r) {
         const float ig = vi[r], fg = vf[r], gg = vg[r], og = vo[r];
-        const float dhv = dh_in<GF>(n_dh[e][r], dhr[r], dS);
+        const float dhv = dh_in<GF>(dh_elem(n_dh[e], r), dhr[r], dSb);
         const float tc = ftanh(c_cur[e][r]);
         const float dov = dhv * tc;
         const float dcv = dc[e][r] + dhv * og * (1.f - tc * tc);
@@ -590,6 +604,8 @@
   WS_REQUIRE(a->gfmt >= WS_GATES_F32 && a->gfmt <= WS_GATES_H2F && (a->gfmt != WS_GATES_H2S || a->dgates) &&
                  (a->gfmt != WS_GATES_H2F || a->amax),
              "ws_lstm_bwd_pair: gfmt %d (WS_GATES_H2S needs dgates, WS_GATES_H2F needs amax)", a->gfmt);
+  WS_REQUIRE(!a->dh_scale || (a->gfmt == WS_GATES_H2F && !(a->dbg & 2048)),
+             "ws_lstm_bwd_pair: dh_scale (block-scaled fp16 d(hcat)) is a format of WS_GATES_H2F; no cycle-stamped build");
   WS_REQUIRE(a->rfmt == 0 || (a->rfmt >= 1 && a->rfmt <= 3 && a->gfmt == WS_GATES_H2F),
              "ws_lstm_bwd_pair: rfmt %d (1 / 2 / 3 = fp16 recurrence, fp16 + fp16 / fp16 + fp8 weights / + the lo term on the FP8 "
              "MFMA: WS_GATES_H2F only)", a->rfmt);
@@ -609,22 +625,34 @@
   ws_prof_begin(WS_PROF_LSTM_BWD, s);
   if (a->rfmt == 3) {
     WS_REQUIRE(!(a->dbg & 2048), "ws_lstm_bwd_pair: cycle stamps (dbg 2048) exist for rfmt 0 .. 2");
-    if (a->dbg & 8) hipLaunchKernelGGL((lstm_bwd_pair_kernel<8, WS_GATES_H2F, 3>), dim3(grid), dim3(512), 0, s, *a);
+    if (a->dh_scale && (a->dbg & 8)) hipLaunchKernelGGL((lstm_bwd_pair_kernel<8, WS_GATES_H2F, 3, true>), dim3(grid), dim3(512), 0, s, *a);
+    else if (a->dh_scale) hipLaunchKernelGGL((lstm_bwd_pair_kernel<0, WS_GATES_H2F, 3, true>), dim3(grid), dim3(512), 0, s, *a);
+    else if (a->dbg & 8) hipLaunchKernelGGL((lstm_bwd_pair_kernel<8, WS_GATES_H2F, 3>), dim3(grid), dim3(512), 0, s, *a);
     else hipLaunchKernelGGL((lstm_bwd_pair_kernel<0, WS_GATES_H2F, 3>), dim3(grid), dim3(512), 0, s, *a);
     ws_prof_end(WS_PROF_LSTM_BWD, s);
     return ws_check_launch("ws_lstm_bwd_pair");
   }
   if (a->rfmt == 2) {
-    if (a->dbg & 8) hipLaunchKernelGGL((lstm_bwd_pair_kernel<8, WS_GATES_H2F, 2>), dim3(grid), dim3(512), 0, s, *a);
+    if (a->dh_scale && (a->dbg & 8)) hipLaunchKernelGGL((lstm_bwd_pair_kernel<8, WS_GATES_H2F, 2, true>), dim3(grid), dim3(512), 0, s, *a);
+    else if (a->dh_scale) hipLaunchKernelGGL((lstm_bwd_pair_kernel<0, WS_GATES_H2F, 2, true>), dim3(grid), dim3(512), 0, s, *a);
+    else if (a->dbg & 8) hipLaunchKernelGGL((lstm_bwd_pair_kernel<8, WS_GATES_H2F, 2>), dim3(grid), dim3(512), 0, s, *a);
     else if (a->dbg & 2048) hipLaunchKernelGGL((lstm_bwd_pair_kernel<2048, WS_GATES_H2F, 2>), dim3(grid), dim3(512), 0, s, *a);
     else hipLaunchKernelGGL((lstm_bwd_pair_kernel<0, WS_GATES_H2F, 2>), dim3(grid), dim3(512), 0, s, *a);
     ws_prof_end(WS_PROF_LSTM_BWD, s);
     return ws_check_launch("ws_lstm_bwd_pair");
   }
   if (a->rfmt == 1) {
-    if (a->dbg & 8) hipLaunchKernelGGL((lstm_bwd_pair_kernel<8, WS_GATES_H2F, 1>), dim3(grid), dim3(512), 0, s, *a);
+    if (a->dh_scale && (a->dbg & 8)) hipLaunchKernelGGL((lstm_bwd_pair_kernel<8, WS_GATES_H2F, 1, true>), dim3(grid), dim3(512), 0, s, *a);
+    else if (a->dh_scale) hipLaunchKernelGGL((lstm_bwd_pair_kernel<0, WS_GATES_H2F, 1, true>), dim3(grid), dim3(512), 0, s, *a);
+    else if (a->dbg & 8) hipLaunchKernelGGL((lstm_bwd_pair_kernel<8, WS_GATES_H2F, 1>), dim3(grid), dim3(512), 0, s, *a);
     else if (a->dbg & 2048) hipLaunchKernelGGL((lstm_bwd_pair_kernel<2048, WS_GATES_H2F, 1>), dim3(grid), dim3(512), 0, s, *a);
     else hipLaunchKernelGGL((lstm_bwd_pair_kernel<0, WS_GATES_H2F, 1>), dim3(grid), dim3(512), 0, s, *a);
+    ws_prof_end(WS_PROF_LSTM_BWD, s);
+    return ws_check_launch("ws_lstm_bwd_pair");
+  }
+  if (a->dh_scale) {
+    if (a->dbg & 8) hipLaunchKernelGGL((lstm_bwd_pair_kernel<8, WS_GATES_H2F, 0, true>), dim3(grid), dim3(512), 0, s, *a);
+    else hipLaunchKernelGGL((lstm_bwd_pair_kernel<0, WS_GATES_H2F, 0, true>), dim3(grid), dim3(512), 0, s, *a);
     ws_prof_end(WS_PROF_LSTM_BWD, s);
     return ws_check_launch("ws_lstm_bwd_pair");
   }
diff --git a/wesep_amd/dev.py b/wesep_amd/dev.py
--- a/wesep_amd/dev.py
+++ b/wesep_amd/dev.py
@@ -1,4 +1,5 @@
 import ctypes as C
+import inspect
 import os
 from typing import NamedTuple, Optional
 
@@ -349,8 +350,21 @@
                                    n_in, _p(wcat), _p(bcat), L.stream_ptr()), "ws_lstm_cat_ih")
 
 
+def dh16_on() -> bool:
+    return os.environ.get("WESEP_DH16", "1") != "0"
+
+
+def dh16_accepted() -> bool:
+    def names(fn, kws):
+        try:
+            return all(k in inspect.signature(fn).parameters for k in kws)
+        except (TypeError, ValueError):
+            return False
+    return (names(gemm_p2b, ("C16", "c_scale", "w_l1")) and names(lstm_bwd, ("dh_scale",)) and names(lstm_bwd_pair, ("dh_scale",)))
+
+
 def _bptt_bytes(gfmt: int) -> int:
-    return {L.GATES_F32: 40, L.GATES_H2: 24, L.GATES_H2S: 32, L.GATES_H2F: 24}[gfmt]
+    return {L.GATES_F32: 40, L.GATES_H2: 24, L.GATES_H2S: 32, L.GATES_H2F: 22 if dh16_on() and dh16_accepted() else 24}[gfmt]
 
 
 def gates_fmt() -> int:
@@ -362,9 +376,9 @@
 
 
 def _lstm_args(gates, cbuf, hcat, wpack, sm: SeqMap, mode, dhcat=None, run_if=None, gfmt=0, gates_in=None, dgates=None,
-               amax=None, rfmt=0, dxn=None, wxpack=None):
+               amax=None, rfmt=0, dxn=None, wxpack=None, dh_scale=None):
     for n, t in (("gates", gates), ("cbuf", cbuf), ("hcat", hcat), ("wpack", wpack), ("dhcat", dhcat),
-                 ("gates_in", gates_in), ("dgates", dgates), ("dxn", dxn), ("wxpack", wxpack)):
+                 ("gates_in", gates_in), ("dgates", dgates), ("dxn", dxn), ("wxpack", wxpack), ("dh_scale", dh_scale)):
         _chk(t, n)
     a = L.LstmArgs()
     a.gates, a.cbuf, a.hcat, a.dhcat, a.wpack = _p(gates), _p(cbuf), _p(hcat), _p(dhcat), _p(wpack)
@@ -377,6 +391,10 @@
         if dxn.dim() != 3 or dxn.shape[0] != 2 or dxn.shape[2] != 128 or getattr(sm, "nvalid", 0):
             raise L.WesepHipError(f"lstm_bwd: dxn must be [2, P, 128] on a sequence map without padding sequences, got {tuple(dxn.shape)}")
         a.dxn, a.dxn_dir_stride, a.wxpack = _p(dxn), dxn.shape[1] * 128, _p(wxpack)
+    if dh_scale is not None:
+        if dhcat is None or dh_scale.numel() < bl_num_blocks(sm) or dhcat.numel() < blh_floats(bl_num_blocks(sm), 2 * L.LSTM_H):
+            raise L.WesepHipError("lstm_bwd: dh_scale needs one float per block and dhcat as the BLH(2H) image")
+        a.dh_scale = _p(dh_scale)
     return a
 
 
@@ -389,9 +407,9 @@
 
 
 def lstm_bwd(gates, cbuf, hcat, dhcat, wpack, sm: SeqMap, mode=L.LSTM_BF16X3, gfmt=0, dgates=None, run_if=None, amax=None,
-             rfmt=0, dxn=None, wxpack=None):
+             rfmt=0, dxn=None, wxpack=None, dh_scale=None):
     a = _lstm_args(gates, cbuf, hcat, wpack, sm, mode, dhcat, gfmt=gfmt, dgates=dgates, run_if=run_if, amax=amax, rfmt=rfmt,
-                   dxn=dxn, wxpack=wxpack)
+                   dxn=dxn, wxpack=wxpack, dh_scale=dh_scale)
     if run_if is None:
         _alg("lstm_bwd", _bptt_bytes(gfmt) * sm.nseq * sm.L * 2 * (ALG_LSTM_UNITS or L.LSTM_H),
              2 * sm.nseq * sm.L * 2 * 4 * (ALG_LSTM_UNITS or L.LSTM_H) ** 2)
@@ -604,9 +622,11 @@
 
 
 def lstm_bwd_pair(gates, cbuf, dhcat, wpack, sm: SeqMap, status=None, dbg=0, dbg_buf=None, gfmt=0, dgates=None,
-                  repairable=False, amax=None, rfmt=0):
-    for n, t in (("gates", gates), ("cbuf", cbuf), ("dhcat", dhcat), ("wpack", wpack), ("dgates", dgates)):
-        _chk(t, n)
+                  repairable=False, amax=None, rfmt=0, dh_scale=None):
+    for n, t in (("gates", gates), ("cbuf", cbuf), ("dhcat", dhcat), ("wpack", wpack), ("dgates", dgates), ("dh_scale", dh_scale)):
+        _chk(t, n)
+    if dh_scale is not None and (dh_scale.numel() < bl_num_blocks(sm) or dhcat.numel() < blh_floats(bl_num_blocks(sm), 2 * L.LSTM_H)):
+        raise L.WesepHipError("lstm_bwd_pair: dh_scale needs one float per block and dhcat as the BLH(2H) image")
     npair = 2 * (-(-sm.nseq // 32))
     sc = _cluster_scratch(gates.device)
     xchg, flags = sc.get(npair * 65536 // 4, npair * 8 + 8)
@@ -619,6 +639,7 @@
     a.gfmt, a.dgates = gfmt, _p(dgates)
     a.amax = C.c_void_p(amax.data_ptr()) if amax is not None else None
     a.rfmt = rfmt
+    a.dh_scale = _p(dh_scale)
     _alg("lstm_bwd", _bptt_bytes(gfmt) * sm.nseq * sm.L * 2 * (ALG_LSTM_UNITS or L.LSTM_H),
              2 * sm.nseq * sm.L * 2 * 4 * (ALG_LSTM_UNITS or L.LSTM_H) ** 2)
     L.check(L.lib().ws_lstm_bwd_pair(C.byref(a), L.stream_ptr()), "ws_lstm_bwd_pair")
@@ -863,10 +884,13 @@
 
 def gemm_p2b(*, A, lda: int, sm: SeqMap, Wpack, N: int, C_out, K=128, bias=None, A_bl=None, stats=None,
              gamma=None, beta=None, stat_map: Optional[StatMap] = None, run_if=None, amax=None, A_bl16=None, steps=None,
-             steps_div=1):
+             steps_div=1, C16=None, c_scale=None, w_l1=None):
     for n, t in (("A", A), ("Wpack", Wpack), ("bias", bias), ("C", C_out), ("A_bl", A_bl), ("stats", stats),
-                 ("gamma", gamma), ("beta", beta), ("A_bl16", A_bl16)):
-        _chk(t, n)
+                 ("gamma", gamma), ("beta", beta), ("A_bl16", A_bl16), ("C16", C16), ("c_scale", c_scale), ("w_l1", w_l1)):
+        _chk(t, n)
+    if C16 is not None and (c_scale is None or w_l1 is None or c_scale.numel() < bl_num_blocks(sm)
+                            or C16.numel() < blh_floats(bl_num_blocks(sm), N)):
+        raise L.WesepHipError("gemm_p2b: C16 needs BLH(N) storage, c_scale with one float per block and w_l1")
     a = L.GemmP2BArgs()
     a.A, a.Wpack, a.bias, a.C, a.A_bl = _p(A), _p(Wpack), _p(bias), _p(C_out), _p(A_bl)
     a.stats, a.gamma, a.beta = _p(stats), _p(gamma), _p(beta)
@@ -877,9 +901,11 @@
     a.run_if = C.c_void_p(run_if.data_ptr()) if run_if is not None else None
     a.amax = C.c_void_p(amax.data_ptr()) if amax is not None else None
     a.A_bl16 = _p(A_bl16)
+    a.C16, a.c_scale, a.w_l1 = _p(C16), _p(c_scale), _p(w_l1)
     if ALG is not None and run_if is None:
         rows = (getattr(sm, "nvalid", 0) or sm.nseq) * sm.L
-        _alg("gemm_nt", rows * (4 * K + 4 * N + (4 * K if A_bl is not None else 0) + (2 * K if A_bl16 is not None else 0)) + 4 * N * K,
+        c_bytes = (rows * 4 * N if C_out is not None else 0) + (rows * 2 * N + 4 * bl_num_blocks(sm) if C16 is not None else 0)
+        _alg("gemm_nt", rows * (4 * K + (4 * K if A_bl is not None else 0) + (2 * K if A_bl16 is not None else 0)) + c_bytes + 4 * N * K,
              2 * rows * N * K)
     if steps is not None:
         _chk_lens(steps, -(-(getattr(sm, "nvalid", 0) or sm.nseq) // steps_div), "ws_gemm_p2b_len")
```
